# olga24912/lodestar

Hardware: AMD Instinct MI355X
Metric: verified signature sets/sec (node) (higher is better)
Workload: dtype u32/u64 (28-bit-limb Montgomery integer arithmetic); 1 GPU; C2 gossip attestation flood: 16384 single-pubkey sets per GPU, 1 set per batchable job; pk_mode=device table, sig_encoding=compressed 96 B, distinct_messages=16384, group_sets=1024, group_policy=0, inflight=32, slots=3, hw_queues=4, merge_sets=131072, pipeline_depth=3, parallelism=shard-by-job x1 (in-process devices), no collective

## Files before the change

### include/blsgpu.h

```cpp
#ifndef BLSGPU_H
#define BLSGPU_H

#include <stdint.h>

#ifdef __cplusplus
extern "C" {
#endif

#define BLSGPU_ABI_VERSION 8

#define BLSGPU_JOB_BATCHABLE 1u
#define BLSGPU_JOB_URGENT 2u

enum blsgpu_code {
  BLSGPU_OK = 0,
  BLSGPU_BAD_ENCODING = 1,
  BLSGPU_POINT_NOT_ON_CURVE = 2,
  BLSGPU_POINT_NOT_IN_GROUP = 3,
  BLSGPU_AGGR_TYPE_MISMATCH = 4,
  BLSGPU_VERIFY_FAIL = 5,
  BLSGPU_PK_IS_INFINITY = 6,
  BLSGPU_BAD_SCALAR = 7,
  BLSGPU_INVALID_SIZE = 8,
  BLSGPU_EMPTY_AGGREGATE = 9,
  BLSGPU_EMPTY_SET = 10,
  BLSGPU_DEVICE_ERROR = 11,
  BLSGPU_ERR_ARGS = 100,
  BLSGPU_ERR_NO_DEVICE = 101,
  BLSGPU_ERR_CLOSED = 102,
  BLSGPU_ERR_ENTROPY = 103
};

typedef struct blsgpu_ctx blsgpu_ctx;

typedef struct blsgpu_batch {
  uint32_t n_sets;
  uint32_t n_jobs;
  const uint32_t* job_first_set;
  const uint8_t* job_flags;
  const uint8_t* pk_bytes;
  const uint32_t* set_pk_first;
  const uint32_t* pk_index;
  const uint8_t* msgs;
  const uint8_t* sigs;
  const uint32_t* sig_len;
  uint32_t sig_stride;
  uint64_t seed;
} blsgpu_batch;

typedef struct blsgpu_stats {
  uint32_t groups;
  uint32_t batch_retries;
  uint32_t batch_sigs_success;
  uint32_t devices_used;
  double device_ms;
  double stage_ms[8];
  uint32_t unique_messages;
  uint32_t pairing_units;
  uint32_t miller_chunks;
  uint32_t run_sets;
  uint32_t run_calls;
  uint32_t fallback_jobs;
  uint32_t fallback_miller;
  uint32_t urgent_lane;
  double host_ms;
} blsgpu_stats;

int blsgpu_init(const int* devices, int n_devices, blsgpu_ctx** out);
void blsgpu_destroy(blsgpu_ctx* ctx);
int blsgpu_device_count(const blsgpu_ctx* ctx);

int blsgpu_pubkeys_upload(blsgpu_ctx* ctx, uint32_t first_index, const uint8_t* pk96, uint32_t n);
uint32_t blsgpu_pubkeys_count(const blsgpu_ctx* ctx);

int blsgpu_verify(blsgpu_ctx* ctx, const blsgpu_batch* batch, int8_t* job_result, blsgpu_stats* stats);

typedef void (*blsgpu_done_cb)(void* user, int status);
int blsgpu_submit(blsgpu_ctx* ctx, const blsgpu_batch* batch, int8_t* job_result, blsgpu_stats* stats,
                  blsgpu_done_cb done, void* user);

int blsgpu_set_option(blsgpu_ctx* ctx, const char* key, int64_t value);
int blsgpu_get_option(const blsgpu_ctx* ctx, const char* key, int64_t* value);

int blsgpu_chunkify(uint32_t len, uint32_t min_per_chunk, uint32_t* chunk_first, uint32_t* n_chunks);

int blsgpu_aggregate_pubkeys(blsgpu_ctx* ctx, const blsgpu_batch* b, uint8_t* out, uint32_t out_len,
                             int8_t* status);

#define BLSGPU_AGG_VALIDATE 1u

int blsgpu_aggregate_signatures(blsgpu_ctx* ctx, uint32_t n_groups, const uint32_t* group_first,
                                const uint8_t* sigs, uint32_t sig_stride, const uint32_t* sig_len,
                                uint32_t flags, uint8_t* out, uint32_t out_len, int8_t* status,
                                uint32_t* first_bad);
uint32_t blsgpu_sig_agg_lanes(uint32_t n_groups, uint32_t n_sigs);

int blsgpu_randomness_words(uint32_t n, uint64_t seed, uint64_t* words);

int blsgpu_aggregate_with_randomness(blsgpu_ctx* ctx, uint32_t n_groups, const uint32_t* group_first,
                                     const uint8_t* pk_bytes, const uint32_t* pk_index, const uint8_t* sigs,
                                     uint32_t sig_stride, const uint32_t* sig_len, uint64_t seed, uint8_t* out_pk,
                                     uint32_t out_pk_len, uint8_t* out_sig, uint32_t out_sig_len, int8_t* status,
                                     uint32_t* first_bad);
uint32_t blsgpu_awr_lanes(uint32_t n_groups, uint32_t n_sets);

#define BLSGPU_SAME_LANE_FORMS 1u

typedef struct blsgpu_same_message_stats {
  uint32_t groups_accepted;
  uint32_t groups_retried;
  uint32_t retry_sets;
  uint32_t unique_messages;
  uint32_t form;
  double device_ms;
} blsgpu_same_message_stats;

int blsgpu_verify_same_message(blsgpu_ctx* ctx, uint32_t n_groups, const uint32_t* group_first,
                               const uint8_t* msgs , const uint8_t* pk_bytes,
                               const uint32_t* pk_index, const uint8_t* sigs, uint32_t sig_stride,
                               const uint32_t* sig_len, uint64_t seed, uint32_t flags,
                               int8_t* set_result , int8_t* group_result ,
                               blsgpu_same_message_stats* stats );
uint32_t blsgpu_same_message_form(uint32_t n_items, uint32_t flags);

int blsgpu_key_validate(blsgpu_ctx* ctx, uint32_t n, const uint8_t* pks, uint32_t pk_len, uint32_t stride,
                        uint8_t* out96, int8_t* status);

#define BLSGPU_ROOT_OBJECT 0
#define BLSGPU_ROOT_ATTESTATION_DATA 1
int blsgpu_signing_roots(blsgpu_ctx* ctx, int kind, uint32_t n, const uint8_t* objects, uint32_t object_stride,
                         const uint8_t* domains, uint32_t domain_stride, uint8_t* out32);

int blsgpu_shard_jobs(const uint32_t* job_first_set, const uint32_t* set_pk_first, uint32_t n_jobs,
                      uint32_t n_parts, uint32_t* part_first_job);

int blsgpu_route_call(uint32_t n_sets, uint32_t n_devices, const int64_t* device_load, int64_t split_sets,
                      uint32_t start, uint32_t* out_devices, uint32_t* n_out);

int blsgpu_batch_scalars(const blsgpu_batch* b, uint64_t* words);

#define BLSGPU_INJECT_ENTROPY 1
#define BLSGPU_INJECT_DEVICE 2
int blsgpu_debug_inject(int what, int64_t skip, int64_t count);

const char* blsgpu_code_name(int code);

int blsgpu_debug_op(blsgpu_ctx* ctx, int op, uint32_t n, const uint8_t* in, uint32_t in_stride,
                    uint8_t* out, uint32_t out_stride, int32_t* status);

#ifdef __cplusplus
}
#endif
#endif
```

### lodestar_amd/build.py

```python
import hashlib
import os
import subprocess
import sys
import time

PKG = os.path.dirname(os.path.abspath(__file__))
ROOT = os.path.dirname(PKG)
CSRC = os.path.join(PKG, "csrc")
LIB = os.environ.get("BLSGPU_LIB") or os.path.join(PKG, "libblsgpu.so")
ARCH = os.environ.get("BLSGPU_ARCH", "gfx950")
HIPCC = os.environ.get("HIPCC", "/opt/rocm/bin/hipcc")
SOURCES = ["k_sig.hip", "k_msm.hip", "k_hash.hip", "k_hmap.hip", "k_pk.hip", "k_sigagg.hip", "k_awr.hip", "k_same.hip", "k_miller.hip", "k_group.hip", "k_inv.hip", "k_ssz.hip", "k_debug.hip",
           "runtime.cpp", "helpers.cpp"]


OBJ_DIR = os.path.join(PKG, "build")


TU_DEFINES = {"k_sig.hip": ["BLS_INLINE_BIG=1"]}


def tu_defines():
    env = os.environ.get("BLSGPU_TU_DEFINES")
    if env is None:
        return TU_DEFINES
    out = {}
    for part in filter(None, env.split(";")):
        tu, _, defs = part.partition("=")
        out[tu] = [d for d in defs.split("+") if d]
    return out


_ILP = ["-mllvm", "-amdgpu-sched-strategy=max-ilp"]
_MINREG = ["-mllvm", "-amdgpu-sched-strategy=iterative-minreg"]
TU_CFLAGS = {"k_hash.hip": _MINREG, "k_pk.hip": _ILP}


def tu_cflags():
    env = os.environ.get("BLSGPU_TU_CFLAGS")
    if env is None:
        return TU_CFLAGS
    out = {}
    for part in filter(None, env.split(";")):
        tu, _, flags = part.partition("=")
        out[tu] = flags.split()
    return out


def _headers():
    out = [os.path.join(ROOT, "include", "blsgpu.h")]
    for f in os.listdir(CSRC):
        if f.endswith((".hpp", ".h")):
            out.append(os.path.join(CSRC, f))
    return out


def _tu_deps(src):
    if src.endswith(".cpp"):
        return [os.path.join(CSRC, f) for f in (src, "kernels.h", "batch_rand.hpp", "runtime_internal.hpp",
                                                "helper_layout.hpp", "miller_plan.hpp")] + [
            os.path.join(ROOT, "include", "blsgpu.h")]
    return [os.path.join(CSRC, src)] + _headers()


def _deps():
    return _headers() + [os.path.join(CSRC, s) for s in SOURCES] + [os.path.abspath(__file__)]


def up_to_date():
    if not os.path.exists(LIB):
        return False
    t = os.path.getmtime(LIB)
    return all(os.path.getmtime(d) <= t for d in _deps())


def build(force=False, verbose=True):
    if not force and up_to_date():
        build_node_addon(verbose=verbose)
        return LIB
    objs = []
    common = ["-O3", "-std=c++17", "-fPIC", f"--offload-arch={ARCH}", "-I", os.path.join(ROOT, "include")]
    defines = os.environ.get("BLSGPU_DEFINES", "").split()
    common += ["-D" + d for d in defines]
    cflags = os.environ.get("BLSGPU_CFLAGS", "").split()
    common += cflags
    tu_defs = tu_defines()
    os.makedirs(OBJ_DIR, exist_ok=True)
    key = os.path.splitext(os.path.basename(LIB))[0] + ("." + "_".join(defines).replace("=", "-") if defines else "")
    if cflags:
        key += ".cf" + hashlib.md5(" ".join(cflags).encode()).hexdigest()[:8]
    procs = []
    t0 = time.time()
    for src in SOURCES:
        tdefs = tu_defs.get(src, [])
        tflags = tu_cflags().get(src, [])
        obj = os.path.join(OBJ_DIR, key + "." + os.path.splitext(src)[0] +
                           ("." + "_".join(tdefs).replace("=", "-") if tdefs else "") +
                           (".cf" + hashlib.md5(" ".join(tflags).encode()).hexdigest()[:8] if tflags else "") + ".o")
        objs.append(obj)
        if not force and os.path.exists(obj) and all(os.path.getmtime(d) <= os.path.getmtime(obj) for d in _tu_deps(src)):
            continue
        cmd = [HIPCC] + common + ["-D" + d for d in tdefs] + tflags + ["-c", os.path.join(CSRC, src), "-o", obj]
        if verbose:
            print(" ".join(cmd), flush=True)
        procs.append((src, subprocess.Popen(cmd)))
    for src, p in procs:
        if p.wait() != 0:
            raise RuntimeError(f"hipcc failed on {src}")
        if verbose:
            print(f"  {src}: done at {time.time() - t0:.0f} s", flush=True)
    cmd = [HIPCC, f"--offload-arch={ARCH}", "-shared", "-o", LIB] + objs + ["-lpthread"]
    if verbose:
        print(" ".join(cmd), flush=True)
    subprocess.check_call(cmd)
    build_node_addon(verbose=verbose)
    return LIB


NODE_DIR = os.path.join(PKG, "node")
ADDON = os.path.join(NODE_DIR, "blsgpu_napi.node")
NODE_INC = "/usr/include/node"


def build_node_addon(force=False, verbose=True):
    src = os.path.join(NODE_DIR, "blsgpu_napi.c")
    if not os.path.exists(os.path.join(NODE_INC, "node_api.h")):
        if verbose:
            print("node headers not found: N-API addon not built", flush=True)
        return None
    if not force and os.path.exists(ADDON) and os.path.getmtime(ADDON) >= max(
            os.path.getmtime(src), os.path.getmtime(LIB), os.path.getmtime(os.path.join(ROOT, "include", "blsgpu.h"))):
        return ADDON
    cmd = ["gcc", "-O2", "-std=c11", "-Wall", "-Wno-unused-parameter", "-shared", "-fPIC",
           "-DNODE_GYP_MODULE_NAME=blsgpu_napi", "-I", NODE_INC, "-I", os.path.join(ROOT, "include"), src,
           "-o", ADDON, "-L", PKG, "-l:libblsgpu.so", "-Wl,-rpath,$ORIGIN/.."]
    if verbose:
        print(" ".join(cmd), flush=True)
    subprocess.check_call(cmd)
    return ADDON


if __name__ == "__main__":
    build(force="--force" in sys.argv)
```

### lodestar_amd/csrc/helpers.cpp

```cpp
#include "helper_layout.hpp"
#include "runtime_internal.hpp"

using namespace blsgpu_rt;
namespace hl = helper_layout;

static_assert(hl::kFp == W_FP && hl::kG1A == W_G1A && hl::kG1J == W_G1J && hl::kG2A == W_G2A && hl::kG2J == W_G2J &&
                  hl::kFp12 == W_FP12 && hl::kAwrTabWords == AWR_TAB_WORDS && hl::kMillerLineWords == kMillerLineWords,
              "helper_layout.hpp restates the element widths of kernels.h");

namespace {

template <class Body>
int helper_call(blsgpu_ctx* ctx, bool reads_table, Body body) {
  if (!enter(ctx)) return BLSGPU_ERR_CLOSED;
  struct Leave {
    blsgpu_ctx* ctx;
    ~Leave() { leave(ctx); }
  } leave_on_exit{ctx};
  Device& d = *ctx->devs[0];
  try {
    std::lock_guard<std::mutex> helper(d.helper_mu);
    std::shared_lock<std::shared_mutex> tl(d.table_mu, std::defer_lock);
    if (reads_table) tl.lock();
    HIPCHK(hipSetDevice(d.id));
    return body(d, d.helper, d.table_stream);
  } catch (HipError&) {
    return BLSGPU_DEVICE_ERROR;
  }
}

struct Grouped {
  uint32_t G;
  const uint32_t* group_first;
  const uint8_t* sigs;
  uint32_t sig_stride;
  const uint32_t* sig_len;
  const uint8_t* pk_bytes = nullptr;
  const uint32_t* pk_index = nullptr;
  uint32_t n = 0;
};

int check_group_layout(Grouped& a) {
  if (a.group_first[0] != 0) return BLSGPU_ERR_ARGS;
  for (uint32_t g = 0; g < a.G; g++)
    if (a.group_first[g + 1] < a.group_first[g]) return BLSGPU_ERR_ARGS;
  a.n = a.group_first[a.G];
  if (a.n > (1u << 20)) return BLSGPU_ERR_ARGS;
  if (a.sig_stride < 192)
    for (uint32_t k = 0; k < a.n; k++)
      if (a.sig_len[k] == 192) return BLSGPU_ERR_ARGS;
  return BLSGPU_OK;
}

int same_begin(const Device& d, const Grouped& a, uint64_t seed, std::vector<uint64_t>& words, uint64_t& hash_key) {
  batch_rand::Key key;
  if (!resolve_key(seed, key, hash_key)) return BLSGPU_ERR_ENTROPY;
  words.resize(a.n);
  batch_rand::words(key, 0, a.n, words.data());
  if (a.pk_index)
    for (uint32_t k = 0; k < a.n; k++)
      if (a.pk_index[k] >= d.table_n) return BLSGPU_ERR_ARGS;
  return BLSGPU_OK;
}

template <class Layout>
PipelineBuffers sig_inputs(Slot& sl, const Grouped& a, const Layout& l, uint8_t* flags, uint8_t* status,
                           hipStream_t s) {
  uint8_t* din = sl.d_in.p;
  HIPCHK(hipMemcpyAsync(din + l.gf, a.group_first, (size_t)(a.G + 1) * 4, hipMemcpyHostToDevice, s));
  if (a.n) {
    HIPCHK(hipMemcpyAsync(din + l.len, a.sig_len, (size_t)a.n * 4, hipMemcpyHostToDevice, s));
    HIPCHK(hipMemcpyAsync(din + l.sigs, a.sigs, (size_t)a.n * a.sig_stride, hipMemcpyHostToDevice, s));
  }
  PipelineBuffers pb{};
  pb.n = a.n;
  pb.sigs = din + l.sigs;
  pb.sig_len = reinterpret_cast<uint32_t*>(din + l.len);
  pb.sig_stride = a.sig_stride;
  pb.sig_aff = sl.d_work.p;
  pb.flags = flags;
  pb.status = reinterpret_cast<int8_t*>(status);
  return pb;
}

template <class Layout>
AwrBuffers same_inputs(Device& d, const Grouped& a, const Layout& l, uint8_t* bytes, const uint64_t* words,
                       uint32_t lanes, hipStream_t s, PipelineBuffers& pb) {
  uint8_t* din = d.helper.d_in.p;
  uint32_t* w = d.helper.d_work.p;
  pb = sig_inputs(d.helper, a, l.in, bytes + l.b_fl, bytes + l.b_st, s);
  if (a.n) {
    HIPCHK(hipMemcpyAsync(din + l.in.words, words, (size_t)a.n * 8, hipMemcpyHostToDevice, s));
    HIPCHK(hipMemcpyAsync(din + l.in.keys, a.pk_bytes ? (const void*)a.pk_bytes : (const void*)a.pk_index,
                          l.in.key_bytes, hipMemcpyHostToDevice, s));
  }
  AwrBuffers ab{};
  ab.n = a.n;
  ab.n_groups = a.G;
  ab.group_first = reinterpret_cast<uint32_t*>(din + l.in.gf);
  ab.words = reinterpret_cast<uint64_t*>(din + l.in.words);
  ab.pk_bytes = a.pk_bytes ? din + l.in.keys : nullptr;
  ab.pk_index = a.pk_bytes ? nullptr : reinterpret_cast<uint32_t*>(din + l.in.keys);
  ab.pk_table = d.table.p;
  ab.pk_table_n = d.table_n;
  ab.sig_aff = pb.sig_aff;
  ab.sig_flags = pb.flags;
  ab.sig_status = pb.status;
  ab.tab = w + l.w_tab;
  ab.tab_n = lanes;
  ab.sum_pk = w + l.w_sum_pk;
  ab.sum_sig = w + l.w_sum_sig;
  ab.err_k = reinterpret_cast<uint32_t*>(bytes + l.b_ek);
  ab.err_c = reinterpret_cast<int8_t*>(bytes + l.b_ec);
  return ab;
}

}

extern "C" {

int blsgpu_aggregate_pubkeys(blsgpu_ctx* ctx, const blsgpu_batch* b, uint8_t* out, uint32_t out_len,
                             int8_t* status) {
  if (!ctx || ctx->devs.empty() || !b || !out || !status || (out_len != 48 && out_len != 96)) return BLSGPU_ERR_ARGS;
  const uint32_t n = b->n_sets;
  if (n == 0) return BLSGPU_OK;
  if (!b->pk_bytes && (!b->set_pk_first || !b->pk_index)) return BLSGPU_ERR_ARGS;
  return helper_call(ctx, true, [&](Device& d, Slot& sl, hipStream_t s) -> int {
    std::vector<uint32_t> spf(n + 1);
    for (uint32_t i = 0; i <= n; i++) spf[i] = b->set_pk_first ? b->set_pk_first[i] : i;
    const uint32_t npk = spf[n];
    if (!b->pk_bytes)
      for (uint32_t k = 0; k < npk; k++)
        if (b->pk_index[k] >= d.table_n) return BLSGPU_ERR_ARGS;
    const hl::AggPubkeys l(n, npk, b->pk_bytes != nullptr, out_len);
    sl.d_in.ensure(l.total);
    sl.d_work.ensure(l.work_words);
    uint8_t* din = sl.d_in.p;
    HIPCHK(hipMemcpyAsync(din + l.spf, spf.data(), (size_t)(n + 1) * 4, hipMemcpyHostToDevice, s));
    HIPCHK(hipMemcpyAsync(din + l.keys, b->pk_bytes ? (const void*)b->pk_bytes : (const void*)b->pk_index,
                          l.key_bytes, hipMemcpyHostToDevice, s));
    PipelineBuffers pb{};
    pb.n = n;
    pb.set_pk_first = reinterpret_cast<uint32_t*>(din + l.spf);
    pb.pk_bytes = b->pk_bytes ? din + l.keys : nullptr;
    pb.pk_index = b->pk_bytes ? nullptr : reinterpret_cast<uint32_t*>(din + l.keys);
    pb.pk_table = d.table.p;
    pb.pk_table_n = d.table_n;
    pb.pk_jac = sl.d_work.p;
    pb.status = reinterpret_cast<int8_t*>(din + l.st);
    launch_pk_aggregate(pb, n, s);
    launch_pk_serialize(pb, n, din + l.out, out_len, s);
    HIPCHK(hipGetLastError());
    HIPCHK(hipMemcpyAsync(out, din + l.out, (size_t)n * out_len, hipMemcpyDeviceToHost, s));
    HIPCHK(hipMemcpyAsync(status, din + l.st, n, hipMemcpyDeviceToHost, s));
    HIPCHK(hipStreamSynchronize(s));
    return BLSGPU_OK;
  });
}

int blsgpu_aggregate_signatures(blsgpu_ctx* ctx, uint32_t n_groups, const uint32_t* group_first,
                                const uint8_t* sigs, uint32_t sig_stride, const uint32_t* sig_len, uint32_t flags,
                                uint8_t* out, uint32_t out_len, int8_t* status, uint32_t* first_bad) {
  if (!ctx || ctx->devs.empty() || !group_first || !sigs || !sig_len || !out || !status) return BLSGPU_ERR_ARGS;
  if ((out_len != 96 && out_len != 192) || sig_stride < 96 || (flags & ~BLSGPU_AGG_VALIDATE)) return BLSGPU_ERR_ARGS;
  if (n_groups == 0) return BLSGPU_OK;
  Grouped a{n_groups, group_first, sigs, sig_stride, sig_len};
  if (int e = check_group_layout(a)) return e;
  const uint32_t n = a.n, G = n_groups;
  return helper_call(ctx, false, [&](Device& d, Slot& sl, hipStream_t s) -> int {
    const hl::AggSigs l(G, n, sig_stride, out_len);
    sl.d_in.ensure(l.total);
    sl.d_work.ensure(l.work_words);
    uint8_t* din = sl.d_in.p;
    const PipelineBuffers pb = sig_inputs(sl, a, l, din + l.fl, din + l.st, s);
    const uint32_t* d_first = reinterpret_cast<uint32_t*>(din + l.gf);
    uint32_t* agg = sl.d_work.p + l.w_agg;
    int8_t* d_gst = reinterpret_cast<int8_t*>(din + l.gst);
    uint32_t* d_fb = reinterpret_cast<uint32_t*>(din + l.fb);
    launch_sig_decode(pb, n, s, n <= 4096, nullptr, false, (flags & BLSGPU_AGG_VALIDATE) != 0);
    launch_sig_aggregate(pb, d_first, G, n, agg, d_gst, d_fb, s);
    launch_sig_agg_serialize(d_first, G, agg, d_gst, din + l.out, out_len, s);
    HIPCHK(hipGetLastError());
    HIPCHK(hipMemcpyAsync(out, din + l.out, (size_t)G * out_len, hipMemcpyDeviceToHost, s));
    HIPCHK(hipMemcpyAsync(status, din + l.gst, G, hipMemcpyDeviceToHost, s));
    if (first_bad) HIPCHK(hipMemcpyAsync(first_bad, din + l.fb, (size_t)G * 4, hipMemcpyDeviceToHost, s));
    HIPCHK(hipStreamSynchronize(s));
    return BLSGPU_OK;
  });
}

uint32_t blsgpu_sig_agg_lanes(uint32_t n_groups, uint32_t n_sigs) { return sig_agg_lanes(n_groups, n_sigs); }

int blsgpu_randomness_words(uint32_t n, uint64_t seed, uint64_t* words) {
  if (n && !words) return BLSGPU_ERR_ARGS;
  batch_rand::Key key;
  uint64_t hash_key = 0;
  if (!resolve_key(seed, key, hash_key)) return BLSGPU_ERR_ENTROPY;
  batch_rand::words(key, 0, n, words);
  return BLSGPU_OK;
}

int blsgpu_aggregate_with_randomness(blsgpu_ctx* ctx, uint32_t n_groups, const uint32_t* group_first,
                                     const uint8_t* pk_bytes, const uint32_t* pk_index, const uint8_t* sigs,
                                     uint32_t sig_stride, const uint32_t* sig_len, uint64_t seed, uint8_t* out_pk,
                                     uint32_t out_pk_len, uint8_t* out_sig, uint32_t out_sig_len, int8_t* status,
                                     uint32_t* first_bad) {
  if (!ctx || ctx->devs.empty() || !group_first || !sigs || !sig_len || !out_pk || !out_sig || !status)
    return BLSGPU_ERR_ARGS;
  if ((pk_bytes != nullptr) == (pk_index != nullptr)) return BLSGPU_ERR_ARGS;
  if ((out_pk_len != 48 && out_pk_len != 96) || (out_sig_len != 96 && out_sig_len != 192) || sig_stride < 96)
    return BLSGPU_ERR_ARGS;
  if (n_groups == 0) return BLSGPU_OK;
  Grouped a{n_groups, group_first, sigs, sig_stride, sig_len, pk_bytes, pk_index};
  if (int e = check_group_layout(a)) return e;
  const uint32_t n = a.n, G = n_groups;
  return helper_call(ctx, true, [&](Device& d, Slot& sl, hipStream_t s) -> int {
    std::vector<uint64_t> words;
    uint64_t hash_key = 0;
    if (int e = same_begin(d, a, seed, words, hash_key)) return e;
    const uint32_t L = awr_lanes(G, n), lanes = awr_launch_lanes(G, L);
    const hl::Awr l(G, n, sig_stride, pk_bytes != nullptr, out_pk_len, out_sig_len, lanes);
    sl.d_in.ensure(l.total);
    sl.d_work.ensure(l.work_words);
    uint8_t* din = sl.d_in.p;
    PipelineBuffers pb;
    const AwrBuffers ab = same_inputs(d, a, l, din, words.data(), lanes, s, pb);
    int8_t* d_gst = reinterpret_cast<int8_t*>(din + l.gst);
    uint32_t* d_fb = reinterpret_cast<uint32_t*>(din + l.fb);
    launch_sig_decode(pb, n, s, n <= 4096, nullptr, false, true);
    launch_awr_sums(ab, L, s);
    launch_awr_serialize(ab, din + l.opk, out_pk_len, din + l.osig, out_sig_len, d_gst, d_fb, s);
    HIPCHK(hipGetLastError());
    HIPCHK(hipMemcpyAsync(out_pk, din + l.opk, (size_t)G * out_pk_len, hipMemcpyDeviceToHost, s));
    HIPCHK(hipMemcpyAsync(out_sig, din + l.osig, (size_t)G * out_sig_len, hipMemcpyDeviceToHost, s));
    HIPCHK(hipMemcpyAsync(status, din + l.gst, G, hipMemcpyDeviceToHost, s));
    if (first_bad) HIPCHK(hipMemcpyAsync(first_bad, din + l.fb, (size_t)G * 4, hipMemcpyDeviceToHost, s));
    HIPCHK(hipStreamSynchronize(s));
    return BLSGPU_OK;
  });
}

uint32_t blsgpu_awr_lanes(uint32_t n_groups, uint32_t n_sets) { return awr_lanes(n_groups, n_sets); }

constexpr uint32_t kSameCoopMax = 512;
uint32_t blsgpu_same_message_form(uint32_t n_items, uint32_t flags) {
  return (flags & BLSGPU_SAME_LANE_FORMS) || n_items > kSameCoopMax ? 1u : 0u;
}
namespace {
inline bool same_serial() {
  static const bool on = [] {
    const char* v = getenv("BLSGPU_SAME_SERIAL");
    return v && v[0] == '1';
  }();
  return on;
}
void same_pairing_phase(const PipelineBuffers& pm, uint32_t n_items, const uint32_t* iota, uint32_t* pk_aff,
                        uint8_t* include, const uint32_t* msg_idx, const uint32_t* S, uint32_t* F, uint32_t* Gs,
                        uint8_t* ok, bool lane, hipStream_t s) {
  PipelineBuffers pb = pm;
  pb.n = n_items;
  pb.pk_aff = pk_aff;
  pb.include = include;
  pb.msg_idx = msg_idx;
  pb.n_chunks = n_items;
  pb.chunk_first = iota;
  pb.chunk_items = iota;
  pb.f_chunk = F;
  if (!lane) {
    launch_miller_coop(pb, false, s, false);
    launch_group_check(S, F, n_items, ok, s);
  } else {
    launch_miller_acc6(pb, false, s);
    launch_group_sig_miller(S, n_items, Gs, s, false, true);
    launch_group_check6(F, Gs, n_items, ok, s);
  }
}
}

int blsgpu_verify_same_message(blsgpu_ctx* ctx, uint32_t n_groups, const uint32_t* group_first, const uint8_t* msgs,
                               const uint8_t* pk_bytes, const uint32_t* pk_index, const uint8_t* sigs,
                               uint32_t sig_stride, const uint32_t* sig_len, uint64_t seed, uint32_t flags,
                               int8_t* set_result, int8_t* group_result, blsgpu_same_message_stats* stats) {
  if (!ctx || ctx->devs.empty() || !group_first || !msgs || !sigs || !sig_len || !set_result) return BLSGPU_ERR_ARGS;
  if ((pk_bytes != nullptr) == (pk_index != nullptr)) return BLSGPU_ERR_ARGS;
  if (sig_stride < 96 || (flags & ~BLSGPU_SAME_LANE_FORMS)) return BLSGPU_ERR_ARGS;
  if (n_groups == 0) {
    if (stats) memset(stats, 0, sizeof *stats);
    return BLSGPU_OK;
  }
  Grouped a{n_groups, group_first, sigs, sig_stride, sig_len, pk_bytes, pk_index};
  if (int e = check_group_layout(a)) return e;
  const uint32_t n = a.n, G = n_groups;
  std::vector<int8_t> h_set(n), h_grp(G);
  blsgpu_same_message_stats st;
  memset(&st, 0, sizeof st);
  const int rc = helper_call(ctx, true, [&](Device& d, Slot& sl, hipStream_t s) -> int {
    std::vector<uint64_t> words;
    uint64_t hash_key = 0;
    if (int e = same_begin(d, a, seed, words, hash_key)) return e;
    std::vector<uint32_t> gmsg(G), uniq;
    {
      MsgIndex mi(G, hash_key ^ 0x6a09e667f3bcc908ull);
      for (uint32_t g = 0; g < G; g++) gmsg[g] = mi.find_or_add(msgs, g, uniq);
    }
    const uint32_t U = (uint32_t)uniq.size();
    st.unique_messages = U;
    bool streams_used = false;
    try {
      if (!d.same_st[0]) {
        for (auto& e : d.same_ev) HIPCHK(hipEventCreateWithFlags(&e, hipEventDisableTiming));
        HIPCHK(hipStreamCreateWithFlags(&d.same_st[1], hipStreamNonBlocking));
        HIPCHK(hipStreamCreateWithFlags(&d.same_st[0], hipStreamNonBlocking));
      }
      const auto t0 = std::chrono::steady_clock::now();
      const bool serial = same_serial();
      hipStream_t sb = serial ? s : d.same_st[0], sc = serial ? s : d.same_st[1];
      const bool lane_g = blsgpu_same_message_form(G, flags) != 0;
      const uint32_t L = awr_lanes(G, n), lanes = awr_launch_lanes(G, L);
      const hl::Same l(G, n, U, sig_stride, pk_bytes != nullptr, lanes);
      sl.d_in.ensure(l.in_total);
      sl.d_bytes.ensure(l.bytes_total);
      sl.d_work.ensure(l.work_words);
      if (lane_g) sl.d_lines.ensure(l.lines_words);
      streams_used = true;
      uint8_t* din = sl.d_in.p;
      uint8_t* db = sl.d_bytes.p;
      uint32_t* w = sl.d_work.p;
      std::vector<uint32_t> iota((size_t)G + 1);
      for (uint32_t g = 0; g <= G; g++) iota[g] = g;
      std::vector<uint8_t> umsgs((size_t)U * 32);
      for (uint32_t u = 0; u < U; u++) memcpy(umsgs.data() + (size_t)u * 32, msgs + (size_t)uniq[u] * 32, 32);
      PipelineBuffers pb;
      const AwrBuffers ab = same_inputs(d, a, l, db, words.data(), lanes, s, pb);
      HIPCHK(hipMemcpyAsync(din + l.umsg, umsgs.data(), (size_t)U * 32, hipMemcpyHostToDevice, s));
      HIPCHK(hipMemcpyAsync(din + l.gmsg, gmsg.data(), (size_t)G * 4, hipMemcpyHostToDevice, s));
      HIPCHK(hipMemcpyAsync(din + l.iota, iota.data(), (size_t)(G + 1) * 4, hipMemcpyHostToDevice, s));
      AwrBuffers ab_pk = ab;
      ab_pk.tab = w + l.w_tab_pk;
      uint32_t* g_pk_aff = w + l.w_pk_aff;
      uint32_t* g_inv = w + l.w_inv;
      uint32_t* g_F = w + l.w_F;
      uint32_t* g_G = w + l.w_G;
      PipelineBuffers pm{};
      pm.umsgs = din + l.umsg;
      pm.n_umsg = U;
      pm.nm = U;
      pm.inv_buf = w + l.w_minv;
      pm.h_aff = w + l.w_haff;
      pm.h_jac = w + l.w_hjac;
      pm.h_norm = w + l.w_hnorm;
      pm.h_prep = w + l.w_hprep;
      pm.h_q = w + l.w_hq;
      pm.mflags = db + l.b_mf;
      pm.lines = sl.d_lines.p;
      uint8_t* g_inc = db + l.b_inc;
      int8_t* g_code = reinterpret_cast<int8_t*>(db + l.b_code);
      uint8_t* g_ok = db + l.b_ok;
      int8_t* d_gres = reinterpret_cast<int8_t*>(db + l.b_gres);
      int8_t* d_sres = reinterpret_cast<int8_t*>(db + l.b_sres);
      const uint32_t* d_gmsg = reinterpret_cast<uint32_t*>(din + l.gmsg);
      const uint32_t* d_iota = reinterpret_cast<uint32_t*>(din + l.iota);
      HIPCHK(hipEventRecord(d.same_ev[0], s));
      if (!serial) {
        HIPCHK(hipStreamWaitEvent(sb, d.same_ev[0], 0));
        HIPCHK(hipStreamWaitEvent(sc, d.same_ev[0], 0));
      }
      launch_sig_decode(pb, n, s, n <= 4096, nullptr, false, true);
      launch_awr_sum_sig(ab, L, s);
      launch_awr_sum_pk(ab_pk, L, sb);
      launch_batch_inv(ab.sum_pk, G, 2 * W_FP, g_inv, G, sb);
      HIPCHK(hipEventRecord(d.same_ev[1], sb));
      bool have_lines = false;
      launch_hash_to_g2(pm, sc, U <= 4096, false);
      launch_h_affine(pm, sc);
      if (lane_g) {
        launch_miller_lines2(pm, sc);
        have_lines = true;
      }
      HIPCHK(hipEventRecord(d.same_ev[2], sc));
      if (!serial) {
        HIPCHK(hipStreamWaitEvent(s, d.same_ev[1], 0));
        HIPCHK(hipStreamWaitEvent(s, d.same_ev[2], 0));
      }
      launch_same_group_items(ab, g_inv, g_pk_aff, g_inc, g_code, s);
      same_pairing_phase(pm, G, d_iota, g_pk_aff, g_inc, d_gmsg, ab.sum_sig, g_F, g_G, g_ok, lane_g, s);
      launch_same_group_results(ab.group_first, G, n, g_inc, g_code, g_ok, d_sres, d_gres, s);
      HIPCHK(hipGetLastError());
      HIPCHK(hipMemcpyAsync(h_grp.data(), d_gres, G, hipMemcpyDeviceToHost, s));
      HIPCHK(hipStreamSynchronize(s));
      if (lane_g) st.form |= 1;
      std::vector<uint32_t> rlist, rmsg, riota;
      for (uint32_t g = 0; g < G; g++) {
        if (group_first[g + 1] == group_first[g]) continue;
        if (h_grp[g] == 1) {
          st.groups_accepted++;
          continue;
        }
        st.groups_retried++;
        for (uint32_t k = group_first[g]; k < group_first[g + 1]; k++) {
          rlist.push_back(k);
          rmsg.push_back(gmsg[g]);
        }
      }
      const uint32_t nr = (uint32_t)rlist.size();
      st.retry_sets = nr;
      if (nr) {
        const bool lane_r = blsgpu_same_message_form(nr, flags) != 0;
        const hl::SameRetry r(nr);
        sl.d_list.ensure(r.list_words);
        sl.d_ok.ensure(r.ok_bytes);
        sl.d_fb.ensure(r.fb_words);
        sl.d_S.ensure(r.S_words);
        sl.d_F.ensure(r.F_words);
        if (lane_r) sl.d_G.ensure(r.F_words);
        if (lane_r && !have_lines) {
          sl.d_lines.ensure(l.lines_words);
          pm.lines = sl.d_lines.p;
        }
        riota.resize((size_t)nr + 1);
        for (uint32_t q = 0; q <= nr; q++) riota[q] = q;
        uint32_t* dl = sl.d_list.p;
        HIPCHK(hipMemcpyAsync(dl, rlist.data(), (size_t)nr * 4, hipMemcpyHostToDevice, s));
        HIPCHK(hipMemcpyAsync(dl + r.msg, rmsg.data(), (size_t)nr * 4, hipMemcpyHostToDevice, s));
        HIPCHK(hipMemcpyAsync(dl + r.iota, riota.data(), (size_t)(nr + 1) * 4, hipMemcpyHostToDevice, s));
        uint8_t* r_inc = sl.d_ok.p;
        int8_t* r_code = reinterpret_cast<int8_t*>(sl.d_ok.p + r.code);
        uint8_t* r_ok = sl.d_ok.p + r.ok;
        launch_same_retry_items(ab, dl, nr, sl.d_fb.p, sl.d_S.p, r_inc, r_code, s);
        if (lane_r && !have_lines) launch_miller_lines2(pm, s);
        same_pairing_phase(pm, nr, dl + r.iota, sl.d_fb.p, r_inc, dl + r.msg, sl.d_S.p, sl.d_F.p, sl.d_G.p, r_ok, lane_r,
                           s);
        launch_same_retry_results(dl, nr, r_inc, r_code, r_ok, d_sres, s);
        HIPCHK(hipGetLastError());
        if (lane_r) st.form |= 2;
      }
      if (n) HIPCHK(hipMemcpyAsync(h_set.data(), d_sres, n, hipMemcpyDeviceToHost, s));
      HIPCHK(hipStreamSynchronize(s));
      st.device_ms = ms_since(t0);
    } catch (HipError&) {
      if (streams_used) {
        (void)hipStreamSynchronize(d.table_stream);
        for (hipStream_t x : d.same_st)
          if (x) (void)hipStreamSynchronize(x);
      }
      throw;
    }
    return BLSGPU_OK;
  });
  if (rc == BLSGPU_OK) {
    if (n) memcpy(set_result, h_set.data(), n);
    if (group_result) memcpy(group_result, h_grp.data(), G);
    if (stats) *stats = st;
  }
  return rc;
}

int blsgpu_key_validate(blsgpu_ctx* ctx, uint32_t n, const uint8_t* pks, uint32_t pk_len, uint32_t stride,
                        uint8_t* out96, int8_t* status) {
  if (!ctx || ctx->devs.empty() || !pks || !status || stride < pk_len) return BLSGPU_ERR_ARGS;
  if (pk_len != 48 && pk_len != 96) return BLSGPU_ERR_ARGS;
  if (n == 0) return BLSGPU_OK;
  return helper_call(ctx, false, [&](Device& d, Slot& sl, hipStream_t s) -> int {
    const hl::KeyValidate l(n, stride);
    sl.d_in.ensure(l.total);
    uint8_t* din = sl.d_in.p;
    HIPCHK(hipMemcpyAsync(din, pks, (size_t)n * stride, hipMemcpyHostToDevice, s));
    launch_key_validate(din, n, pk_len, stride, din + l.out, reinterpret_cast<int8_t*>(din + l.st), s);
    HIPCHK(hipGetLastError());
    if (out96) HIPCHK(hipMemcpyAsync(out96, din + l.out, (size_t)n * 96, hipMemcpyDeviceToHost, s));
    HIPCHK(hipMemcpyAsync(status, din + l.st, n, hipMemcpyDeviceToHost, s));
    HIPCHK(hipStreamSynchronize(s));
    return BLSGPU_OK;
  });
}

int blsgpu_signing_roots(blsgpu_ctx* ctx, int kind, uint32_t n, const uint8_t* objects, uint32_t object_stride,
                         const uint8_t* domains, uint32_t domain_stride, uint8_t* out32) {
  if (!ctx || ctx->devs.empty() || !objects || !domains || !out32) return BLSGPU_ERR_ARGS;
  const uint32_t obj_len = kind == BLSGPU_ROOT_OBJECT ? 32 : (kind == BLSGPU_ROOT_ATTESTATION_DATA ? 128 : 0);
  if (!obj_len || object_stride < obj_len || (domain_stride != 0 && domain_stride < 32)) return BLSGPU_ERR_ARGS;
  if (n == 0) return BLSGPU_OK;
  return helper_call(ctx, false, [&](Device& d, Slot& sl, hipStream_t s) -> int {
    const hl::SigningRoots l(n, object_stride, domain_stride);
    sl.d_in.ensure(l.total);
    uint8_t* din = sl.d_in.p;
    HIPCHK(hipMemcpyAsync(din, objects, (size_t)n * object_stride, hipMemcpyHostToDevice, s));
    HIPCHK(hipMemcpyAsync(din + l.dom, domains, l.dom_bytes, hipMemcpyHostToDevice, s));
    launch_signing_roots(kind, din, n, object_stride, din + l.dom, domain_stride, din + l.out, s);
    HIPCHK(hipGetLastError());
    HIPCHK(hipMemcpyAsync(out32, din + l.out, 32 * (size_t)n, hipMemcpyDeviceToHost, s));
    HIPCHK(hipStreamSynchronize(s));
    return BLSGPU_OK;
  });
}

int blsgpu_debug_op(blsgpu_ctx* ctx, int op, uint32_t n, const uint8_t* in, uint32_t in_stride, uint8_t* out,
                    uint32_t out_stride, int32_t* status) {
  if (!ctx || ctx->devs.empty() || !in || !out || !status) return BLSGPU_ERR_ARGS;
  struct OpSize {
    int op;
    uint32_t in, out;
  };
  static const OpSize kOpSizes[] = {{0, 96, 48},    {1, 194, 192},  {2, 32, 192},   {3, 288, 576},  {4, 576, 576},
                                    {5, 104, 96},   {6, 200, 192},  {7, 64, 96},    {8, 32, 96},    {9, 200, 2880},
                                    {10, 104, 1440}, {11, 840, 56}, {16, 576, 576}, {17, 288, 576}, {18, 384, 192}};
  const OpSize* sz = nullptr;
  for (const OpSize& o : kOpSizes)
    if (o.op == op) sz = &o;
  if (!sz || in_stride < sz->in || out_stride < sz->out) return BLSGPU_ERR_ARGS;
  if (n == 0) return BLSGPU_OK;
  return helper_call(ctx, false, [&](Device& d, Slot& sl, hipStream_t s) -> int {
    struct Temp {
      void* p = nullptr;
      ~Temp() {
        if (p) (void)hipFree(p);
      }
    } din, dout, dst;
    HIPCHK(hipMalloc(&din.p, (size_t)n * in_stride));
    HIPCHK(hipMalloc(&dout.p, (size_t)n * out_stride));
    HIPCHK(hipMalloc(&dst.p, (size_t)n * 4));
    HIPCHK(hipMemcpyAsync(din.p, in, (size_t)n * in_stride, hipMemcpyHostToDevice, s));
    HIPCHK(hipMemsetAsync(dout.p, 0, (size_t)n * out_stride, s));
    launch_debug_op(op, n, (uint8_t*)din.p, in_stride, (uint8_t*)dout.p, out_stride, (int32_t*)dst.p, s);
    HIPCHK(hipGetLastError());
    HIPCHK(hipMemcpyAsync(out, dout.p, (size_t)n * out_stride, hipMemcpyDeviceToHost, s));
    HIPCHK(hipMemcpyAsync(status, dst.p, (size_t)n * 4, hipMemcpyDeviceToHost, s));
    HIPCHK(hipStreamSynchronize(s));
    return BLSGPU_OK;
  });
}

}
```

### lodestar_amd/csrc/k_pk.hip

```cpp
#include "k_common.hpp"

#ifndef BLSGPU_PK_AGG_GROUPS
#define BLSGPU_PK_AGG_GROUPS 1
#endif
__global__ __launch_bounds__(WAVE) void k_pk_aggregate(PipelineBuffers b, uint32_t n_sets) {
  __shared__ uint32_t red[WAVE * W_G1J];
  __shared__ uint32_t err_k[WAVE];
  __shared__ int32_t err_c[WAVE];
  if (blockIdx.x >= n_sets) return;
  const uint32_t set = b.agg_sets ? b.agg_sets[blockIdx.x] : blockIdx.x;
  uint32_t lane = threadIdx.x;
  int8_t* agg_status = b.status + 2 * b.n;
  const uint32_t first = b.set_pk_first[set], last = b.set_pk_first[set + 1];
  g1j acc = jac_infinity<fp>();
  uint32_t my_err_k = 0xffffffffu;
  int my_err = 0;
  for (uint32_t k = first + lane; k < last; k += WAVE) {
    g1a q;
    if (b.pk_bytes) {
      uint8_t raw[96];
      const uint8_t* src = b.pk_bytes + (size_t)k * 96;
#pragma unroll
      for (int t = 0; t < 96; t++) raw[t] = src[t];
      bool inf = false;
      const int st = pk_decode96(raw, q, inf);
      if (st != BLS_OK) {
        if (my_err == 0) {
          my_err = st;
          my_err_k = k;
        }
        continue;
      }
      if (inf) continue;
    } else {
      const uint32_t idx = b.pk_index[k];
      if (idx >= b.pk_table_n) {
        if (my_err == 0) {
          my_err = BLS_DEVICE_ERROR;
          my_err_k = k;
        }
        continue;
      }
      q = ld_pktab(b.pk_table, idx);
    }
    acc = jac_add_aff(acc, q);
  }
  err_k[lane] = my_err_k;
  err_c[lane] = my_err;
  __syncthreads();
  if (lane == 0) {
    uint32_t bk = 0xffffffffu;
    int bc = 0;
    for (int l = 0; l < WAVE; l++)
      if (err_k[l] < bk) {
        bk = err_k[l];
        bc = err_c[l];
      }
    agg_status[set] = (int8_t)bc;
  }
  const uint32_t cnt = last - first;
  if (cnt <= 1) {
    if (lane == 0) st_g1j(b.pk_jac, b.n, set, acc);
    return;
  }
#pragma unroll 1
  for (int s = WAVE / 2; s >= 1; s >>= 1) {
    if (lane >= (uint32_t)s && lane < (uint32_t)(2 * s)) {
#pragma unroll
      for (int l = 0; l < BLS_NL; l++) {
        red[(lane - s) * W_G1J + l] = acc.x.l[l];
        red[(lane - s) * W_G1J + W_FP + l] = acc.y.l[l];
        red[(lane - s) * W_G1J + 2 * W_FP + l] = acc.z.l[l];
      }
    }
    __syncthreads();
    if (lane < (uint32_t)s) {
      g1j o;
#pragma unroll
      for (int l = 0; l < BLS_NL; l++) {
        o.x.l[l] = red[lane * W_G1J + l];
        o.y.l[l] = red[lane * W_G1J + W_FP + l];
        o.z.l[l] = red[lane * W_G1J + 2 * W_FP + l];
      }
      acc = jac_add(acc, o);
    }
    __syncthreads();
  }
  if (lane == 0) st_g1j(b.pk_jac, b.n, set, acc);
}

BLS_INL fp fp_shfl_xor(const fp& x, int m) {
  fp r;
#pragma unroll
  for (int i = 0; i < BLS_NL; i++) r.l[i] = (uint32_t)__shfl_xor((int)x.l[i], m);
  return r;
}
template <int L>
__global__ __launch_bounds__(WAVE) __attribute__((amdgpu_waves_per_eu(2, 2))) void k_pk_aggregate_g(PipelineBuffers b, uint32_t n_sets) {
  const uint32_t q = blockIdx.x * WAVE + threadIdx.x, t = q % L;
  const uint32_t si = q / L;
  const bool on = si < n_sets;
  const uint32_t set = on ? (b.agg_sets ? b.agg_sets[si] : si) : 0;
  const uint32_t first = on ? b.set_pk_first[set] : 0, last = on ? b.set_pk_first[set + 1] : 0;
  g1j acc = jac_infinity<fp>();
  uint32_t my_err_k = 0xffffffffu;
  int my_err = 0;
  for (uint32_t k = first + t; k < last; k += L) {
    g1a pt;
    if (b.pk_bytes) {
      uint8_t raw[96];
      const uint8_t* src = b.pk_bytes + (size_t)k * 96;
#pragma unroll
      for (int z = 0; z < 96; z++) raw[z] = src[z];
      bool inf = false;
      const int st = pk_decode96(raw, pt, inf);
      if (st != BLS_OK) {
        if (my_err == 0) {
          my_err = st;
          my_err_k = k;
        }
        continue;
      }
      if (inf) continue;
    } else {
      const uint32_t idx = b.pk_index[k];
      if (idx >= b.pk_table_n) {
        if (my_err == 0) {
          my_err = BLS_DEVICE_ERROR;
          my_err_k = k;
        }
        continue;
      }
      pt = ld_pktab(b.pk_table, idx);
    }
    acc = jac_add_aff(acc, pt);
  }
#pragma unroll 1
  for (int m = L / 2; m >= 1; m >>= 1) {
    g1j o;
    o.x = fp_shfl_xor(acc.x, m);
    o.y = fp_shfl_xor(acc.y, m);
    o.z = fp_shfl_xor(acc.z, m);
    const uint32_t ok = (uint32_t)__shfl_xor((int)my_err_k, m);
    const int oc = __shfl_xor(my_err, m);
    if (ok < my_err_k) {
      my_err_k = ok;
      my_err = oc;
    }
    acc = jac_add(acc, o);
  }
  if (on && t == 0) {
    b.status[2 * b.n + set] = (int8_t)my_err;
    st_g1j(b.pk_jac, b.n, set, acc);
  }
}

__device__ __forceinline__ int set_pubkey(const PipelineBuffers& b, uint32_t i, g1j& P) {
  const bool one = b.set_pk_first && b.pk_direct1 && b.set_pk_first[i + 1] - b.set_pk_first[i] == 1;
  if (one && !b.pk_bytes) {
    const uint32_t idx = b.pk_index[b.set_pk_first[i]];
    if (idx >= b.pk_table_n) return BLS_DEVICE_ERROR;
    P = jac_from_aff(ld_pktab(b.pk_table, idx));
    return BLS_OK;
  }
  if (b.pk_bytes && (!b.set_pk_first || one)) {
    uint8_t raw[96];
    const uint32_t k = b.set_pk_first ? b.set_pk_first[i] : i;
    const uint4* src = reinterpret_cast<const uint4*>(b.pk_bytes + (size_t)k * 96);
#pragma unroll
    for (int k = 0; k < 6; k++) {
      uint4 v = src[k];
      uint32_t w[4] = {v.x, v.y, v.z, v.w};
#pragma unroll
      for (int j = 0; j < 16; j++) raw[16 * k + j] = (uint8_t)(w[j >> 2] >> (8 * (j & 3)));
    }
    g1a a;
    bool inf = false;
    int st = pk_decode96(raw, a, inf);
    if (st == BLS_OK && inf) st = BLS_PK_IS_INFINITY;
    if (st == BLS_OK) P = jac_from_aff(a);
    return st;
  }
  if (b.set_pk_first[i + 1] == b.set_pk_first[i]) return BLS_EMPTY_AGGREGATE;
  const int st = b.status[2 * b.n + i];
  if (st) return st;
  P = ld_g1j(b.pk_jac, b.n, i);
  return jac_is_inf(P) ? BLS_PK_IS_INFINITY : BLS_OK;
}

STAGE_KERNEL_W(BLSGPU_WPE_PK) void k_pk_finish(PipelineBuffers b, uint32_t n_sets, int8_t* pk_status) {
  uint32_t i = blockIdx.x * WAVE + threadIdx.x;
  if (i >= n_sets) return;
  g1j P;
  int st = set_pubkey(b, i, P);
  g1j R = jac_infinity<fp>();
  if (st == BLS_OK) {
    const uint64_t w = b.scalars[i];
    R = (w == 0) ? P : jac_mul_scalar_word(P, w, b.scal_tab, b.n, i);
  }
  st_g1j(b.pk_jac, b.n, i, R);
  pk_status[i] = (int8_t)st;
}

STAGE_KERNEL void k_unit_aggregate(PipelineBuffers b) {
  uint32_t u = blockIdx.x * WAVE + threadIdx.x;
  if (u >= b.n_units) return;
  const uint32_t a = b.unit_set_first[u], e = b.unit_set_first[u + 1];
  g1a out;
  out.x = fp_zero();
  out.y = fp_zero();
  bool ok = false;
  if (e - a == 1) {
    const uint32_t i = b.unit_sets[a];
    if (b.include[i]) {
      out = ld_g1a(b.pk_aff, b.n, i);
      ok = true;
    }
  } else {
    g1j acc = jac_infinity<fp>();
    for (uint32_t k = a; k < e; k++) {
      const uint32_t i = b.unit_sets[k];
      if (b.include[i]) acc = jac_add_aff(acc, ld_g1a(b.pk_aff, b.n, i));
    }
    ok = jac_to_aff(acc, out);
  }
  st_g1a(b.unit_p, b.n, u, out);
  b.unit_ok[u] = ok ? 1 : 0;
}

__global__ __launch_bounds__(WAVE) void k_pk_serialize(PipelineBuffers b, uint32_t n_sets, uint8_t* out,
                                                       uint32_t out_len) {
  uint32_t i = blockIdx.x * WAVE + threadIdx.x;
  if (i >= n_sets) return;
  int st = b.set_pk_first[i + 1] == b.set_pk_first[i] ? BLS_EMPTY_AGGREGATE : b.status[2 * b.n + i];
  uint8_t buf[96];
  for (int k = 0; k < 96; k++) buf[k] = 0;
  if (st == BLS_OK) {
    g1a a;
    if (!jac_to_aff(ld_g1j(b.pk_jac, b.n, i), a)) {
      buf[0] = out_len == 48 ? 0xc0 : 0x40;
    } else if (out_len == 48) {
      g1a_compress(a, buf);
    } else {
      g1a_to_be96(a, buf);
    }
  }
  uint8_t* o = out + (size_t)i * out_len;
  for (uint32_t k = 0; k < out_len; k++) o[k] = buf[k];
  b.status[i] = (int8_t)st;
}

__global__ __launch_bounds__(WAVE) void k_key_validate(const uint8_t* pks, uint32_t n, uint32_t pk_len, uint32_t stride,
                                                       uint8_t* out96, int8_t* status) {
  uint32_t i = blockIdx.x * WAVE + threadIdx.x;
  if (i >= n) return;
  uint8_t raw[96];
  const uint8_t* src = pks + (size_t)i * stride;
  for (uint32_t k = 0; k < 96; k++) raw[k] = k < pk_len ? src[k] : 0;
  g1a a;
  const int st = pk_key_validate(raw, pk_len, a);
  uint8_t buf[96];
  for (int k = 0; k < 96; k++) buf[k] = 0;
  if (st == BLS_OK) g1a_to_be96(a, buf);
  if (out96)
    for (int k = 0; k < 96; k++) out96[(size_t)i * 96 + k] = buf[k];
  status[i] = (int8_t)st;
}

__global__ __launch_bounds__(WAVE) void k_pk_table_fill(const uint8_t* pk96, uint32_t n, uint32_t* table_dst,
                                                        int8_t* status) {
  uint32_t i = blockIdx.x * WAVE + threadIdx.x;
  if (i >= n) return;
  uint8_t raw[96];
  for (int k = 0; k < 96; k++) raw[k] = pk96[(size_t)i * 96 + k];
  g1a a;
  bool inf = false;
  int st = pk_decode96(raw, a, inf);
  if (st == BLS_OK && inf) st = BLS_PK_IS_INFINITY;
  uint32_t* dst = table_dst + (size_t)i * W_PKTAB;
  for (int l = 0; l < BLS_NL; l++) {
    dst[l] = st == BLS_OK ? a.x.l[l] : 0;
    dst[BLS_NL + l] = st == BLS_OK ? a.y.l[l] : 0;
  }
  dst[2 * BLS_NL] = 0;
  dst[2 * BLS_NL + 1] = 0;
  dst[2 * BLS_NL + 2] = 0;
  dst[2 * BLS_NL + 3] = 0;
  status[i] = (int8_t)st;
}

static inline dim3 grid_for(uint32_t n) { return dim3((n + WAVE - 1) / WAVE); }

void launch_pk_aggregate(const PipelineBuffers& b, uint32_t n, hipStream_t s) {
  if (b.agg_sets) n = b.n_agg;
  if (!n) return;
  const uint32_t lanes = 1024 * WAVE;
  if ((uint64_t)n * 64 <= lanes || !BLSGPU_PK_AGG_GROUPS)
    hipLaunchKernelGGL(k_pk_aggregate, dim3(n), dim3(WAVE), 0, s, b, n);
  else if ((uint64_t)n * 32 <= 2 * lanes)
    hipLaunchKernelGGL(k_pk_aggregate_g<32>, dim3((n * 32 + WAVE - 1) / WAVE), dim3(WAVE), 0, s, b, n);
  else if ((uint64_t)n * 16 <= 2 * lanes)
    hipLaunchKernelGGL(k_pk_aggregate_g<16>, dim3((n * 16 + WAVE - 1) / WAVE), dim3(WAVE), 0, s, b, n);
  else
    hipLaunchKernelGGL(k_pk_aggregate_g<8>, dim3((n * 8 + WAVE - 1) / WAVE), dim3(WAVE), 0, s, b, n);
}
void launch_pk_finish(const PipelineBuffers& b, uint32_t n, hipStream_t s) {
  if (n) hipLaunchKernelGGL(k_pk_finish, grid_for(n), dim3(WAVE), 0, s, b, n, b.status + b.n);
}
void launch_unit_aggregate(const PipelineBuffers& b, hipStream_t s) {
  if (b.n_units) hipLaunchKernelGGL(k_unit_aggregate, grid_for(b.n_units), dim3(WAVE), 0, s, b);
}
void launch_pk_serialize(const PipelineBuffers& b, uint32_t n, uint8_t* out, uint32_t out_len, hipStream_t s) {
  if (n) hipLaunchKernelGGL(k_pk_serialize, grid_for(n), dim3(WAVE), 0, s, b, n, out, out_len);
}
void launch_key_validate(const uint8_t* pks, uint32_t n, uint32_t pk_len, uint32_t stride, uint8_t* out96,
                         int8_t* status, hipStream_t s) {
  if (n) hipLaunchKernelGGL(k_key_validate, grid_for(n), dim3(WAVE), 0, s, pks, n, pk_len, stride, out96, status);
}
void launch_pk_table_fill(const uint8_t* pk96, uint32_t n, uint32_t* table_dst, int8_t* status, hipStream_t s) {
  if (n) hipLaunchKernelGGL(k_pk_table_fill, grid_for(n), dim3(WAVE), 0, s, pk96, n, table_dst, status);
}
```

### lodestar_amd/csrc/kernels.h

```cpp
#pragma once
#include <hip/hip_runtime.h>
#include <stdint.h>
#include <vector>

#define W_FP 14
#define W_G1A (2 * W_FP)
#define W_G1J (3 * W_FP)
#define W_G2A (4 * W_FP)
#define W_G2J (6 * W_FP)
#define W_FP12 (12 * W_FP)
#define W_PKTAB 32
#define MILLER_STEPS 68
#define W_LINE (3 * 2 * W_FP)

#define SF_SIG_INF 1u
#define MF_H_INF 1u

struct PipelineBuffers {
  uint32_t n;
  const uint8_t* sigs;
  const uint32_t* sig_len;
  uint32_t sig_stride;
  const uint8_t* pk_bytes;
  const uint32_t* set_pk_first;
  const uint32_t* pk_index;
  const uint32_t* pk_table;
  uint32_t pk_table_n;
  const uint32_t* agg_sets;
  uint32_t n_agg;
  uint32_t pk_direct1;
  const uint64_t* scalars;
  uint32_t* scal_tab;
  const uint32_t* job_first_set;
  uint32_t n_jobs;
  const uint8_t* umsgs;
  const uint32_t* msg_idx;
  uint32_t n_umsg;
  uint32_t nm;
  uint32_t n_units;
  const uint32_t* unit_set_first;
  const uint32_t* unit_sets;
  const uint32_t* unit_msg;
  uint32_t* sig_aff;
  uint32_t* h_aff;
  uint32_t* h_jac;
  uint32_t* h_norm;
  uint32_t* h_prep;
  uint32_t* h_q;
  uint32_t* inv_buf;
  uint32_t* inv_buf_pk;
  uint32_t* pk_jac;
  uint32_t* pk_aff;
  uint32_t* rsig;
  uint32_t* unit_p;
  uint32_t n_chunks;
  const uint32_t* chunk_first;
  const uint32_t* chunk_items;
  uint32_t* f_chunk;
  uint32_t* lines;
  uint8_t* flags;
  uint8_t* mflags;
  uint8_t* unit_ok;
  int8_t* status;
  int8_t* job_err;
  uint8_t* include;
};

void launch_sig_decode(const PipelineBuffers& b, uint32_t n_sets, hipStream_t s, bool coop = false,
                       hipEvent_t decoded = nullptr, bool exclusive = true, bool subgroup = true);
void launch_spec_mask(const PipelineBuffers& b, uint32_t n_sets, uint8_t* spec, hipStream_t s);
void launch_hash_prep(const PipelineBuffers& b, hipStream_t s);
void launch_hash_map(const PipelineBuffers& b, const uint32_t* inv, hipStream_t s);
void launch_hash_to_g2(const PipelineBuffers& b, hipStream_t s, bool coop = false,
                       bool exclusive = true);
void launch_pk_aggregate(const PipelineBuffers& b, uint32_t n_sets, hipStream_t s);
void launch_pk_finish(const PipelineBuffers& b, uint32_t n_sets, hipStream_t s);
void launch_batch_inv(const uint32_t* src, uint32_t src_stride, int w0, uint32_t* dst, uint32_t n, hipStream_t s);
void launch_pk_affine(const PipelineBuffers& b, uint32_t n_sets, hipStream_t s);
void launch_h_affine(const PipelineBuffers& b, hipStream_t s);
void launch_sig_scale(const PipelineBuffers& b, uint32_t n_sets, hipStream_t s, const uint32_t* list = nullptr);
#ifndef MSM_SLICE
#define MSM_SLICE 256
#endif
#define MSM_BUCKET_WORDS (128 * W_G2J)
#define MSM_WINDOW_WORDS (16 * W_G2J)
void launch_sig_msm(const PipelineBuffers& b, const uint32_t* slices, uint32_t n_slices, const uint32_t* range_slices,
                    uint32_t n_ranges, uint32_t* B, uint32_t* W, uint32_t* S, hipStream_t s, bool lane_tail = false,
                    uint32_t tree_slices = 0);
void launch_job_mask(const PipelineBuffers& b, hipStream_t s);
void launch_unit_aggregate(const PipelineBuffers& b, hipStream_t s);
void launch_miller_lines(const PipelineBuffers& b, hipStream_t s);
void launch_miller_lines2(const PipelineBuffers& b, hipStream_t s);
void launch_miller_accx(const PipelineBuffers& b, bool units, hipStream_t s);
#define MILLER_MAX_SEGS 8
struct MillerSegs {
  uint32_t n;
  uint32_t first[MILLER_MAX_SEGS + 1];
  uint32_t dbl[MILLER_MAX_SEGS];
};
void launch_miller_acc(const PipelineBuffers& b, bool units, hipStream_t s, const MillerSegs* segs = nullptr);
void launch_miller_acc2(const PipelineBuffers& b, bool units, hipStream_t s);
void launch_miller_acc6(const PipelineBuffers& b, bool units, hipStream_t s);
#ifndef BLSGPU_EXCLUSIVE_SMALL
#define BLSGPU_EXCLUSIVE_SMALL 1
#endif
void launch_miller_coop(const PipelineBuffers& b, bool units, hipStream_t s, bool exclusive = false);
void launch_group_reduce(const PipelineBuffers& b, const uint32_t* f_ranges, uint32_t n_groups, uint32_t* F,
                         hipStream_t s);
void launch_group_tree(const PipelineBuffers& b, const uint32_t* f_ranges, uint32_t n_groups, const uint32_t* runs,
                       uint32_t n_runs, const uint32_t* pairs, const std::vector<uint32_t>& level_end, uint32_t* F,
                       hipStream_t s, const MillerSegs* segs = nullptr, uint32_t* H = nullptr);
void launch_group_check(const uint32_t* S, const uint32_t* F, uint32_t n_groups, uint8_t* ok, hipStream_t s,
                        const uint32_t* sel = nullptr, uint32_t n_sel = 0, const uint32_t* G = nullptr,
                        bool exclusive = false, bool lane = false);
void launch_group_check6(const uint32_t* F, const uint32_t* G, uint32_t n_groups, uint8_t* ok, hipStream_t s,
                         const uint32_t* sel = nullptr, uint32_t n_sel = 0);
void launch_check6_miller(const uint32_t* S, const uint32_t* F, uint32_t n_groups, uint8_t* ok, hipStream_t s,
                          const uint32_t* sel, uint32_t n_sel, uint32_t* lines, uint8_t* flags);
void launch_group_sig_miller_sel(const uint32_t* S, uint32_t n_groups, const uint32_t* sel, uint32_t n_sel, uint32_t* G,
                                 hipStream_t s);
void launch_group_sig_miller(const uint32_t* S, uint32_t n_groups, uint32_t* G, hipStream_t s, bool exclusive = false,
                             bool lane = false);
void launch_copy_words(uint32_t* dst, const uint32_t* src, size_t n, hipStream_t s);
void launch_group_reduce_lane(const PipelineBuffers& b, const uint32_t* set_ranges, const uint32_t* f_ranges,
                              uint32_t n_groups, uint32_t* S, uint32_t* F, hipStream_t s);
void launch_range_combine_lane(const uint32_t* S_in, const uint32_t* F_in, uint32_t n_in, const uint32_t* ranges,
                               uint32_t n_out, uint32_t* S_out, uint32_t* F_out, hipStream_t s);
void launch_range_combine(const uint32_t* S_in, const uint32_t* F_in, uint32_t n_in, const uint32_t* ranges,
                          uint32_t n_out, uint32_t* S_out, uint32_t* F_out, hipStream_t s);
void launch_pk_table_fill(const uint8_t* pk96, uint32_t n, uint32_t* table_dst, int8_t* status, hipStream_t s);
void launch_pk_serialize(const PipelineBuffers& b, uint32_t n_sets, uint8_t* out, uint32_t out_len, hipStream_t s);
void launch_key_validate(const uint8_t* pks, uint32_t n, uint32_t pk_len, uint32_t stride, uint8_t* out96,
                         int8_t* status, hipStream_t s);
inline uint32_t sig_agg_lanes(uint32_t n_groups, uint32_t n_sigs) {
  if (n_groups == 0) return 1;
  const uint64_t n = n_groups, lanes = 1024 * 64;
  const uint32_t by_count = n * 64 <= lanes ? 64 : n * 32 <= 2 * lanes ? 32 : n * 16 <= 2 * lanes ? 16
                            : n * 8 <= 2 * lanes ? 8 : 1;
  const uint64_t mean = ((uint64_t)n_sigs + n - 1) / n;
  const uint32_t by_size = mean <= 3 ? 1 : mean <= 8 ? 8 : mean <= 16 ? 16 : mean <= 32 ? 32 : 64;
  return by_count < by_size ? by_count : by_size;
}
void launch_sig_aggregate(const PipelineBuffers& b, const uint32_t* group_first, uint32_t n_groups, uint32_t n_sigs,
                          uint32_t* agg, int8_t* agg_status, uint32_t* first_bad, hipStream_t s);
void launch_sig_agg_serialize(const uint32_t* group_first, uint32_t n_groups, const uint32_t* agg, int8_t* agg_status,
                              uint8_t* out, uint32_t out_len, hipStream_t s);
struct AwrBuffers {
  uint32_t n;
  uint32_t n_groups;
  const uint32_t* group_first;
  const uint64_t* words;
  const uint8_t* pk_bytes;
  const uint32_t* pk_index;
  const uint32_t* pk_table;
  uint32_t pk_table_n;
  const uint32_t* sig_aff;
  const uint8_t* sig_flags;
  const int8_t* sig_status;
  uint32_t* tab;
  uint32_t tab_n;
  uint32_t* sum_pk;
  uint32_t* sum_sig;
  uint32_t* err_k;
  int8_t* err_c;
};
#define AWR_TAB_WORDS (9 * W_G2J)
inline uint32_t awr_lanes(uint32_t n_groups, uint32_t n_sets) {
  if (n_groups == 0) return 1;
  const uint64_t n = n_groups, lanes = 1024 * 64;
  const uint32_t by_count = n * 64 <= lanes ? 64 : n * 32 <= lanes ? 32 : n * 16 <= lanes ? 16 : n * 8 <= lanes ? 8 : 1;
  const uint64_t mean = ((uint64_t)n_sets + n - 1) / n;
  const uint32_t by_size = mean <= 1 ? 1 : mean <= 8 ? 8 : mean <= 16 ? 16 : mean <= 32 ? 32 : 64;
  return by_count < by_size ? by_count : by_size;
}
uint32_t awr_launch_lanes(uint32_t n_groups, uint32_t L);
void launch_awr_sums(const AwrBuffers& a, uint32_t L, hipStream_t s);
void launch_awr_sum_pk(const AwrBuffers& a, uint32_t L, hipStream_t s);
void launch_awr_sum_sig(const AwrBuffers& a, uint32_t L, hipStream_t s);
void launch_same_group_items(const AwrBuffers& a, const uint32_t* inv, uint32_t* pk_aff, uint8_t* include, int8_t* code,
                             hipStream_t s);
void launch_same_retry_items(const AwrBuffers& a, const uint32_t* list, uint32_t n_retry, uint32_t* pk_aff, uint32_t* S,
                             uint8_t* include, int8_t* code, hipStream_t s);
void launch_same_group_results(const uint32_t* group_first, uint32_t n_groups, uint32_t n_sets, const uint8_t* include,
                               const int8_t* code, const uint8_t* ok, int8_t* set_result, int8_t* group_result,
                               hipStream_t s);
void launch_same_retry_results(const uint32_t* list, uint32_t n_retry, const uint8_t* include, const int8_t* code,
                               const uint8_t* ok, int8_t* set_result, hipStream_t s);
void launch_awr_serialize(const AwrBuffers& a, uint8_t* out_pk, uint32_t out_pk_len, uint8_t* out_sig,
                          uint32_t out_sig_len, int8_t* status, uint32_t* first_bad, hipStream_t s);
void launch_signing_roots(int kind, const uint8_t* in, uint32_t n, uint32_t in_stride, const uint8_t* domain,
                          uint32_t domain_stride, uint8_t* out, hipStream_t s);
void launch_debug_op(int op, uint32_t n, const uint8_t* in, uint32_t in_stride, uint8_t* out, uint32_t out_stride,
                     int32_t* status, hipStream_t s);
```

### lodestar_amd/csrc/runtime.cpp

```cpp
#include <pthread.h>
#include <stdio.h>
#include <sys/random.h>

#include <cmath>
#include <string>
#include <system_error>

#include "runtime_internal.hpp"
#include "miller_plan.hpp"

using namespace blsgpu_rt;

namespace {

std::atomic<int64_t> g_fail_run_skip{0}, g_fail_run_count{0};
thread_local bool tl_dispatcher = false;

inline uint32_t chunk_size(uint32_t len, uint32_t min_per_chunk) {
  const uint32_t count = min_per_chunk ? len / min_per_chunk : 0;
  return count <= 1 ? len : (len + count - 1) / count;
}

struct GroupPlanEntry {
  uint32_t first, end;
// ... 75 lines not shown
};

}

namespace {

void shard_rule(const uint32_t* jfs, const uint32_t* spf, uint32_t n_jobs, uint32_t n_parts, uint32_t* out) {
  const uint32_t n_sets = n_jobs ? jfs[n_jobs] : 0;
  std::vector<double> set_prefix(n_sets + 1, 0.0);
  for (uint32_t i = 0; i < n_sets; i++)
    set_prefix[i + 1] = set_prefix[i] + 1.0 + (spf ? (double)(spf[i + 1] - spf[i]) / 256.0 : 0.0);
  std::vector<double> cost(n_jobs + 1);
  for (uint32_t j = 0; j <= n_jobs; j++) cost[j] = set_prefix[n_jobs ? jfs[j] : 0];
  uint32_t j0 = 0;
  out[0] = 0;
  for (uint32_t k = 0; k < n_parts; k++) {
    uint32_t j1;
    if (k + 1 == n_parts) {
      j1 = n_jobs;
    } else {
      const double target = cost[n_jobs] * (k + 1) / n_parts;
      j1 = (uint32_t)(std::upper_bound(cost.begin(), cost.end(), target) - cost.begin());
      j1 = j1 ? j1 - 1 : 0;
      j1 = std::max(j0, j1);
    }
    out[k + 1] = j1;
    j0 = j1;
  }
}

uint32_t route_rule(uint32_t n_sets, uint32_t n_dev, const int64_t* load, int64_t split_sets, uint32_t start,
                    uint32_t* out) {
  if (n_dev == 0) return 0;
  const uint64_t per = (uint64_t)std::max<int64_t>(1, split_sets);
  const uint32_t k = (uint32_t)std::max<uint64_t>(1, std::min<uint64_t>(n_dev, n_sets / per));
  std::vector<uint32_t> order(n_dev);
  for (uint32_t d = 0; d < n_dev; d++) order[d] = d;
  std::stable_sort(order.begin(), order.end(), [&](uint32_t a, uint32_t b) {
    if (load[a] != load[b]) return load[a] < load[b];
    return (a + n_dev - start % n_dev) % n_dev < (b + n_dev - start % n_dev) % n_dev;
  });
  std::sort(order.begin(), order.begin() + k);
  for (uint32_t i = 0; i < k; i++) out[i] = order[i];
  return k;
}


uint32_t adapt_group_sets(Device& d, int64_t group_sets, double sets_per_job) {
  double f;
  {
    std::lock_guard<std::mutex> lk(d.fail_mu);
    f = d.fail_rate;
  }
  const uint32_t gmax = (uint32_t)std::max<int64_t>(1, group_sets);
  if (f <= 0 || gmax <= 8) return gmax;
  const double retry = 13600.0 / (16.0 * std::max(1.0, sets_per_job)) + 1300.0, fixed = 14700.0;
  uint32_t best = gmax;
  double best_c = fixed / gmax + (1.0 - std::pow(1.0 - f, (double)gmax)) * retry;
  for (uint32_t g = 8; g < gmax; g *= 2) {
    const double c = fixed / g + (1.0 - std::pow(1.0 - f, (double)g)) * retry;
    if (c < best_c) best_c = c, best = g;
  }
  return best;
}

static bool host_trace() {
  static const bool on = [] {
    const char* v = getenv("BLSGPU_HOST_TRACE");
    return v && v[0] == '1';
  }();
  return on;
}
thread_local std::chrono::steady_clock::time_point tl_run_t0;
thread_local double tl_merge_ms = 0;

void release_inflight(Device& d, Slot& sl) {
  {
    std::lock_guard<std::mutex> lk(d.q_mu);
    if (!sl.in_flight) return;
    sl.in_flight = false;
    d.runs_inflight--;
  }
  d.q_cv.notify_all();
}

int run_shard(Device& d, Slot& sl, const blsgpu_batch& b, const Shard& sh, int8_t* job_result, uint64_t seed,
              const Options& opt, uint32_t max_index, blsgpu_stats& st, const uint64_t* scal_words,
              const std::vector<GroupPlanEntry>* plan = nullptr) {
  const uint32_t n = sh.set_end - sh.set_begin;
  const uint32_t nj = sh.job_end - sh.job_begin;
  if (nj == 0) return BLSGPU_OK;
  HIPCHK(hipSetDevice(d.id));
  const auto t_prep0 = std::chrono::steady_clock::now();
  const uint64_t grow0 = tl_async_grow;
  const uint32_t s0 = sh.set_begin;
  const uint32_t stride = std::max<uint32_t>(n, 1);
  const bool table_mode = b.pk_bytes == nullptr;
  const bool bytes_agg = b.pk_bytes && b.set_pk_first;
  const uint32_t pk_base = b.set_pk_first ? b.set_pk_first[s0] : 0;
  const uint32_t npk = b.set_pk_first ? b.set_pk_first[sh.set_end] - pk_base : 0;
  if (table_mode && npk && max_index >= d.table_n) return BLSGPU_ERR_ARGS;

  std::vector<uint64_t> scal(n);
  std::vector<std::pair<uint32_t, uint32_t>> group_jobs;
  std::vector<uint8_t> group_batchable;
  if (plan) {
    for (const GroupPlanEntry& g : *plan) {
      uint32_t sets = 0;
      for (uint32_t j = g.first; j < g.end; j++)
        sets += b.job_first_set[sh.job_begin + j + 1] - b.job_first_set[sh.job_begin + j];
      if (!sets) continue;
      group_jobs.push_back({g.first, g.end});
      group_batchable.push_back(g.batchable);
    }
  } else {
    const uint32_t gs = opt.group_adapt ? adapt_group_sets(d, opt.group_sets, (double)n / std::max(nj, 1u))
                                        : (uint32_t)opt.group_sets;
    uint32_t cur_sets = 0;
    bool open = false;
    for (uint32_t j = 0; j < nj; j++) {
      const uint32_t gj = sh.job_begin + j;
      const uint32_t a = b.job_first_set[gj] - s0, e = b.job_first_set[gj + 1] - s0;
      const bool batchable = b.job_flags && (b.job_flags[gj] & 1u);
      if (e == a) {
        open = false;
        continue;
      }
      if (!batchable) {
        group_jobs.push_back({j, j + 1});
        open = false;
        continue;
      }
      if (!open || cur_sets >= gs) {
        group_jobs.push_back({j, j});
        cur_sets = 0;
        open = true;
      }
      group_jobs.back().second = j + 1;
      cur_sets += e - a;
    }
  }
  memcpy(scal.data(), scal_words, (size_t)n * 8);
  auto job_sets = [&](uint32_t j) {
    const uint32_t gj = sh.job_begin + j;
    return std::make_pair(b.job_first_set[gj] - s0, b.job_first_set[gj + 1] - s0);
  };
  const uint32_t ng0 = (uint32_t)group_jobs.size();

  std::vector<uint32_t> msg_idx(n), uniq;
  if (opt.dedupe) {
    MsgIndex mi(n, seed ^ 0x6a09e667f3bcc908ull);
    uniq.reserve(n);
    const uint8_t* ms = b.msgs + (size_t)s0 * 32;
    constexpr uint32_t kAhead = 16;
    size_t hq[kAhead];
    for (uint32_t i = 0; i < std::min(n, kAhead); i++) {
      hq[i] = mi.hash(ms, i);
      __builtin_prefetch(&mi.slot[hq[i]]);
    }
    for (uint32_t i = 0; i < n; i++) {
      const size_t h = hq[i % kAhead];
      if (i + kAhead < n) {
        hq[i % kAhead] = mi.hash(ms, i + kAhead);
        __builtin_prefetch(&mi.slot[hq[i % kAhead]]);
      }
      msg_idx[i] = mi.find_or_add_h(ms, i, h, uniq);
    }
  } else {
    uniq.resize(n);
    for (uint32_t i = 0; i < n; i++) msg_idx[i] = uniq[i] = i;
  }
  const uint32_t n_umsg = (uint32_t)uniq.size();
  const uint32_t nm = std::max<uint32_t>(n_umsg, 1);
  const double t_dedupe_ms = host_trace() ? ms_since(t_prep0) : 0;
  std::vector<uint32_t> unit_of_set(n, UINT32_MAX), unit_msg, unit_first, unit_sets, g_unit_first(ng0 + 1, 0);
  bool merged = false;
  if (opt.dedupe && n_umsg < n) {
    std::vector<uint32_t> stamp(n_umsg, UINT32_MAX), unit_of_msg(n_umsg, 0);
    for (uint32_t g = 0; g < ng0; g++) {
      g_unit_first[g] = (uint32_t)unit_msg.size();
      const uint32_t a = job_sets(group_jobs[g].first).first, e = job_sets(group_jobs[g].second - 1).second;
      for (uint32_t i = a; i < e; i++) {
        const uint32_t m = msg_idx[i];
        if (stamp[m] != g) {
          stamp[m] = g;
          unit_of_msg[m] = (uint32_t)unit_msg.size();
          unit_msg.push_back(m);
        }
        unit_of_set[i] = unit_of_msg[m];
      }
    }
    g_unit_first[ng0] = (uint32_t)unit_msg.size();
    merged = unit_msg.size() < (size_t)n;
    if (merged) {
      const uint32_t nu = (uint32_t)unit_msg.size();
      unit_first.assign(nu + 1, 0);
      for (uint32_t i = 0; i < n; i++)
        if (unit_of_set[i] != UINT32_MAX) unit_first[unit_of_set[i] + 1]++;
      for (uint32_t u = 0; u < nu; u++) unit_first[u + 1] += unit_first[u];
      unit_sets.resize(unit_first[nu]);
      std::vector<uint32_t> fill(unit_first.begin(), unit_first.end() - 1);
      for (uint32_t i = 0; i < n; i++)
        if (unit_of_set[i] != UINT32_MAX) unit_sets[fill[unit_of_set[i]]++] = i;
    }
  }
  const uint32_t n_units = merged ? (uint32_t)unit_msg.size() : 0;
  const uint32_t n_items = merged ? n_units : n;
  const bool coop = n_items <= (uint32_t)opt.coop_max && opt.miller_k <= 1;
  const bool coop_g2 = n <= (uint32_t)opt.coop_g2_max;
  const bool excl = BLSGPU_EXCLUSIVE_SMALL && n_items <= (uint32_t)opt.coop_excl_max && (!sl.urgent || opt.urgent_excl);
  const uint32_t mk_whole = coop ? 1u : opt.miller_k > 0 ? (uint32_t)opt.miller_k : miller_k_auto(n_items);
  auto group_items = [&](uint32_t g) -> std::pair<uint32_t, uint32_t> {
    if (merged) return {g_unit_first[g], g_unit_first[g + 1]};
    return {job_sets(group_jobs[g].first).first, job_sets(group_jobs[g].second - 1).second};
  };
  const AccForm form_whole = acc_form(mk_whole, n_items, opt.miller_lanes, opt.acc6_max, opt.miller_pairs != 0);
  uint32_t mk = mk_whole, segs = 1;
  bool seg_plan = false;
  if (opt.miller_segments > 0) {
    if (!coop && form_whole == AccForm::one) segs = (uint32_t)std::min<int64_t>(opt.miller_segments, mk);
  } else if (!coop && opt.miller_lanes == 0 && (form_whole == AccForm::one || form_whole == AccForm::two)) {
    std::vector<uint32_t> g_len(ng0);
    for (uint32_t g = 0; g < ng0; g++) g_len[g] = group_items(g).second - group_items(g).first;
    bool hold = false;
    if (opt.keep_f && !merged && mk_whole == 1 && ng0) {
      std::lock_guard<std::mutex> lk(d.fail_mu);
      hold = miller_plan::hold_kept_values(d.fail_rate, (double)n / ng0);
    }
    const miller_plan::Plan pl =
        miller_plan::plan_auto(n_items, g_len.data(), ng0, stride, opt.miller_k > 0 || hold, mk_whole);
    seg_plan = pl.k != mk_whole || pl.segs > 1;
    mk = pl.k, segs = pl.segs;
  }
  const bool interleave = segs > 1 || seg_plan;
  std::vector<uint32_t> chunk_first{0}, chunk_items, g_chunks(2 * (size_t)ng0);
  chunk_items.reserve(n);
  for (uint32_t g = 0; g < ng0; g++) {
    const auto ae = group_items(g);
    const auto cr = add_chunks(chunk_first, chunk_items, ae.first, ae.second, mk, interleave);
    g_chunks[2 * g] = cr.first;
    g_chunks[2 * g + 1] = cr.second;
  }
  const uint32_t n_chunks = (uint32_t)chunk_first.size() - 1;
  segs = miller_plan::fit_segments(n_chunks, segs, stride);
  MillerSegs msegs{};
  {
    const miller_plan::Segments sg = miller_plan::segments(segs);
    msegs.n = sg.n;
    for (uint32_t j = 0; j <= sg.n; j++) msegs.first[j] = sg.first[j];
    for (uint32_t j = 0; j < sg.n; j++) msegs.dbl[j] = sg.dbl[j];
  }
  const bool keep_f = opt.keep_f && !merged && mk == 1 && n_chunks == n;
  const bool small = n <= (uint32_t)opt.small_max;
  const bool spec = BLSGPU_STREAM_PAIRS && (small || opt.spec_large) && sl.alone && !opt.serial;
  const bool rsig_spec = spec && small && opt.rsig_spec;
  constexpr uint32_t kMsmHalfSliceMaxSets = 32768, kMsmSmallSliceMaxSets = 1024;
  const uint32_t slice_len = n <= kMsmSmallSliceMaxSets  ? 32
                             : n <= kMsmHalfSliceMaxSets ? (uint32_t)opt.msm_slice_mid
                                                         : MSM_SLICE;
  std::vector<uint32_t> slices, range_slices{0};
  uint32_t msm_tree = 0;
  for (uint32_t g = 0; g < ng0; g++)
    add_slices(slices, range_slices, job_sets(group_jobs[g].first).first, job_sets(group_jobs[g].second - 1).second,
               slice_len);
  const uint32_t n_slices = (uint32_t)(slices.size() / 2);
  if (n <= kMsmHalfSliceMaxSets && opt.msm_tree) {
    for (uint32_t g = 0; g < ng0; g++) msm_tree = std::max(msm_tree, range_slices[g + 1] - range_slices[g]);
    if ((uint64_t)ng0 * msm_tree > 2ull * n_slices) msm_tree = 0;
  }
  std::vector<uint32_t> ftree, f_level_end;
  uint32_t f_k = 1, f_max = 0;
  const uint32_t n_slots = n_chunks * segs, n_franges = ng0 * segs;
  std::vector<uint32_t> f_rng(2 * (size_t)n_franges);
  for (uint32_t j = 0; j < segs; j++)
    for (uint32_t g = 0; g < ng0; g++) {
      f_rng[2 * ((size_t)j * ng0 + g)] = j * n_chunks + g_chunks[2 * g];
      f_rng[2 * ((size_t)j * ng0 + g) + 1] = j * n_chunks + g_chunks[2 * g + 1];
    }
  if (n_slots > 16384)
    for (const uint32_t heads = opt.f_run_max > 16 ? 256u : 8192u;
         n_slots / f_k > heads && f_k < (uint32_t)opt.f_run_max;)
      f_k *= 2;
  for (uint32_t g = 0; g < ng0; g++) f_max = std::max(f_max, g_chunks[2 * g + 1] - g_chunks[2 * g]);
  if (f_k > 1)
    for (uint32_t r = 0; r < n_franges; r++)
      for (uint32_t x = f_rng[2 * r], e = f_rng[2 * r + 1]; x < e; x += f_k)
        if (std::min(e, x + f_k) - x > 1) {
          ftree.push_back(x);
          ftree.push_back(std::min(e, x + f_k));
        }
  const uint32_t n_fruns = (uint32_t)(ftree.size() / 2);
  for (uint32_t st = f_k; st < f_max; st *= 2) {
    for (uint32_t r = 0; r < n_franges; r++)
      for (uint32_t i = f_rng[2 * r], e = f_rng[2 * r + 1]; i + st < e; i += 2 * st) {
        ftree.push_back(i);
        ftree.push_back(i + st);
      }
    f_level_end.push_back((uint32_t)(ftree.size() / 2) - n_fruns);
  }
  std::vector<uint32_t> agg_sets;
  if (table_mode || bytes_agg)
    for (uint32_t i = 0; i < n; i++)
      if (b.set_pk_first[s0 + i + 1] - b.set_pk_first[s0 + i] >= 2) agg_sets.push_back(i);

  const double t_struct_ms = host_trace() ? ms_since(t_prep0) : 0;
  uint32_t sig_w = 96;
  for (uint32_t i = 0; i < n; i++)
    if (b.sig_len[s0 + i] == 192) {
      sig_w = 192;
      break;
    }
  const size_t o_scal = 0, o_jobs = al256(o_scal + (size_t)n * 8), o_sigs = al256(o_jobs + (size_t)(nj + 1) * 4),
               o_siglen = al256(o_sigs + (size_t)n * sig_w), o_umsg = al256(o_siglen + (size_t)n * 4),
               o_midx = al256(o_umsg + (size_t)n_umsg * 32), o_ranges = al256(o_midx + (size_t)n * 4),
               o_franges = al256(o_ranges + (size_t)std::max(ng0, 1u) * 8),
               o_ufirst = al256(o_franges + (size_t)std::max(n_franges, 1u) * 8),
               o_usets = al256(o_ufirst + (size_t)(n_units + 1) * 4), o_umsgi = al256(o_usets + (size_t)unit_sets.size() * 4),
               o_cfirst = al256(o_umsgi + (size_t)n_units * 4), o_citems = al256(o_cfirst + (size_t)(n_chunks + 1) * 4),
               o_agg = al256(o_citems + chunk_items.size() * 4), o_slices = al256(o_agg + agg_sets.size() * 4),
               o_rslices = al256(o_slices + slices.size() * 4), o_ftree = al256(o_rslices + range_slices.size() * 4),
               o_pk = al256(o_ftree + ftree.size() * 4);
  size_t in_bytes;
  if (table_mode)
    in_bytes = al256(o_pk + (size_t)(n + 1) * 4) + (size_t)npk * 4;
  else if (bytes_agg)
    in_bytes = al256(o_pk + (size_t)(n + 1) * 4) + (size_t)npk * 96;
  else
    in_bytes = o_pk + (size_t)n * 96;
  const size_t o_pk2 = al256(o_pk + (size_t)(n + 1) * 4);
  hipStream_t* const dst = sl.urgent ? d.ust : d.st;
  const int npairs = sl.urgent ? 2 : d.npairs;
  const int par = sl.urgent ? 0 : BLSGPU_STREAM_PAIRS ? (int)(d.run_seq.fetch_add(1) % (uint32_t)npairs) : 0;
  const int other = (par + 1) % npairs;
  hipStream_t s = BLSGPU_STREAM_PAIRS ? dst[2 * par] : dst[kSig];
  sl.set_stream(s);
  sl.h_in.ensure(in_bytes);
  sl.d_in.ensure(in_bytes);
  uint8_t* const hin = sl.h_in.p;
  memcpy(hin + o_scal, scal.data(), (size_t)n * 8);
  uint32_t* hjobs = reinterpret_cast<uint32_t*>(hin + o_jobs);
  for (uint32_t j = 0; j < nj; j++) hjobs[j] = job_sets(j).first;
  hjobs[nj] = n;
  uint8_t* hsigs = hin + o_sigs;
  uint32_t* hsiglen = reinterpret_cast<uint32_t*>(hin + o_siglen);
  if (b.sig_stride == sig_w) {
    memcpy(hsigs, b.sigs + (size_t)s0 * sig_w, (size_t)n * sig_w);
    memcpy(hsiglen, b.sig_len + s0, (size_t)n * 4);
  } else {
    for (uint32_t i = 0; i < n; i++) {
      const uint32_t len = b.sig_len[s0 + i];
      const uint32_t cl = (len == 96 || len == 192) ? len : 0;
      memcpy(hsigs + (size_t)i * sig_w, b.sigs + (size_t)(s0 + i) * b.sig_stride, cl);
      hsiglen[i] = len;
    }
  }
  for (uint32_t u = 0; u < n_umsg; u++) memcpy(hin + o_umsg + (size_t)u * 32, b.msgs + (size_t)(s0 + uniq[u]) * 32, 32);
  memcpy(hin + o_midx, msg_idx.data(), (size_t)n * 4);
  uint32_t* hranges = reinterpret_cast<uint32_t*>(hin + o_ranges);
  uint32_t* hfranges = reinterpret_cast<uint32_t*>(hin + o_franges);
  for (uint32_t g = 0; g < ng0; g++) {
    hranges[2 * g] = job_sets(group_jobs[g].first).first;
    hranges[2 * g + 1] = job_sets(group_jobs[g].second - 1).second;
  }
  memcpy(hfranges, f_rng.data(), f_rng.size() * 4);
  memcpy(hin + o_cfirst, chunk_first.data(), chunk_first.size() * 4);
  memcpy(hin + o_citems, chunk_items.data(), chunk_items.size() * 4);
  if (!agg_sets.empty()) memcpy(hin + o_agg, agg_sets.data(), agg_sets.size() * 4);
  if (!slices.empty()) memcpy(hin + o_slices, slices.data(), slices.size() * 4);
  memcpy(hin + o_rslices, range_slices.data(), range_slices.size() * 4);
  if (!ftree.empty()) memcpy(hin + o_ftree, ftree.data(), ftree.size() * 4);
  if (merged) {
    memcpy(hin + o_ufirst, unit_first.data(), (size_t)(n_units + 1) * 4);
    memcpy(hin + o_usets, unit_sets.data(), unit_sets.size() * 4);
    memcpy(hin + o_umsgi, unit_msg.data(), (size_t)n_units * 4);
  }
  if (table_mode || bytes_agg) {
    uint32_t* hpkfirst = reinterpret_cast<uint32_t*>(hin + o_pk);
    for (uint32_t i = 0; i <= n; i++) hpkfirst[i] = b.set_pk_first[s0 + i] - pk_base;
    if (table_mode)
      memcpy(hin + o_pk2, b.pk_index + pk_base, (size_t)npk * 4);
    else
      memcpy(hin + o_pk2, b.pk_bytes + (size_t)pk_base * 96, (size_t)npk * 96);
  } else {
    memcpy(hin + o_pk, b.pk_bytes + (size_t)s0 * 96, (size_t)n * 96);
  }

  const size_t ob_flags = 0, ob_mflags = al256(n), ob_unit = al256(ob_mflags + nm), ob_status = al256(ob_unit + n),
               ob_include = al256(ob_status + 3 * (size_t)stride), ob_spec = al256(ob_include + stride),
               bytes_total = al256(ob_spec + stride);
  sl.d_bytes.ensure(bytes_total);
  const uint32_t max_ranges = std::max<uint32_t>(std::max(ng0, nj), 1);
  const size_t o_ok = al256(nj), res_bytes = o_ok + max_ranges;
  sl.d_res.ensure(res_bytes);
  sl.h_res.ensure(res_bytes);
  sl.d_S.ensure((size_t)W_G2J * max_ranges);
  sl.d_F.ensure((size_t)W_FP12 * max_ranges);
  sl.d_G.ensure((size_t)W_FP12 * std::max<uint32_t>(ng0, 1));
  sl.d_msmB.ensure((size_t)MSM_BUCKET_WORDS * std::max<uint32_t>(n_slices, 1));
  sl.d_msmW.ensure((size_t)MSM_WINDOW_WORDS * max_ranges);
  const size_t per_set = W_G2A + W_G1J + W_G1A + W_FP12 + 8 * W_G1J + 2 * W_FP + (merged ? W_G1A : 0);
  sl.d_work.ensure((size_t)stride * per_set + (size_t)nm * (W_G2A + W_G2J + W_FP + 14 * W_FP + 2 * W_G2J));
  sl.d_lines.ensure((size_t)nm * kMillerLineWords);
  if (keep_f) sl.d_fkeep.ensure((size_t)stride * W_FP12);
  if (segs > 1) sl.d_fseg.ensure((size_t)W_FP12 * n_franges);
  if (rsig_spec) sl.d_fb.ensure((size_t)stride * 9 * W_G2J);
  uint8_t* const din = sl.d_in.p;
  uint8_t* const d_ok0 = sl.d_res.p + o_ok;

  PipelineBuffers pb;
  memset(&pb, 0, sizeof pb);
  pb.n = stride;
  pb.sigs = din + o_sigs;
  pb.sig_len = reinterpret_cast<uint32_t*>(din + o_siglen);
  pb.sig_stride = sig_w;
  pb.pk_bytes = table_mode ? nullptr : din + (bytes_agg ? o_pk2 : o_pk);
  pb.set_pk_first = (table_mode || bytes_agg) ? reinterpret_cast<uint32_t*>(din + o_pk) : nullptr;
  pb.pk_index = table_mode ? reinterpret_cast<uint32_t*>(din + o_pk2) : nullptr;
  pb.pk_table = d.table.p;
  pb.pk_table_n = d.table_n;
  pb.agg_sets = reinterpret_cast<uint32_t*>(din + o_agg);
  pb.n_agg = (uint32_t)agg_sets.size();
  pb.pk_direct1 = 1;
  pb.scalars = reinterpret_cast<uint64_t*>(din + o_scal);
  pb.job_first_set = reinterpret_cast<uint32_t*>(din + o_jobs);
  pb.n_jobs = nj;
  pb.umsgs = din + o_umsg;
  pb.msg_idx = reinterpret_cast<uint32_t*>(din + o_midx);
  pb.n_umsg = n_umsg;
  pb.nm = nm;
  pb.n_units = n_units;
  pb.unit_set_first = reinterpret_cast<uint32_t*>(din + o_ufirst);
  pb.unit_sets = reinterpret_cast<uint32_t*>(din + o_usets);
  pb.unit_msg = reinterpret_cast<uint32_t*>(din + o_umsgi);
  uint32_t* w = sl.d_work.p;
  pb.sig_aff = w; w += (size_t)stride * W_G2A;
  pb.pk_jac = w; w += (size_t)stride * W_G1J;
  pb.pk_aff = w; w += (size_t)stride * W_G1A;
  pb.rsig = nullptr;
  pb.f_chunk = w; w += (size_t)stride * W_FP12;
  pb.scal_tab = w; w += (size_t)stride * 8 * W_G1J;
  if (merged) {
    pb.unit_p = w; w += (size_t)stride * W_G1A;
  }
  pb.n_chunks = n_chunks;
  pb.chunk_first = reinterpret_cast<uint32_t*>(din + o_cfirst);
  pb.chunk_items = reinterpret_cast<uint32_t*>(din + o_citems);
  pb.inv_buf = w; w += (size_t)stride * W_FP;
  pb.inv_buf_pk = w; w += (size_t)stride * W_FP;
  pb.h_aff = w; w += (size_t)nm * W_G2A;
  pb.h_jac = w; w += (size_t)nm * W_G2J;
  pb.h_norm = w; w += (size_t)nm * W_FP;
  pb.h_prep = w; w += (size_t)nm * 14 * W_FP;
  pb.h_q = w;
  pb.lines = sl.d_lines.p;
  uint8_t* const db = sl.d_bytes.p;
  pb.flags = db + ob_flags;
  pb.mflags = db + ob_mflags;
  pb.unit_ok = db + ob_unit;
  pb.status = reinterpret_cast<int8_t*>(db + ob_status);
  pb.include = db + ob_include;
  pb.job_err = reinterpret_cast<int8_t*>(sl.d_res.p);

  const bool prof = opt.profile;
  const bool lane_tail = opt.lane_tail_min > 0 && n >= (uint32_t)opt.lane_tail_min;
  hipStream_t sm = BLSGPU_STREAM_PAIRS ? dst[2 * par + 1] : dst[kMsg],
              sp = BLSGPU_STREAM_PAIRS ? (small && sl.alone ? dst[2 * other] : s) : dst[kPk],
              stl = BLSGPU_STREAM_PAIRS ? s : dst[kTail];
  if (opt.serial) sm = sp = stl = s;
  auto beg = [&](int k, hipStream_t st) {
    if (prof) HIPCHK(hipEventRecord(sl.ev[2 * k], st));
  };
  auto end = [&](int k, hipStream_t st) {
    if (prof) HIPCHK(hipEventRecord(sl.ev[2 * k + 1], st));
  };
  {
    std::unique_lock<std::mutex> enq(d.enq_mu, std::defer_lock);
    if (!sl.urgent) enq.lock();
    st.host_ms = ms_since(tl_run_t0);
    if (host_trace())
      fprintf(stderr,
              "[blsgpu host] run %u sets: merge %.2f ms, prep %.2f ms (dedupe %.2f, structure %.2f), pick-to-copy %.2f "
              "ms, %zu B in, %u Miller chunks of %u x %u segments\n",
              n, tl_merge_ms, ms_since(t_prep0), t_dedupe_ms, t_struct_ms, ms_since(tl_run_t0), in_bytes, n_chunks, mk,
              segs);
    const bool own_copy = opt.copy_stream && !opt.serial && !sl.urgent && tl_async_grow == grow0;
    hipStream_t sc = own_copy ? d.table_stream : s;
    HIPCHK(hipMemcpyAsync(din, hin, in_bytes, hipMemcpyHostToDevice, sc));
    HIPCHK(hipEventRecord(sl.join_in, sc));
    if (own_copy) HIPCHK(hipStreamWaitEvent(s, sl.join_in, 0));
    HIPCHK(hipStreamWaitEvent(sm, sl.join_in, 0));
    HIPCHK(hipStreamWaitEvent(sp, sl.join_in, 0));
    beg(1, sm);
    launch_hash_to_g2(pb, sm, coop_g2, excl);
    launch_h_affine(pb, sm);
    end(1, sm);
    beg(kStages, sm);
    if (!coop) {
      const bool two = opt.lines_lanes == 2;
      if (two)
        launch_miller_lines2(pb, sm);
      else
        launch_miller_lines(pb, sm);
    }
    end(kStages, sm);
    beg(2, sp);
    if ((table_mode || bytes_agg) && pb.n_agg) launch_pk_aggregate(pb, n, sp);
    end(2, sp);
    beg(3, sp);
    launch_pk_finish(pb, n, sp);
    launch_pk_affine(pb, n, sp);
    end(3, sp);
    HIPCHK(hipEventRecord(sl.join_pk, sp));
    hipStream_t smsm = spec ? dst[2 * other + 1] : s;
    PipelineBuffers pbm = pb;
    if (spec) pbm.include = db + ob_spec;
    beg(0, s);
    launch_sig_decode(pb, n, s, coop_g2, spec ? sl.join_dec : nullptr, excl);
    end(0, s);
    const uint32_t* d_slices = reinterpret_cast<uint32_t*>(din + o_slices);
    const uint32_t* d_rslices = reinterpret_cast<uint32_t*>(din + o_rslices);
    if (rsig_spec) {
      HIPCHK(hipEventRecord(sl.join_rsig, s));
      HIPCHK(hipStreamWaitEvent(sp, sl.join_rsig, 0));
      PipelineBuffers pq = pb;
      pq.rsig = sl.d_fb.p;
      pq.scal_tab = sl.d_fb.p + (size_t)stride * W_G2J;
      launch_sig_scale(pq, n, sp);
      HIPCHK(hipEventRecord(sl.join_rsig, sp));
    }
    if (spec) {
      HIPCHK(hipStreamWaitEvent(smsm, sl.join_dec, 0));
      launch_spec_mask(pb, n, pbm.include, smsm);
      launch_sig_msm(pbm, d_slices, n_slices, d_rslices, ng0, sl.d_msmB.p, sl.d_msmW.p, sl.d_S.p, smsm, false,
                     msm_tree);
      HIPCHK(hipEventRecord(sl.join_msm, smsm));
    }
    HIPCHK(hipStreamWaitEvent(s, sl.join_pk, 0));
    beg(4, s);
    launch_job_mask(pb, s);
    HIPCHK(hipEventRecord(sl.join_mask, s));
    HIPCHK(hipStreamWaitEvent(sm, sl.join_mask, 0));
    beg(5, sm);
    if (merged) launch_unit_aggregate(pb, sm);
    if (coop)
      launch_miller_coop(pb, merged, sm, excl);
    else if (seg_plan)
      launch_miller_acc(pb, merged, sm, &msegs);
    else
      launch_miller_acc_auto(pb, merged, sm, mk, opt.miller_lanes, opt.acc6_max, opt.miller_pairs != 0, &msegs);
    end(5, sm);
    if (keep_f && opt.keep_copy == 1)
      launch_copy_words(sl.d_fkeep.p, pb.f_chunk, (size_t)stride * W_FP12, sm);
    else if (keep_f)
      HIPCHK(hipMemcpyAsync(sl.d_fkeep.p, pb.f_chunk, (size_t)stride * W_FP12 * 4, hipMemcpyDeviceToDevice, sm));
    const uint32_t* d_franges = reinterpret_cast<uint32_t*>(din + o_franges);
    beg(6, sm);
    const uint32_t* d_ftree = reinterpret_cast<uint32_t*>(din + o_ftree);
    launch_group_tree(pb, d_franges, ng0, d_ftree, n_fruns, d_ftree + 2 * (size_t)n_fruns, f_level_end, sl.d_F.p, sm,
                      &msegs, sl.d_fseg.p);
    end(6, sm);
    HIPCHK(hipEventRecord(sl.join_msg, sm));
    if (spec)
      HIPCHK(hipStreamWaitEvent(s, sl.join_msm, 0));
    else
      launch_sig_msm(pb, d_slices, n_slices, d_rslices, ng0, sl.d_msmB.p, sl.d_msmW.p, sl.d_S.p, s,
                     lane_tail && (opt.lane_tail_parts & 1), msm_tree);
    end(4, s);
    const bool tail_msg = opt.tail_on_msg && !opt.serial && BLSGPU_STREAM_PAIRS;
    hipStream_t sg = s;
    if (spec && opt.spec_gsm && !tail_msg) sg = smsm;
    if (tail_msg) {
      HIPCHK(hipEventRecord(sl.join_gsm, s));
      HIPCHK(hipStreamWaitEvent(sm, sl.join_gsm, 0));
      sg = stl = sm;
    }
    beg(kStages + 1, sg);
    launch_group_sig_miller(sl.d_S.p, ng0, sl.d_G.p, sg, excl && coop,
                            lane_tail && (opt.lane_tail_parts & 2));
    end(kStages + 1, sg);
    HIPCHK(hipEventRecord(sl.join_gsm, sg));
    HIPCHK(hipStreamWaitEvent(stl, sl.join_gsm, 0));
    HIPCHK(hipStreamWaitEvent(stl, sl.join_msg, 0));
    if (rsig_spec) HIPCHK(hipStreamWaitEvent(stl, sl.join_rsig, 0));
    beg(7, stl);
    launch_group_check(sl.d_S.p, sl.d_F.p, ng0, d_ok0, stl, nullptr, 0, sl.d_G.p, excl && coop);
    end(7, stl);
    HIPCHK(hipGetLastError());
    HIPCHK(hipMemcpyAsync(sl.h_res.p, sl.d_res.p, o_ok + ng0, hipMemcpyDeviceToHost, stl));
    HIPCHK(hipEventRecord(sl.done, stl));
  }
  if (opt.early_release && !opt.serial) {
    HIPCHK(hipEventSynchronize(sl.join_msg));
    release_inflight(d, sl);
  }
  HIPCHK(hipEventSynchronize(sl.done));
  if (batch_rand::take_injection(g_fail_run_skip, g_fail_run_count)) throw HipError{hipErrorLaunchFailure};
  release_inflight(d, sl);
  st.groups += ng0;
  st.unique_messages += n_umsg;
  st.pairing_units += merged ? n_units : n;
  st.miller_chunks += n_chunks;
  st.run_sets = n;
  if (prof) {
    for (int k = 0; k < kStages; k++) {
      float ms = 0;
      HIPCHK(hipEventElapsedTime(&ms, sl.ev[2 * k], sl.ev[2 * k + 1]));
      if (k == 5 || k == 7) {
        const int x = k == 5 ? kStages : kStages + 1;
        float ml = 0;
        HIPCHK(hipEventElapsedTime(&ml, sl.ev[2 * x], sl.ev[2 * x + 1]));
        ms += ml;
      }
      st.stage_ms[k] += ms;
    }
  }

  std::vector<int> jr(nj, 0);
  for (uint32_t j = 0; j < nj; j++) {
    const int err = (int8_t)sl.h_res.p[j];
    jr[j] = err ? -err : 2;
  }
  std::vector<uint32_t> retry;
  std::vector<uint32_t> failed_g;
  for (uint32_t g = 0; g < ng0; g++) {
    std::vector<uint32_t> clean;
    bool dropped = false;
    for (uint32_t j = group_jobs[g].first; j < group_jobs[g].second; j++) {
      if (jr[j] == 2)
        clean.push_back(j);
      else if (job_sets(j).second > job_sets(j).first)
        dropped = true;
    }
    if (spec && dropped && !clean.empty()) {
      if (plan && group_batchable[g]) st.batch_retries++;
      if (!plan && clean.size() > 1) st.batch_retries++;
      retry.insert(retry.end(), clean.begin(), clean.end());
      continue;
    }
    if (plan) {
      if (!group_batchable[g]) {
      } else if (clean.size() == group_jobs[g].second - group_jobs[g].first && sl.h_res.p[o_ok + g]) {
        st.batch_sigs_success += job_sets(group_jobs[g].second - 1).second - job_sets(group_jobs[g].first).first;
      } else {
        st.batch_retries++;
      }
    }
    if (clean.empty()) continue;
    if (plan) {
      if (sl.h_res.p[o_ok + g]) {
        for (uint32_t j : clean) jr[j] = 1;
      } else {
        retry.insert(retry.end(), clean.begin(), clean.end());
        failed_g.push_back(g);
      }
      continue;
    }
    if (sl.h_res.p[o_ok + g]) {
      for (uint32_t j : clean) jr[j] = 1;
      if (group_jobs[g].second - group_jobs[g].first > 1)
        for (uint32_t j : clean) st.batch_sigs_success += job_sets(j).second - job_sets(j).first;
    } else {
      if (clean.size() > 1) st.batch_retries++;
      retry.insert(retry.end(), clean.begin(), clean.end());
      failed_g.push_back(g);
    }
  }

  if (!retry.empty()) {
    constexpr uint32_t kFbSub = 16;
    constexpr uint32_t kFbLaneMin = 128;
    const uint32_t nr = (uint32_t)retry.size();
    const hipStream_t sfb = sl.fb ? sl.fb : stl;
    sl.set_stream(sfb);
    std::vector<uint32_t> rfirst{0}, ritems, rr(2 * (size_t)nr), rf(2 * (size_t)nr), rsl, rrs{0}, rset;
    for (uint32_t q = 0; q < nr; q++) {
      const auto js = job_sets(retry[q]);
      rr[2 * q] = js.first;
      rr[2 * q + 1] = js.second;
      add_slices(rsl, rrs, js.first, js.second);
      for (uint32_t i = js.first; i < js.second; i++) rset.push_back(i);
      if (keep_f) {
        rf[2 * q] = js.first;
        rf[2 * q + 1] = js.second;
        continue;
      }
      const auto cr = add_chunks(rfirst, ritems, js.first, js.second, mk_whole);
      rf[2 * q] = cr.first;
      rf[2 * q + 1] = cr.second;
    }
    const bool small_jobs = rset.size() < (size_t)32 * nr;
    constexpr uint32_t kFbDirectMax = 640;
    const bool busy = (!small && !sl.alone) || opt.fb_force_busy;
    auto lane_checks = [&](uint32_t count) { return busy && opt.fb_lane_min > 0 && count >= (uint32_t)opt.fb_lane_min; };
    const bool direct = (small && nr <= kFbDirectMax) || (busy && opt.fb_direct_min > 0 && nr >= (uint32_t)opt.fb_direct_min);
    const uint32_t nsub = !direct && nr >= 2 * kFbSub ? (nr + kFbSub - 1) / kFbSub : 0;
    auto fb_check = [&](const uint32_t* S, const uint32_t* F, uint32_t ng, uint8_t* ok, const uint32_t* sel,
                        uint32_t count) {
      if (lane_checks(count) && opt.fb_check6 == 2) {
        sl.d_lines.ensure((size_t)ng * kMillerLineWords);
        sl.d_fbflags.ensure(ng);
        launch_check6_miller(S, F, ng, ok, sfb, sel, count, sl.d_lines.p, sl.d_fbflags.p);
      } else if (lane_checks(count) && opt.fb_check6) {
        sl.d_G.ensure((size_t)W_FP12 * ng);
        launch_group_sig_miller_sel(S, ng, sel, count, sl.d_G.p, sfb);
        launch_group_check6(F, sl.d_G.p, ng, ok, sfb, sel, count);
      } else {
        launch_group_check(S, F, ng, ok, sfb, sel, count, nullptr, false, lane_checks(count));
      }
    };
    std::vector<uint32_t> subr(2 * (size_t)nsub);
    for (uint32_t t = 0; t < nsub; t++) {
      subr[2 * t] = t * kFbSub;
      subr[2 * t + 1] = std::min(nr, (t + 1) * kFbSub);
    }
    const uint32_t nc = (uint32_t)rfirst.size() - 1;
    const uint32_t nrs = (uint32_t)(rsl.size() / 2);
    const size_t o_rsl = 4 * (size_t)nr + rfirst.size() + ritems.size(), o_rrs = o_rsl + rsl.size(),
                 o_rset = o_rrs + rrs.size(), o_sub = o_rset + rset.size(), o_sel = o_sub + subr.size();
    const size_t words = o_sel + nr;
    sl.h_list.ensure(words);
    sl.d_list.ensure(words);
    uint32_t* hl = sl.h_list.p;
    memcpy(hl, rr.data(), rr.size() * 4);
    memcpy(hl + 2 * (size_t)nr, rf.data(), rf.size() * 4);
    memcpy(hl + 4 * (size_t)nr, rfirst.data(), rfirst.size() * 4);
// ... 541 lines not shown
    {
      std::unique_lock<std::mutex> lk(d->q_mu);
      d->q_cv.wait(lk, [&] {
        return d->stop || sl->retire ||
               (!d->queue.empty() && d->runs_inflight < std::max<int64_t>(1, d->queue.front().call->opt.pipeline_depth));
      });
      if (sl->retire) return;
      if (d->queue.empty()) return;
      parts.push_back(d->queue.front());
      d->queue.pop_front();
      const Call* c0 = parts[0].call;
      uint32_t total = task_sets(parts[0]);
      int64_t cap = c0->opt.merge_sets;
      if (cap > 0 && c0->opt.merge_balance) {
        int64_t backlog = total;
        for (const Task& t : d->queue) backlog += task_sets(t);
        if (backlog > cap) {
          const int64_t runs = (backlog + cap - 1) / cap;
          cap = (backlog + runs - 1) / runs;
        }
      }
      const auto t_start = std::chrono::steady_clock::now();
      const auto deadline = t_start + std::chrono::microseconds(c0->opt.merge_wait_us);
      const auto idle_end = t_start + std::chrono::microseconds(c0->opt.idle_wait_us);
      auto idle_deadline = t_start + std::chrono::microseconds(c0->opt.idle_wait_us / 4);
      for (;;) {
        size_t took = 0;
        while (!d->queue.empty() && cap > 0 && !(c0->ctx->closed)) {
          const Task& nx = d->queue.front();
          const Call* c = nx.call;
          if ((int64_t)(total + task_sets(nx)) > cap || pk_mode(c->b) != pk_mode(c0->b) || !c->opt.same_run(c0->opt))
            break;
          total += task_sets(nx);
          parts.push_back(nx);
          d->queue.pop_front();
          took++;
        }
        const bool room = cap > 0 && (int64_t)total < cap && d->queue.empty();
        if (!room || d->stop || c0->ctx->closed) break;
        if (d->runs_inflight == 0) {
          if (c0->opt.idle_wait_us <= 0) break;
          const auto now = std::chrono::steady_clock::now();
          if (took) idle_deadline = std::min(idle_end, now + std::chrono::microseconds(c0->opt.idle_wait_us / 4));
          if (now >= idle_deadline) break;
          if (d->q_cv.wait_until(lk, idle_deadline) == std::cv_status::timeout && d->queue.empty()) break;
          continue;
        }
        if (d->q_cv.wait_until(lk, deadline) == std::cv_status::timeout && d->queue.empty()) break;
      }
      sl->alone = d->runs_inflight == 0;
      d->runs_inflight++;
      sl->in_flight = true;
    }
    tl_run_t0 = std::chrono::steady_clock::now();
    tl_merge_ms = 0;
    struct InflightGuard {
      Device* d;
      Slot* sl;
      ~InflightGuard() { release_inflight(*d, *sl); }
    } guard{d, sl};
    if (parts.size() == 1) {
      run_task(*d, *sl, parts[0]);
      continue;
    }
    std::vector<int> rcs(parts.size(), BLSGPU_OK);
    try {
      std::shared_lock<std::shared_mutex> tl(d->table_mu);
      run_merged(*d, *sl, parts, rcs);
    } catch (...) {
      for (size_t p = 0; p < parts.size(); p++) {
        const Shard& sh = parts[p].call->shards[parts[p].shard];
        for (uint32_t j = sh.job_begin; j < sh.job_end; j++) parts[p].call->job_result[j] = -BLSGPU_DEVICE_ERROR;
        rcs[p] = BLSGPU_DEVICE_ERROR;
      }
    }
    for (size_t p = 0; p < parts.size(); p++) {
      Call* c = parts[p].call;
      c->rc[parts[p].shard] = rcs[p];
      d->load.fetch_sub(c->shards[parts[p].shard].cost, std::memory_order_relaxed);
      if (c->remaining.fetch_sub(1) == 1) finish_call(c);
    }
  }
}

bool ensure_urgent_streams(Device* d, Slot* sl);
void urgent_loop(Device* d, Slot* sl) {
  tl_dispatcher = true;
  pthread_setname_np(pthread_self(), "blsgpu-urgent");
  (void)hipSetDevice(d->id);
  for (;;) {
    std::vector<Task> parts;
    {
      std::unique_lock<std::mutex> lk(d->q_mu);
      d->q_cv.wait(lk, [&] { return d->stop || !d->uqueue.empty(); });
      if (d->uqueue.empty()) return;
      parts.push_back(d->uqueue.front());
      d->uqueue.pop_front();
      const Call* c0 = parts[0].call;
      uint32_t total = task_sets(parts[0]);
      const auto gap = std::chrono::microseconds(std::max<int64_t>(c0->opt.urgent_wait_us, 0));
      const auto linger_end = std::chrono::steady_clock::now() + 8 * gap;
      for (;;) {
        bool blocked = false;
        while (!d->uqueue.empty()) {
          const Task& nx = d->uqueue.front();
          if ((int64_t)(total + task_sets(nx)) > c0->opt.urgent_max_sets || pk_mode(nx.call->b) != pk_mode(c0->b) ||
              !nx.call->opt.same_run(c0->opt)) {
            blocked = true;
            break;
          }
          total += task_sets(nx);
          parts.push_back(nx);
          d->uqueue.pop_front();
        }
        if (blocked || gap.count() == 0 || d->stop || (int64_t)total >= c0->opt.urgent_max_sets) break;
        const auto now = std::chrono::steady_clock::now();
        if (now >= linger_end) break;
        if (!d->q_cv.wait_for(lk, std::min<std::chrono::steady_clock::duration>(gap, linger_end - now),
                              [&] { return d->stop || !d->uqueue.empty(); }))
          break;
      }
    }
    sl->alone = true;
    tl_run_t0 = std::chrono::steady_clock::now();
    tl_merge_ms = 0;
    const size_t np = parts.size();
    if (!ensure_urgent_streams(d, sl)) {
      for (size_t p = 0; p < np; p++) {
        Call* c = parts[p].call;
        const Shard& sh = c->shards[parts[p].shard];
        for (uint32_t j = sh.job_begin; j < sh.job_end; j++) c->job_result[j] = -BLSGPU_DEVICE_ERROR;
        c->rc[parts[p].shard] = BLSGPU_DEVICE_ERROR;
        c->sst[parts[p].shard].urgent_lane = 1;
        if (c->remaining.fetch_sub(1) == 1) finish_call(c);
      }
      d->upending.fetch_sub((int)np, std::memory_order_relaxed);
      continue;
    }
    if (np == 1) {
      run_task(*d, *sl, parts[0]);
    } else {
      std::vector<int> rcs(np, BLSGPU_OK);
      try {
        std::shared_lock<std::shared_mutex> tl(d->table_mu);
        run_merged(*d, *sl, parts, rcs);
      } catch (...) {
        for (size_t p = 0; p < np; p++) {
          const Shard& sh = parts[p].call->shards[parts[p].shard];
          for (uint32_t j = sh.job_begin; j < sh.job_end; j++) parts[p].call->job_result[j] = -BLSGPU_DEVICE_ERROR;
          rcs[p] = BLSGPU_DEVICE_ERROR;
        }
      }
      for (size_t p = 0; p < np; p++) {
        Call* c = parts[p].call;
        c->rc[parts[p].shard] = rcs[p];
        c->sst[parts[p].shard].urgent_lane = 1;
        if (c->remaining.fetch_sub(1) == 1) finish_call(c);
      }
    }
    d->upending.fetch_sub((int)np, std::memory_order_relaxed);
  }
}

void free_slot(Device* d, Slot* s) {
  (void)hipSetDevice(d->id);
  hipStream_t last = s->d_in.st;
  s->release_all();
  if (last) (void)hipStreamSynchronize(last);
  for (auto& e : s->ev)
    if (e) (void)hipEventDestroy(e);
  for (hipEvent_t e : {s->join_in, s->join_msg, s->join_pk, s->join_mask, s->join_gsm, s->join_dec, s->join_msm,
                       s->join_rsig, s->done})
    if (e) (void)hipEventDestroy(e);
  if (s->fb) (void)hipStreamSynchronize(s->fb), (void)hipStreamDestroy(s->fb);
  delete s;
}

hipStream_t make_stream(const std::vector<uint32_t>& mask, int prio) {
  hipStream_t st = nullptr;
  if (!mask.empty())
    HIPCHK(hipExtStreamCreateWithCUMask(&st, (uint32_t)mask.size(), mask.data()));
  else
    HIPCHK(hipStreamCreateWithPriority(&st, hipStreamNonBlocking, prio));
  return st;
}

void create_streams(blsgpu_ctx* ctx, Device* d) {
  HIPCHK(hipSetDevice(d->id));
  int prio_lo = 0, prio_hi = 0;
  HIPCHK(hipDeviceGetStreamPriorityRange(&prio_lo, &prio_hi));
  int n_cu = 0;
  HIPCHK(hipDeviceGetAttribute(&n_cu, hipDeviceAttributeMultiprocessorCount, d->id));
  const int part = (int)std::min<int64_t>(ctx->urgent_cus, n_cu / 2) & ~7;
  d->urgent_cus = part;
  const size_t words = (size_t)(n_cu + 31) / 32;
  std::vector<uint32_t> pmask(words, 0);
  d->main_mask.clear();
  for (int i = 0; i < n_cu; i++)
    if (part == 0 || i < part) pmask[i / 32] |= 1u << (i % 32);
  if (part > 0 && ctx->urgent_isolate == 1) {
    d->main_mask.assign(words, 0);
    for (int i = part; i < n_cu; i++) d->main_mask[i / 32] |= 1u << (i % 32);
  }
  if (ctx->urgent_isolate == 3) d->main_mask.assign(words, ~0u);
  if (ctx->urgent_isolate == 2) pmask.clear();
  d->npairs = ctx->hw_queues >= 6 ? kMaxPairs : 2;
  for (int k = 0; k < 2 * d->npairs; k++) {
    const bool high = ctx->pipeline_prio && ((BLSGPU_STREAM_PRIO & (1 << (k & 3))) != 0 || (k >= kStreams && (k & 1)));
    d->st[k] = make_stream(d->main_mask, high ? prio_hi : prio_lo);
  }
  d->umask = pmask;
  d->uprio = prio_hi;
#if BLSGPU_URGENT_EAGER
  for (int k = 0; k < 4; k++) d->ust[k] = make_stream(d->umask, d->uprio);
#endif
}

bool ensure_urgent_streams(Device* d, Slot* sl) {
  if (d->ust[0]) return true;
  try {
    HIPCHK(hipSetDevice(d->id));
    for (int k = 0; k < 4; k++) d->ust[k] = make_stream(d->umask, d->uprio);
  } catch (HipError&) {
    for (hipStream_t& st : d->ust)
      if (st) (void)hipStreamDestroy(st), st = nullptr;
    return false;
  }
  sl->set_stream(d->ust[0]);
  return true;
}

void create_slot_events(Device* d, Slot* s) {
  const unsigned wait_flags = hipEventDisableTiming | (d->blocking_sync ? hipEventBlockingSync : 0u);
  for (hipEvent_t* e : {&s->join_in, &s->join_pk, &s->join_mask, &s->join_gsm, &s->join_dec, &s->join_msm, &s->join_rsig})
    HIPCHK(hipEventCreateWithFlags(e, hipEventDisableTiming));
  for (hipEvent_t* e : {&s->join_msg, &s->done}) HIPCHK(hipEventCreateWithFlags(e, wait_flags));
  for (auto& e : s->ev) HIPCHK(hipEventCreate(&e));
}

void add_slot(Device* d) {
  Slot* s = new Slot();
  HIPCHK(hipSetDevice(d->id));
  try {
    s->set_stream(d->st[kSig]);
    create_slot_events(d, s);
    int prio_lo = 0, prio_hi = 0;
    HIPCHK(hipDeviceGetStreamPriorityRange(&prio_lo, &prio_hi));
    s->fb = make_stream(d->main_mask, prio_lo);
  } catch (HipError&) {
    free_slot(d, s);
    throw;
  }
  d->slots.push_back(s);
  d->workers.emplace_back(worker_loop, d, s);
}

void resize_slots(Device* d, int64_t want) {
  std::vector<std::thread> joins;
  std::vector<Slot*> gone;
  {
    std::lock_guard<std::mutex> lk(d->q_mu);
    while ((int64_t)d->slots.size() < want) add_slot(d);
    while ((int64_t)d->slots.size() > want) {
      Slot* s = d->slots.back();
      s->retire = true;
      gone.push_back(s);
      joins.push_back(std::move(d->workers.back()));
      d->slots.pop_back();
      d->workers.pop_back();
    }
  }
  d->q_cv.notify_all();
  for (size_t k = 0; k < joins.size(); k++) {
    try {
      joins[k].join();
      free_slot(d, gone[k]);
    } catch (std::system_error&) {
      joins[k].detach();
    }
  }
}

void destroy_device(Device* d) {
  {
    std::lock_guard<std::mutex> lk(d->q_mu);
    d->stop = true;
  }
  d->q_cv.notify_all();
  for (auto& t : d->workers) t.join();
  if (d->uworker.joinable()) d->uworker.join();
  for (Slot* s : d->slots) free_slot(d, s);
  if (d->uslot) free_slot(d, d->uslot);
  (void)hipSetDevice(d->id);
  for (hipStream_t st : d->st)
    if (st) (void)hipStreamSynchronize(st), (void)hipStreamDestroy(st);
  for (hipStream_t st : d->ust)
    if (st) (void)hipStreamSynchronize(st), (void)hipStreamDestroy(st);
  for (hipStream_t st : d->same_st)
    if (st) (void)hipStreamSynchronize(st), (void)hipStreamDestroy(st);
  for (hipEvent_t e : d->same_ev)
    if (e) (void)hipEventDestroy(e);
  d->helper.release_all();
  d->table.release();
  if (d->table_stream) (void)hipStreamDestroy(d->table_stream);
  delete d;
}

int64_t hw_queues_of_process() {
  const char* v = getenv("GPU_MAX_HW_QUEUES");
  const long q = v ? strtol(v, nullptr, 10) : 0;
  return q > 0 ? q : 4;
}

int64_t default_slots(int64_t) { return 3; }

int ensure_slots(blsgpu_ctx* ctx) {
  std::lock_guard<std::mutex> lk(ctx->slots_mu);
  if (ctx->slots_started) return BLSGPU_OK;
  try {
    for (Device* d : ctx->devs) {
      if (!d->st[0]) {
        d->blocking_sync = ctx->blocking_sync != 0;
        create_streams(ctx, d);
      }
      resize_slots(d, ctx->slots_per_device);
      if (!d->uslot) {
        Slot* u = new Slot();
        u->urgent = true;
        try {
          u->set_stream(d->ust[0]);
          create_slot_events(d, u);
        } catch (HipError&) {
          free_slot(d, u);
          throw;
        }
        d->uslot = u;
        try {
          d->uworker = std::thread(urgent_loop, d, u);
        } catch (std::system_error&) {
          d->uslot = nullptr;
          free_slot(d, u);
          return BLSGPU_DEVICE_ERROR;
        }
      }
    }
  } catch (HipError&) {
    return BLSGPU_DEVICE_ERROR;
  }
  ctx->slots_started = true;
  return BLSGPU_OK;
}

int64_t shard_cost(const blsgpu_batch& b, const Shard& sh) {
  int64_t c = 256 * (int64_t)(sh.set_end - sh.set_begin);
  if (b.set_pk_first) c += b.set_pk_first[sh.set_end] - b.set_pk_first[sh.set_begin];
  return c;
}

bool launch_urgent(blsgpu_ctx* ctx, Call* c) {
  const blsgpu_batch& b = c->b;
  const uint32_t nd = (uint32_t)std::min<int64_t>((int64_t)ctx->devs.size(), c->opt.max_devices);
  if (!c->opt.urgent_lane || (int64_t)b.n_sets > c->opt.urgent_max_sets || nd == 0) return false;
  const uint32_t start = ctx->route_seq.fetch_add(1, std::memory_order_relaxed) % nd;
  uint32_t best = start;
  for (uint32_t k = 1; k < nd; k++) {
    const uint32_t x = (start + k) % nd;
    if (ctx->devs[x]->upending.load(std::memory_order_relaxed) < ctx->devs[best]->upending.load(std::memory_order_relaxed))
      best = x;
  }
  Device* d = ctx->devs[best];
  if (!d->uslot) return false;
  Shard sh{0, b.n_jobs, 0, b.n_sets};
  sh.dev = best;
  sh.cost = 0;
  c->shards.push_back(sh);
  c->sst.assign(1, blsgpu_stats{});
  c->rc.assign(1, BLSGPU_OK);
  c->remaining = 1;
  c->t0 = std::chrono::steady_clock::now();
  d->upending.fetch_add(1, std::memory_order_relaxed);
  {
    std::lock_guard<std::mutex> lk(d->q_mu);
    d->uqueue.push_back({c, 0});
  }
  d->q_cv.notify_all();
  return true;
}

void launch_call(blsgpu_ctx* ctx, Call* c) {
  const blsgpu_batch& b = c->b;
  bool urgent = false;
  if (b.job_flags)
    for (uint32_t j = 0; j < b.n_jobs && !urgent; j++) urgent = (b.job_flags[j] & BLSGPU_JOB_URGENT) != 0;
  if (urgent && launch_urgent(ctx, c)) return;
  const uint32_t nd_all = (uint32_t)std::min<int64_t>((int64_t)ctx->devs.size(), c->opt.max_devices);
  std::vector<int64_t> load(nd_all);
  for (uint32_t d = 0; d < nd_all; d++) load[d] = ctx->devs[d]->load.load(std::memory_order_relaxed);
  std::vector<uint32_t> devs(std::max<uint32_t>(nd_all, 1));
  const uint32_t nd = route_rule(b.n_sets, nd_all, load.data(), c->opt.route_split_sets,
                                 ctx->route_seq.fetch_add(1, std::memory_order_relaxed), devs.data());
  std::vector<uint32_t> parts(nd + 1);
  shard_rule(b.job_first_set, b.set_pk_first, b.n_jobs, nd, parts.data());
  for (uint32_t k = 0; k < nd; k++) {
    Shard sh{parts[k], parts[k + 1], b.n_jobs ? b.job_first_set[parts[k]] : 0,
             b.n_jobs ? b.job_first_set[parts[k + 1]] : 0};
    sh.dev = devs[k];
    sh.cost = shard_cost(b, sh);
    c->shards.push_back(sh);
  }
  c->sst.assign(nd, blsgpu_stats{});
  c->rc.assign(nd, BLSGPU_OK);
  c->remaining = nd;
  c->t0 = std::chrono::steady_clock::now();
  for (uint32_t k = 0; k < nd; k++) {
    Device* d = ctx->devs[c->shards[k].dev];
    d->load.fetch_add(c->shards[k].cost, std::memory_order_relaxed);
    {
      std::lock_guard<std::mutex> lk(d->q_mu);
      if (urgent)
        d->queue.push_front({c, k});
      else
        d->queue.push_back({c, k});
    }
    d->q_cv.notify_all();
  }
}

}
bool blsgpu_rt::resolve_key(uint64_t seed, batch_rand::Key& key, uint64_t& hash_key) {
  if (seed == 0) {
    if (!batch_rand::os_key(key)) return false;
    hash_key = batch_rand::hash_key(key);
  } else {
    key = batch_rand::seed_key(seed);
    hash_key = batch_rand::hash_key(key);
  }
  return true;
}
namespace {

void reject_all(const blsgpu_batch* b, int8_t* job_result, int code) {
  if (job_result)
    for (uint32_t j = 0; j < b->n_jobs; j++) job_result[j] = (int8_t)-code;
}

Options snapshot(blsgpu_ctx* ctx) {
  std::lock_guard<std::mutex> lk(ctx->opt_mu);
  return ctx->opt;
}

}

extern "C" {

int blsgpu_init(const int* devices, int n_devices, blsgpu_ctx** out) {
  if (!out) return BLSGPU_ERR_ARGS;
  *out = nullptr;
  int count = 0;
  if (hipGetDeviceCount(&count) != hipSuccess || count <= 0) return BLSGPU_ERR_NO_DEVICE;
  std::vector<int> ids;
  if (devices && n_devices > 0) {
    for (int i = 0; i < n_devices; i++) {
      if (devices[i] < 0 || devices[i] >= count) return BLSGPU_ERR_ARGS;
      ids.push_back(devices[i]);
    }
  } else {
    for (int i = 0; i < count; i++) ids.push_back(i);
  }
  blsgpu_ctx* ctx = new blsgpu_ctx();
  ctx->hw_queues = hw_queues_of_process();
  ctx->slots_per_device = default_slots(ctx->hw_queues);
  if (const char* v = getenv("BLSGPU_MILLER_SEGMENTS")) {
    const long j = strtol(v, nullptr, 10);
    if (j >= 1 && j <= MILLER_MAX_SEGS) ctx->opt.miller_segments = j;
  }
  try {
    for (int id : ids) {
      Device* d = new Device();
      d->id = id;
      ctx->devs.push_back(d);
      HIPCHK(hipSetDevice(id));
      HIPCHK(hipStreamCreateWithFlags(&d->table_stream, hipStreamNonBlocking));
    }
  } catch (HipError&) {
    blsgpu_destroy(ctx);
    return BLSGPU_ERR_NO_DEVICE;
  }
  *out = ctx;
  return BLSGPU_OK;
}

void blsgpu_destroy(blsgpu_ctx* ctx) {
  if (!ctx) return;
  {
    std::unique_lock<std::mutex> lk(ctx->active_mu);
    ctx->closed = true;
    ctx->active_cv.wait(lk, [&] { return ctx->active == 0; });
  }
  for (Device* d : ctx->devs) destroy_device(d);
  delete ctx;
}

int blsgpu_device_count(const blsgpu_ctx* ctx) { return ctx ? (int)ctx->devs.size() : 0; }

uint32_t blsgpu_pubkeys_count(const blsgpu_ctx* ctx) {
  if (!ctx || ctx->devs.empty()) return 0;
  uint32_t n = UINT32_MAX;
  for (Device* d : ctx->devs) {
    std::shared_lock<std::shared_mutex> lk(d->table_mu);
    n = std::min(n, d->table_n);
  }
  return n;
}

int blsgpu_pubkeys_upload(blsgpu_ctx* ctx, uint32_t first_index, const uint8_t* pk96, uint32_t n) {
  if (!ctx) return BLSGPU_ERR_ARGS;
  if (n == 0) return BLSGPU_OK;
  if (!pk96) return BLSGPU_ERR_ARGS;
  if (!enter(ctx)) return BLSGPU_ERR_CLOSED;
  std::lock_guard<std::mutex> tl(ctx->table_mu);
  int result = BLSGPU_OK;
  for (Device* d : ctx->devs) {
    std::shared_lock<std::shared_mutex> lk(d->table_mu);
    if (first_index > d->table_n) result = BLSGPU_ERR_ARGS;
  }
  auto upload_one = [&](Device* d) -> int {
    try {
      HIPCHK(hipSetDevice(d->id));
      hipStream_t ts = d->table_stream;
      const uint32_t need = first_index + n;
      uint8_t* dpk = nullptr;
      int8_t* dst = nullptr;
      uint32_t* tmp = nullptr;
      HIPCHK(hipMalloc((void**)&dpk, (size_t)n * 96));
      HIPCHK(hipMalloc((void**)&dst, n));
      HIPCHK(hipMalloc((void**)&tmp, (size_t)n * W_PKTAB * 4));
      HIPCHK(hipMemcpyAsync(dpk, pk96, (size_t)n * 96, hipMemcpyHostToDevice, ts));
      launch_pk_table_fill(dpk, n, tmp, dst, ts);
      HIPCHK(hipGetLastError());
      std::vector<int8_t> hst(n);
      HIPCHK(hipMemcpyAsync(hst.data(), dst, n, hipMemcpyDeviceToHost, ts));
      HIPCHK(hipStreamSynchronize(ts));
      int err = 0;
      for (uint32_t i = 0; i < n && !err; i++) err = hst[i];
      if (!err) {
        std::unique_lock<std::shared_mutex> lk(d->table_mu);
        if (need > d->table.cap / W_PKTAB) {
          DevBuf<uint32_t> nt;
          nt.ensure((size_t)std::max<uint32_t>(need, d->table_n + d->table_n / 2) * W_PKTAB);
          if (d->table_n)
            HIPCHK(hipMemcpyAsync(nt.p, d->table.p, (size_t)d->table_n * W_PKTAB * 4, hipMemcpyDeviceToDevice, ts));
          d->table.release();
          d->table = nt;
        }
        HIPCHK(hipMemcpyAsync(d->table.p + (size_t)first_index * W_PKTAB, tmp, (size_t)n * W_PKTAB * 4,
                              hipMemcpyDeviceToDevice, ts));
        HIPCHK(hipStreamSynchronize(ts));
        d->table_n = std::max(d->table_n, need);
      }
      (void)hipFree(dpk);
      (void)hipFree(dst);
      (void)hipFree(tmp);
      return err;
    } catch (HipError&) {
      return BLSGPU_DEVICE_ERROR;
    } catch (std::exception&) {
      return BLSGPU_DEVICE_ERROR;
    }
  };
  if (!result) {
    std::vector<int> rc(ctx->devs.size(), 0);
    if (ctx->devs.size() == 1) {
      rc[0] = upload_one(ctx->devs[0]);
    } else {
      std::vector<std::thread> th;
      for (size_t k = 0; k < ctx->devs.size(); k++) th.emplace_back([&, k] { rc[k] = upload_one(ctx->devs[k]); });
      for (auto& t : th) t.join();
    }
    for (int r : rc)
      if (r && !result) result = r;
  }
  leave(ctx);
  return result;
}

int blsgpu_set_option(blsgpu_ctx* ctx, const char* key, int64_t value) {
  if (!ctx || !key) return BLSGPU_ERR_ARGS;
  std::string k(key);
  if (k == "urgent_cus" || k == "urgent_isolate" || k == "blocking_sync" || k == "pipeline_prio") {
    std::lock_guard<std::mutex> sk(ctx->slots_mu);
    if (ctx->slots_started) return BLSGPU_ERR_ARGS;
    if (k == "blocking_sync" || k == "pipeline_prio") {
      if (value < 0 || value > 1) return BLSGPU_ERR_ARGS;
      (k == "blocking_sync" ? ctx->blocking_sync : ctx->pipeline_prio) = value;
    } else if (k == "urgent_cus") {
      if (value < 0 || value > 128 || (value & 7)) return BLSGPU_ERR_ARGS;
      ctx->urgent_cus = value;
    } else {
      if (value < 0 || value > 3) return BLSGPU_ERR_ARGS;
      ctx->urgent_isolate = value;
    }
    return BLSGPU_OK;
  }
  if (k == "slots") {
    if (value < 1 || value > 64 || tl_dispatcher) return BLSGPU_ERR_ARGS;
    std::lock_guard<std::mutex> sk(ctx->slots_mu);
    ctx->slots_per_device = value;
    if (ctx->slots_started) {
      try {
        for (Device* d : ctx->devs) resize_slots(d, value);
      } catch (HipError&) {
        return BLSGPU_DEVICE_ERROR;
      }
    }
    return BLSGPU_OK;
  }
  std::lock_guard<std::mutex> lk(ctx->opt_mu);
  if (k == "group_sets") {
    if (value < 1) return BLSGPU_ERR_ARGS;
    ctx->opt.group_sets = value;
  } else if (k == "profile") {
    ctx->opt.profile = value != 0;
  } else if (k == "max_devices") {
    if (value < 1) return BLSGPU_ERR_ARGS;
    ctx->opt.max_devices = value;
  } else if (k == "dedupe") {
    ctx->opt.dedupe = value != 0;
  } else if (k == "merge_sets") {
    if (value < 0) return BLSGPU_ERR_ARGS;
    ctx->opt.merge_sets = value;
  } else if (k == "miller_k") {
    if (value < 0 || value > 64) return BLSGPU_ERR_ARGS;
    ctx->opt.miller_k = value;
  } else if (k == "group_policy") {
    if (value < 0 || value > 1) return BLSGPU_ERR_ARGS;
    ctx->opt.group_policy = value;
  } else if (k == "merge_wait_us") {
    if (value < 0 || value > 1000000) return BLSGPU_ERR_ARGS;
    ctx->opt.merge_wait_us = value;
  } else if (k == "idle_wait_us") {
    if (value < 0 || value > 1000000) return BLSGPU_ERR_ARGS;
    ctx->opt.idle_wait_us = value;
  } else if (k == "pipeline_depth") {
    if (value < 1 || value > 64) return BLSGPU_ERR_ARGS;
    ctx->opt.pipeline_depth = value;
  } else if (k == "serial") {
    ctx->opt.serial = value != 0;
  } else if (k == "miller_lanes") {
    if (value < 0 || (value > 3 && value != 6)) return BLSGPU_ERR_ARGS;
    ctx->opt.miller_lanes = value;
  } else if (k == "msm_slice_mid") {
    if (value < 8 || value > MSM_SLICE) return BLSGPU_ERR_ARGS;
    ctx->opt.msm_slice_mid = value;
  } else if (k == "copy_stream") {
    ctx->opt.copy_stream = value != 0;
  } else if (k == "tail_on_msg") {
    ctx->opt.tail_on_msg = value != 0;
  } else if (k == "early_release") {
    ctx->opt.early_release = value != 0;
  } else if (k == "merge_balance") {
    ctx->opt.merge_balance = value != 0;
  } else if (k == "lines_lanes") {
    if (value < 1 || value > 2) return BLSGPU_ERR_ARGS;
    ctx->opt.lines_lanes = value;
  } else if (k == "msm_tree") {
    ctx->opt.msm_tree = value != 0;
  } else if (k == "coop_max") {
    if (value < 0 || value > (1 << 24)) return BLSGPU_ERR_ARGS;
    ctx->opt.coop_max = value;
  } else if (k == "coop_g2_max") {
    if (value < 0 || value > (1 << 24)) return BLSGPU_ERR_ARGS;
    ctx->opt.coop_g2_max = value;
  } else if (k == "coop_excl_max") {
    if (value < 0 || value > (1 << 24)) return BLSGPU_ERR_ARGS;
    ctx->opt.coop_excl_max = value;
  } else if (k == "rsig_spec") {
    ctx->opt.rsig_spec = value != 0;
  } else if (k == "spec_large") {
    ctx->opt.spec_large = value != 0;
  } else if (k == "spec_gsm") {
    ctx->opt.spec_gsm = value != 0;
  } else if (k == "fb_lane_min") {
    if (value < 0) return BLSGPU_ERR_ARGS;
    ctx->opt.fb_lane_min = value;
  } else if (k == "fb_force_busy") {
    ctx->opt.fb_force_busy = value != 0;
  } else if (k == "keep_f") {
    ctx->opt.keep_f = value != 0;
  } else if (k == "keep_copy") {
    ctx->opt.keep_copy = value != 0;
  } else if (k == "urgent_lane") {
    ctx->opt.urgent_lane = value != 0;
  } else if (k == "urgent_max_sets") {
    if (value < 0) return BLSGPU_ERR_ARGS;
    ctx->opt.urgent_max_sets = value;
  } else if (k == "urgent_excl") {
    ctx->opt.urgent_excl = value != 0;
  } else if (k == "group_adapt") {
    ctx->opt.group_adapt = value != 0;
  } else if (k == "urgent_wait_us") {
    if (value < 0 || value > 100000) return BLSGPU_ERR_ARGS;
    ctx->opt.urgent_wait_us = value;
  } else if (k == "fb_check6") {
    if (value < 0 || value > 2) return BLSGPU_ERR_ARGS;
    ctx->opt.fb_check6 = value;
  } else if (k == "fb_direct_min") {
    if (value < 0) return BLSGPU_ERR_ARGS;
    ctx->opt.fb_direct_min = value;
  } else if (k == "small_max") {
    if (value < 0) return BLSGPU_ERR_ARGS;
    ctx->opt.small_max = value;
  } else if (k == "miller_pairs") {
    if (value < 0 || value > 1) return BLSGPU_ERR_ARGS;
    ctx->opt.miller_pairs = value;
  } else if (k == "acc6_max") {
    if (value < 0) return BLSGPU_ERR_ARGS;
    ctx->opt.acc6_max = value;
  } else if (k == "route_split_sets") {
    if (value < 1) return BLSGPU_ERR_ARGS;
    ctx->opt.route_split_sets = value;
  } else if (k == "lane_tail_parts") {
    if (value < 0 || value > 3) return BLSGPU_ERR_ARGS;
    ctx->opt.lane_tail_parts = value;
  } else if (k == "lane_tail_min") {
    if (value < 0) return BLSGPU_ERR_ARGS;
    ctx->opt.lane_tail_min = value;
  } else if (k == "f_run_max") {
    if (value < 1 || value > 1024 || (value & (value - 1))) return BLSGPU_ERR_ARGS;
    ctx->opt.f_run_max = value;
  } else {
    return BLSGPU_ERR_ARGS;
  }
  return BLSGPU_OK;
}

int blsgpu_get_option(const blsgpu_ctx* cctx, const char* key, int64_t* value) {
  if (!cctx || !key || !value) return BLSGPU_ERR_ARGS;
  blsgpu_ctx* ctx = const_cast<blsgpu_ctx*>(cctx);
  const std::string k(key);
  if (k == "slots") {
    std::lock_guard<std::mutex> sk(ctx->slots_mu);
    if (ctx->slots_started && !ctx->devs.empty()) {
      std::lock_guard<std::mutex> lk(ctx->devs[0]->q_mu);
      *value = (int64_t)ctx->devs[0]->slots.size();
    } else {
      *value = ctx->slots_per_device;
    }
    return BLSGPU_OK;
  }
  if (k == "hw_queues") {
    *value = ctx->hw_queues;
    return BLSGPU_OK;
  }
  if (k == "blocking_sync" || k == "pipeline_prio") {
    std::lock_guard<std::mutex> sk(ctx->slots_mu);
    *value = k == "blocking_sync" ? ctx->blocking_sync : ctx->pipeline_prio;
    return BLSGPU_OK;
  }
  if (k == "urgent_cus" || k == "urgent_isolate") {
    std::lock_guard<std::mutex> sk(ctx->slots_mu);
    if (k == "urgent_cus")
      *value = ctx->slots_started && !ctx->devs.empty() ? ctx->devs[0]->urgent_cus : ctx->urgent_cus;
    else
      *value = ctx->urgent_isolate;
    return BLSGPU_OK;
  }
  if (k == "abi_version") {
    *value = BLSGPU_ABI_VERSION;
    return BLSGPU_OK;
  }
  if (k == "spurious_groups") {
    uint64_t c = 0;
    for (const Device* d : ctx->devs) c += d->spurious_groups.load(std::memory_order_relaxed);
    *value = (int64_t)c;
    return BLSGPU_OK;
  }
  std::lock_guard<std::mutex> lk(ctx->opt_mu);
  const Options& o = ctx->opt;
  if (k == "group_sets") *value = o.group_sets;
  else if (k == "profile") *value = o.profile;
  else if (k == "max_devices") *value = o.max_devices;
  else if (k == "dedupe") *value = o.dedupe;
  else if (k == "merge_sets") *value = o.merge_sets;
  else if (k == "miller_k") *value = o.miller_k;
  else if (k == "group_policy") *value = o.group_policy;
  else if (k == "merge_wait_us") *value = o.merge_wait_us;
  else if (k == "idle_wait_us") *value = o.idle_wait_us;
  else if (k == "pipeline_depth") *value = o.pipeline_depth;
  else if (k == "serial") *value = o.serial;
  else if (k == "miller_lanes") *value = o.miller_lanes;
  else if (k == "f_run_max") *value = o.f_run_max;
  else if (k == "lane_tail_min") *value = o.lane_tail_min;
  else if (k == "lane_tail_parts") *value = o.lane_tail_parts;
  else if (k == "msm_slice_mid") *value = o.msm_slice_mid;
  else if (k == "msm_tree") *value = o.msm_tree;
  else if (k == "lines_lanes") *value = o.lines_lanes;
  else if (k == "merge_balance") *value = o.merge_balance;
  else if (k == "early_release") *value = o.early_release;
  else if (k == "tail_on_msg") *value = o.tail_on_msg;
  else if (k == "copy_stream") *value = o.copy_stream;
  else if (k == "coop_max") *value = o.coop_max;
  else if (k == "coop_g2_max") *value = o.coop_g2_max;
  else if (k == "coop_excl_max") *value = o.coop_excl_max;
  else if (k == "rsig_spec") *value = o.rsig_spec;
  else if (k == "spec_large") *value = o.spec_large;
  else if (k == "spec_gsm") *value = o.spec_gsm;
  else if (k == "fb_lane_min") *value = o.fb_lane_min;
  else if (k == "route_split_sets") *value = o.route_split_sets;
  else if (k == "acc6_max") *value = o.acc6_max;
  else if (k == "miller_pairs") *value = o.miller_pairs;
  else if (k == "small_max") *value = o.small_max;
  else if (k == "fb_direct_min") *value = o.fb_direct_min;
  else if (k == "fb_check6") *value = o.fb_check6;
  else if (k == "fb_force_busy") *value = o.fb_force_busy;
  else if (k == "keep_f") *value = o.keep_f;
  else if (k == "keep_copy") *value = o.keep_copy;
  else if (k == "urgent_lane") *value = o.urgent_lane;
  else if (k == "urgent_max_sets") *value = o.urgent_max_sets;
  else if (k == "urgent_excl") *value = o.urgent_excl;
  else if (k == "urgent_wait_us") *value = o.urgent_wait_us;
  else if (k == "group_adapt") *value = o.group_adapt;
  else return BLSGPU_ERR_ARGS;
  return BLSGPU_OK;
}

int blsgpu_chunkify(uint32_t len, uint32_t min_per_chunk, uint32_t* chunk_first, uint32_t* n_chunks) {
  if (!chunk_first || !n_chunks || min_per_chunk == 0) return BLSGPU_ERR_ARGS;
  const uint32_t per = chunk_size(len, min_per_chunk);
  uint32_t c = 0;
  if (len / min_per_chunk <= 1) chunk_first[c++] = 0;
  else
    for (uint32_t i = 0; i < len; i += per) chunk_first[c++] = i;
  chunk_first[c] = len;
  *n_chunks = c;
  return BLSGPU_OK;
}

int blsgpu_verify(blsgpu_ctx* ctx, const blsgpu_batch* b, int8_t* job_result, blsgpu_stats* stats) {
  if (!ctx) return BLSGPU_ERR_ARGS;
  int v = validate_batch(b);
  if (v) return v;
  if (b->n_jobs && !job_result) return BLSGPU_ERR_ARGS;
  if (!enter(ctx)) return BLSGPU_ERR_CLOSED;
  Call c;
  c.ctx = ctx;
  c.b = *b;
  c.job_result = job_result;
  c.stats = stats;
  if (!resolve_key(b->seed, c.key, c.seed)) {
    reject_all(b, job_result, BLSGPU_DEVICE_ERROR);
    leave(ctx);
    return BLSGPU_ERR_ENTROPY;
  }
  c.max_index = max_table_index(b);
  c.opt = snapshot(ctx);
  c.sync = true;
  if (b->n_jobs == 0) {
    if (stats) *stats = blsgpu_stats{};
    leave(ctx);
    return BLSGPU_OK;
  }
// ... 147 lines not shown
```

### lodestar_amd/csrc/runtime_internal.hpp

```cpp
#pragma once
#include <hip/hip_runtime.h>
#include <stdint.h>
#include <stdlib.h>
#include <string.h>

#include <algorithm>
#include <atomic>
#include <chrono>
#include <condition_variable>
#include <deque>
#include <mutex>
#include <shared_mutex>
#include <thread>
#include <vector>

#include "../../include/blsgpu.h"
#include "batch_rand.hpp"
#include "kernels.h"

namespace blsgpu_rt __attribute__((visibility("hidden"))) {

struct HipError {
  hipError_t e;
};
#define HIPCHK(x)                             \
  do {                                        \
    hipError_t _e = (x);                      \
    if (_e != hipSuccess) throw HipError{_e}; \
  } while (0)

inline thread_local uint64_t tl_async_grow = 0;
inline bool poison_buffers() {
  static const bool on = [] {
    const char* v = getenv("BLSGPU_POISON");
    return v && v[0] == '1';
  }();
  return on;
}
inline bool sync_grow() {
  static const bool on = [] {
    const char* v = getenv("BLSGPU_SYNC_GROW");
    return v && v[0] == '1';
  }();
  return on;
}
inline std::mutex g_grow_mu;
inline bool grow_unlocked() {
  static const bool on = [] {
    const char* v = getenv("BLSGPU_GROW_UNLOCKED");
    return v && v[0] == '1';
  }();
  return on;
}
inline bool fb_verify() {
  static const bool on = [] {
    const char* v = getenv("BLSGPU_FB_VERIFY");
    return v && v[0] == '1';
  }();
  return on;
}
inline bool grow_free() {
  static const bool on = [] {
    const char* v = getenv("BLSGPU_GROW_FREE");
    return v && v[0] == '1';
  }();
  return on;
}
template <class T>
struct DevBuf {
  T* p = nullptr;
  size_t cap = 0;
  hipStream_t st = nullptr;
  std::vector<T*> retired;
  void ensure(size_t n) {
    if (n <= cap) return;
    std::unique_lock<std::mutex> lk(g_grow_mu, std::defer_lock);
    if (!grow_unlocked()) lk.lock();
    const size_t c = std::max<size_t>(n, cap * 2);
    if (st && sync_grow()) {
      HIPCHK(hipDeviceSynchronize());
      if (p) HIPCHK(hipFree(p));
      p = nullptr;
      HIPCHK(hipMalloc((void**)&p, c * sizeof(T)));
      if (poison_buffers()) HIPCHK(hipMemset(p, 0xA5, c * sizeof(T)));
      HIPCHK(hipDeviceSynchronize());
      tl_async_grow++;
    } else if (st) {
      if (p && grow_free()) HIPCHK(hipFreeAsync(p, st));
      else if (p) retired.push_back(p);
      p = nullptr;
      HIPCHK(hipMallocAsync((void**)&p, c * sizeof(T), st));
      if (poison_buffers()) HIPCHK(hipMemsetAsync(p, 0xA5, c * sizeof(T), st));
      tl_async_grow++;
    } else {
      if (p) HIPCHK(hipFree(p));
      p = nullptr;
      HIPCHK(hipMalloc((void**)&p, c * sizeof(T)));
      if (poison_buffers()) {
        HIPCHK(hipMemset(p, 0xA5, c * sizeof(T)));
        HIPCHK(hipStreamSynchronize(nullptr));
      }
    }
    cap = c;
  }
  void release() {
    std::unique_lock<std::mutex> lk(g_grow_mu, std::defer_lock);
    if (!grow_unlocked()) lk.lock();
    if (p) (void)(st ? hipFreeAsync(p, st) : hipFree(p));
    for (T* q : retired) (void)(st ? hipFreeAsync(q, st) : hipFree(q));
    retired.clear();
    p = nullptr;
    cap = 0;
  }
};

template <class T>
struct HostBuf {
  T* p = nullptr;
  size_t cap = 0;
  void ensure(size_t n) {
    if (n <= cap) return;
    std::unique_lock<std::mutex> lk(g_grow_mu, std::defer_lock);
    if (!grow_unlocked()) lk.lock();
    if (p) HIPCHK(hipHostFree(p));
    p = nullptr;
    size_t c = std::max<size_t>(n, cap * 2);
    HIPCHK(hipHostMalloc((void**)&p, c * sizeof(T), hipHostMallocDefault));
    if (poison_buffers()) memset(p, 0x5A, c * sizeof(T));
    cap = c;
  }
  void release() {
    if (p) (void)hipHostFree(p);
    p = nullptr;
    cap = 0;
  }
};

constexpr int kStages = 8;
constexpr size_t kMillerLineWords = (size_t)MILLER_STEPS * W_LINE;

inline size_t al256(size_t x) { return (x + 255) & ~(size_t)255; }

struct Slot {
  hipEvent_t join_in = nullptr, join_msg = nullptr, join_pk = nullptr, join_mask = nullptr, join_gsm = nullptr,
             join_dec = nullptr, join_msm = nullptr, join_rsig = nullptr, done = nullptr;
  hipEvent_t ev[2 * (kStages + 2)] = {};
  DevBuf<uint8_t> d_in, d_res, d_bytes, d_ok, d_fbflags;
  DevBuf<uint32_t> d_work, d_lines, d_S, d_F, d_G, d_list, d_msmB, d_msmW, d_fb;
  DevBuf<uint32_t> d_fkeep;
  DevBuf<uint32_t> d_fseg;
  HostBuf<uint8_t> h_in, h_res, h_ok;
  HostBuf<uint32_t> h_list;
  hipStream_t fb = nullptr;
  bool retire = false;
  bool in_flight = false;
  bool alone = false;
  bool urgent = false;

  void set_stream(hipStream_t st) {
    for (auto* b : {&d_in, &d_res, &d_bytes, &d_ok, &d_fbflags}) b->st = st;
    for (auto* b : {&d_work, &d_lines, &d_S, &d_F, &d_G, &d_list, &d_msmB, &d_msmW, &d_fb, &d_fkeep, &d_fseg}) b->st = st;
  }
  void release_all() {
    d_in.release(); d_res.release(); d_bytes.release(); d_ok.release(); d_fbflags.release();
    d_work.release(); d_lines.release(); d_S.release(); d_F.release(); d_list.release();
    d_msmB.release(); d_msmW.release(); d_fb.release(); d_G.release(); d_fkeep.release(); d_fseg.release();
    h_in.release(); h_res.release(); h_ok.release(); h_list.release();
  }
};

struct Call;
struct Task {
  Call* call;
  uint32_t shard;
};

enum { kSig = 0, kMsg = 1, kPk = 2, kTail = 3, kStreams = 4, kMaxPairs = 3 };
#ifndef BLSGPU_STREAM_PRIO
#define BLSGPU_STREAM_PRIO ((1 << kMsg) | (1 << kTail))
#endif
#ifndef BLSGPU_STREAM_PAIRS
#define BLSGPU_STREAM_PAIRS 1
#endif


struct Device {
  int id = 0;
  hipStream_t table_stream = nullptr;
  hipStream_t st[2 * kMaxPairs] = {};
  int npairs = 2;
  std::mutex enq_mu;
  std::mutex helper_mu;
  Slot helper;
  hipStream_t same_st[2] = {};
  hipEvent_t same_ev[3] = {};
  std::shared_mutex table_mu;
  DevBuf<uint32_t> table;
  uint32_t table_n = 0;
  std::mutex q_mu;
  std::condition_variable q_cv;
  std::deque<Task> queue;
  bool stop = false;
  std::vector<Slot*> slots;
  std::vector<std::thread> workers;
  int runs_inflight = 0;
  std::atomic<uint32_t> run_seq{0};
  std::atomic<int64_t> load{0};
  hipStream_t ust[4] = {};
  std::vector<uint32_t> umask;
  int uprio = 0;
  std::deque<Task> uqueue;
  Slot* uslot = nullptr;
  std::thread uworker;
  std::atomic<int> upending{0};
  std::atomic<uint64_t> spurious_groups{0};
  int urgent_cus = 0;
  std::vector<uint32_t> main_mask;
  bool blocking_sync = true;
  std::mutex fail_mu;
  double fail_rate = 0;
};

struct Options {
  int64_t group_sets = 1024;
  int64_t max_devices = 64;
  bool profile = false;
  bool dedupe = true;
  int64_t miller_k = 0;
  int64_t merge_sets = 131072;
  int64_t merge_wait_us = 2000;
  int64_t idle_wait_us = 0;
  int64_t pipeline_depth = 3;
  int64_t group_policy = 0;
  bool serial = false;
  int64_t miller_segments = 0;
  int64_t miller_lanes = 0;
  int64_t f_run_max = 16;
  int64_t lane_tail_min = 0;
  int64_t lane_tail_parts = 3;
  int64_t msm_slice_mid = 32;
  int64_t lines_lanes = 2;
  int64_t merge_balance = 0;
  int64_t early_release = 0;
  int64_t tail_on_msg = 0;
  int64_t copy_stream = 0;
  int64_t msm_tree = 1;
  int64_t coop_max = 512;
  int64_t coop_g2_max = 4096;
  int64_t coop_excl_max = 512;
  int64_t rsig_spec = 1;
  int64_t spec_large = 1;
  int64_t spec_gsm = 0;
  int64_t fb_lane_min = 256;
  int64_t route_split_sets = 16384;
  int64_t acc6_max = 16384;
  int64_t miller_pairs = 0;
  int64_t small_max = 4096;
  int64_t fb_direct_min = 1024;
  int64_t fb_check6 = 2;
  int64_t keep_f = 1;
  int64_t keep_copy = 0;
  int64_t fb_force_busy = 0;
  int64_t urgent_lane = 1;
  int64_t urgent_max_sets = 512;
  int64_t urgent_excl = 0;
  int64_t urgent_wait_us = 300;
  int64_t group_adapt = 1;
  bool same_run(const struct Options& o) const {
    return group_sets == o.group_sets && profile == o.profile && dedupe == o.dedupe && miller_k == o.miller_k &&
           group_policy == o.group_policy && serial == o.serial && miller_lanes == o.miller_lanes && miller_segments == o.miller_segments &&
           f_run_max == o.f_run_max && lane_tail_min == o.lane_tail_min &&
           lane_tail_parts == o.lane_tail_parts &&
           msm_slice_mid == o.msm_slice_mid && msm_tree == o.msm_tree &&
           lines_lanes == o.lines_lanes && merge_balance == o.merge_balance && early_release == o.early_release && tail_on_msg == o.tail_on_msg && copy_stream == o.copy_stream && coop_max == o.coop_max &&
           coop_g2_max == o.coop_g2_max && coop_excl_max == o.coop_excl_max && rsig_spec == o.rsig_spec && spec_large == o.spec_large && spec_gsm == o.spec_gsm &&
           fb_lane_min == o.fb_lane_min && acc6_max == o.acc6_max && miller_pairs == o.miller_pairs && small_max == o.small_max &&
           fb_direct_min == o.fb_direct_min && fb_check6 == o.fb_check6 && fb_force_busy == o.fb_force_busy &&
           group_adapt == o.group_adapt && keep_f == o.keep_f && keep_copy == o.keep_copy;
  }
};

struct MsgIndex {
  std::vector<uint32_t> slot;
  uint64_t key;
  explicit MsgIndex(uint32_t n, uint64_t k) : key(k) {
    size_t cap = 16;
    while (cap < (size_t)n * 2) cap <<= 1;
    slot.assign(cap, 0);
  }
  static uint64_t mix(uint64_t z) {
    z = (z ^ (z >> 30)) * 0xBF58476D1CE4E5B9ull;
    z = (z ^ (z >> 27)) * 0x94D049BB133111EBull;
    return z ^ (z >> 31);
  }
  size_t hash(const uint8_t* msgs, uint32_t i) const {
    uint64_t w[4];
    memcpy(w, msgs + (size_t)i * 32, 32);
    return (size_t)(mix(w[0] ^ key) ^ mix(w[1] + key) ^ w[2] ^ (w[3] << 1)) & (slot.size() - 1);
  }
  uint32_t find_or_add(const uint8_t* msgs, uint32_t i, std::vector<uint32_t>& uniq) {
    return find_or_add_h(msgs, i, hash(msgs, i), uniq);
  }
  uint32_t find_or_add_h(const uint8_t* msgs, uint32_t i, size_t h, std::vector<uint32_t>& uniq) {
    const size_t mask = slot.size() - 1;
    for (;;) {
      const uint32_t s = slot[h];
      if (!s) {
        uniq.push_back(i);
        slot[h] = (uint32_t)uniq.size();
        return (uint32_t)uniq.size() - 1;
      }
      if (memcmp(msgs + (size_t)uniq[s - 1] * 32, msgs + (size_t)i * 32, 32) == 0) return s - 1;
      h = (h + 1) & mask;
    }
  }
};

inline double ms_since(std::chrono::steady_clock::time_point t) {
  return std::chrono::duration<double, std::milli>(std::chrono::steady_clock::now() - t).count();
}

bool resolve_key(uint64_t seed, batch_rand::Key& key, uint64_t& hash_key);

}

struct blsgpu_ctx {
  std::vector<blsgpu_rt::Device*> devs;
  std::atomic<bool> closed{false};
  std::mutex active_mu;
  std::condition_variable active_cv;
  int active = 0;
  std::mutex table_mu;
  std::mutex opt_mu;
  blsgpu_rt::Options opt;
  int64_t slots_per_device = 2;
  int64_t hw_queues = 4;
  std::mutex slots_mu;
  bool slots_started = false;
  std::atomic<uint32_t> route_seq{0};
  int64_t urgent_cus = 0;
  int64_t urgent_isolate = 1;
  int64_t blocking_sync = 1;
  int64_t pipeline_prio = 1;
};

namespace blsgpu_rt __attribute__((visibility("hidden"))) {
inline bool enter(blsgpu_ctx* ctx) {
  std::lock_guard<std::mutex> lk(ctx->active_mu);
  if (ctx->closed) return false;
  ctx->active++;
  return true;
}
inline void leave(blsgpu_ctx* ctx) {
  {
    std::lock_guard<std::mutex> lk(ctx->active_mu);
    ctx->active--;
  }
  ctx->active_cv.notify_all();
}
}
```

### lodestar_amd/native.py

```python
import ctypes
import os

import numpy as np

PKG = os.path.dirname(os.path.abspath(__file__))
LIB_PATH = os.environ.get("BLSGPU_LIB") or os.path.join(PKG, "libblsgpu.so")

OK = 0
BAD_ENCODING = 1
POINT_NOT_ON_CURVE = 2
POINT_NOT_IN_GROUP = 3
PK_IS_INFINITY = 6
INVALID_SIZE = 8
EMPTY_AGGREGATE = 9
EMPTY_SET = 10
DEVICE_ERROR = 11
ERR_ARGS = 100
ERR_NO_DEVICE = 101
ERR_CLOSED = 102
ERR_ENTROPY = 103
JOB_BATCHABLE = 1
JOB_URGENT = 2
AGG_VALIDATE = 1
AGG_MAX_SIGS = 1 << 20
INJECT_ENTROPY = 1
INJECT_DEVICE = 2

EXPORTED_SYMBOLS = [
    "blsgpu_init",
    "blsgpu_destroy",
    "blsgpu_device_count",
    "blsgpu_pubkeys_upload",
    "blsgpu_pubkeys_count",
    "blsgpu_verify",
    "blsgpu_submit",
    "blsgpu_set_option",
    "blsgpu_code_name",
    "blsgpu_debug_op",
    "blsgpu_aggregate_pubkeys",
    "blsgpu_key_validate",
    "blsgpu_signing_roots",
    "blsgpu_shard_jobs",
    "blsgpu_get_option",
    "blsgpu_chunkify",
    "blsgpu_batch_scalars",
    "blsgpu_debug_inject",
    "blsgpu_route_call",
    "blsgpu_aggregate_signatures",
    "blsgpu_sig_agg_lanes",
    "blsgpu_randomness_words",
    "blsgpu_aggregate_with_randomness",
    "blsgpu_awr_lanes",
    "blsgpu_verify_same_message",
    "blsgpu_same_message_form",
]
SAME_LANE_FORMS = 1
ROOT_OBJECT = 0
ROOT_ATTESTATION_DATA = 1


class Batch(ctypes.Structure):
    _fields_ = [
        ("n_sets", ctypes.c_uint32),
        ("n_jobs", ctypes.c_uint32),
        ("job_first_set", ctypes.c_void_p),
        ("job_flags", ctypes.c_void_p),
        ("pk_bytes", ctypes.c_void_p),
        ("set_pk_first", ctypes.c_void_p),
        ("pk_index", ctypes.c_void_p),
        ("msgs", ctypes.c_void_p),
        ("sigs", ctypes.c_void_p),
        ("sig_len", ctypes.c_void_p),
        ("sig_stride", ctypes.c_uint32),
        ("seed", ctypes.c_uint64),
    ]


class Stats(ctypes.Structure):
    _fields_ = [
        ("groups", ctypes.c_uint32),
        ("batch_retries", ctypes.c_uint32),
        ("batch_sigs_success", ctypes.c_uint32),
        ("devices_used", ctypes.c_uint32),
        ("device_ms", ctypes.c_double),
        ("stage_ms", ctypes.c_double * 8),
        ("unique_messages", ctypes.c_uint32),
        ("pairing_units", ctypes.c_uint32),
        ("miller_chunks", ctypes.c_uint32),
        ("run_sets", ctypes.c_uint32),
        ("run_calls", ctypes.c_uint32),
        ("fallback_jobs", ctypes.c_uint32),
        ("fallback_miller", ctypes.c_uint32),
        ("urgent_lane", ctypes.c_uint32),
        ("host_ms", ctypes.c_double),
    ]


class SameMessageStats(ctypes.Structure):
    _fields_ = [
        ("groups_accepted", ctypes.c_uint32),
        ("groups_retried", ctypes.c_uint32),
        ("retry_sets", ctypes.c_uint32),
        ("unique_messages", ctypes.c_uint32),
        ("form", ctypes.c_uint32),
        ("device_ms", ctypes.c_double),
    ]


STAGES = ["sig_decode", "hash_to_g2", "pk_aggregate", "pk_finish", "sig_msm", "miller_sets",
          "group_reduce", "group_check"]
KERNEL_OF_STAGE = ["k_sig_decode+k_sig_subgroup2+k_sig_subgroup_coop",
                   "k_hash_prep+k_batch_inv+k_hash_map+k_hash_clear+k_hash_clear2+k_hash_clear_coop+k_h_affine",
                   "k_pk_aggregate+k_pk_aggregate_g", "k_pk_finish+k_batch_inv+k_pk_affine",
                   "k_job_mask+k_msm_bucket+k_msm_bucket2+k_msm_slice_pairs+k_msm_slice_pairs2+k_msm_window+k_msm_window2"
                   "+k_msm_horner+k_msm_horner_lane",
                   "k_miller_lines+k_miller_lines2+k_miller_acc+k_miller_acc2+k_miller_acc6+k_miller_accx+k_miller_coop",
                   "k_f_runs+k_f_pairs+k_f_gather", "k_group_sig_miller+k_group_check"]


DONE_CB = ctypes.CFUNCTYPE(None, ctypes.c_void_p, ctypes.c_int)

_lib = None


def load():
    global _lib
    if _lib is not None:
        return _lib
    if not os.path.exists(LIB_PATH):
        raise RuntimeError(
            f"{LIB_PATH} is missing: build it with `python -m lodestar_amd.build` (hipcc, gfx950). "
            "There is no CPU verification path."
        )
    lib = ctypes.CDLL(LIB_PATH)
    lib.blsgpu_init.argtypes = [ctypes.POINTER(ctypes.c_int), ctypes.c_int, ctypes.POINTER(ctypes.c_void_p)]
    lib.blsgpu_init.restype = ctypes.c_int
    lib.blsgpu_destroy.argtypes = [ctypes.c_void_p]
    lib.blsgpu_destroy.restype = None
    lib.blsgpu_device_count.argtypes = [ctypes.c_void_p]
    lib.blsgpu_device_count.restype = ctypes.c_int
    lib.blsgpu_pubkeys_upload.argtypes = [ctypes.c_void_p, ctypes.c_uint32, ctypes.c_char_p, ctypes.c_uint32]
    lib.blsgpu_pubkeys_upload.restype = ctypes.c_int
    lib.blsgpu_pubkeys_count.argtypes = [ctypes.c_void_p]
    lib.blsgpu_pubkeys_count.restype = ctypes.c_uint32
    lib.blsgpu_verify.argtypes = [ctypes.c_void_p, ctypes.POINTER(Batch), ctypes.c_void_p, ctypes.POINTER(Stats)]
    lib.blsgpu_verify.restype = ctypes.c_int
    lib.blsgpu_submit.argtypes = [ctypes.c_void_p, ctypes.POINTER(Batch), ctypes.c_void_p, ctypes.POINTER(Stats),
                                  DONE_CB, ctypes.c_void_p]
    lib.blsgpu_submit.restype = ctypes.c_int
    lib.blsgpu_set_option.argtypes = [ctypes.c_void_p, ctypes.c_char_p, ctypes.c_int64]
    lib.blsgpu_set_option.restype = ctypes.c_int
    lib.blsgpu_code_name.argtypes = [ctypes.c_int]
    lib.blsgpu_code_name.restype = ctypes.c_char_p
    lib.blsgpu_debug_op.argtypes = [ctypes.c_void_p, ctypes.c_int, ctypes.c_uint32, ctypes.c_void_p, ctypes.c_uint32,
                                    ctypes.c_void_p, ctypes.c_uint32, ctypes.c_void_p]
    lib.blsgpu_debug_op.restype = ctypes.c_int
    vp, u32 = ctypes.c_void_p, ctypes.c_uint32
    lib.blsgpu_aggregate_pubkeys.argtypes = [vp, ctypes.POINTER(Batch), vp, u32, vp]
    lib.blsgpu_key_validate.argtypes = [vp, u32, vp, u32, u32, vp, vp]
    lib.blsgpu_signing_roots.argtypes = [vp, ctypes.c_int, u32, vp, u32, vp, u32, vp]
    lib.blsgpu_shard_jobs.argtypes = [vp, vp, u32, u32, vp]
    lib.blsgpu_get_option.argtypes = [vp, ctypes.c_char_p, ctypes.POINTER(ctypes.c_int64)]
    lib.blsgpu_chunkify.argtypes = [u32, u32, vp, vp]
    lib.blsgpu_batch_scalars.argtypes = [ctypes.POINTER(Batch), vp]
    lib.blsgpu_batch_scalars.restype = ctypes.c_int
    lib.blsgpu_debug_inject.argtypes = [ctypes.c_int, ctypes.c_int64, ctypes.c_int64]
    lib.blsgpu_debug_inject.restype = ctypes.c_int
    lib.blsgpu_route_call.argtypes = [u32, u32, vp, ctypes.c_int64, u32, vp, vp]
    lib.blsgpu_route_call.restype = ctypes.c_int
    lib.blsgpu_aggregate_signatures.argtypes = [vp, u32, vp, vp, u32, vp, u32, vp, u32, vp, vp]
    lib.blsgpu_aggregate_signatures.restype = ctypes.c_int
    lib.blsgpu_sig_agg_lanes.argtypes = [u32, u32]
    lib.blsgpu_sig_agg_lanes.restype = u32
    lib.blsgpu_randomness_words.argtypes = [u32, ctypes.c_uint64, vp]
    lib.blsgpu_randomness_words.restype = ctypes.c_int
    lib.blsgpu_aggregate_with_randomness.argtypes = [vp, u32, vp, vp, vp, vp, u32, vp, ctypes.c_uint64, vp, u32, vp,
                                                     u32, vp, vp]
    lib.blsgpu_aggregate_with_randomness.restype = ctypes.c_int
    lib.blsgpu_awr_lanes.argtypes = [u32, u32]
    lib.blsgpu_awr_lanes.restype = u32
    lib.blsgpu_verify_same_message.argtypes = [vp, u32, vp, vp, vp, vp, vp, u32, vp, ctypes.c_uint64, u32, vp, vp, vp]
    lib.blsgpu_verify_same_message.restype = ctypes.c_int
    lib.blsgpu_same_message_form.argtypes = [u32, u32]
    lib.blsgpu_same_message_form.restype = u32
    _lib = lib
    return lib


def code_name(code: int) -> str:
    n = load().blsgpu_code_name(code)
    return n.decode() if n else f"BLSGPU_{code}"


def shard_jobs(job_first_set, n_parts, set_pk_first=None):
    jfs = np.ascontiguousarray(job_first_set, dtype=np.uint32)
    spf = None if set_pk_first is None else np.ascontiguousarray(set_pk_first, dtype=np.uint32)
    out = np.zeros(n_parts + 1, np.uint32)
    rc = load().blsgpu_shard_jobs(jfs.ctypes.data, None if spf is None else spf.ctypes.data, len(jfs) - 1, n_parts,
                                  out.ctypes.data)
    if rc != OK:
        raise ValueError(f"blsgpu_shard_jobs -> {code_name(rc)}")
    return [(int(out[k]), int(out[k + 1])) for k in range(n_parts)]


def route_call(n_sets, device_load, split_sets=16384, start=0):
    dl = np.ascontiguousarray(device_load, dtype=np.int64)
    out = np.zeros(max(len(dl), 1), np.uint32)
    k = ctypes.c_uint32(0)
    rc = load().blsgpu_route_call(n_sets, len(dl), dl.ctypes.data, split_sets, start, out.ctypes.data,
                                  ctypes.addressof(k))
    if rc != OK:
        raise ValueError(f"blsgpu_route_call -> {code_name(rc)}")
    return [int(x) for x in out[: k.value]]


def sig_agg_lanes(n_groups, n_sigs):
    return int(load().blsgpu_sig_agg_lanes(n_groups, n_sigs))


def aggregate_layout(sigs, group_first, sig_len=None, sig_stride=None, out_len=96):
    gf = np.ascontiguousarray(group_first, dtype=np.int64)
    if gf.ndim != 1 or len(gf) == 0:
        raise ValueError("group_first needs n_groups + 1 >= 1 entries")
    if gf[0] != 0 or (np.diff(gf) < 0).any():
        raise ValueError("group_first must start at 0 and never decrease")
    n = int(gf[-1])
    if n > AGG_MAX_SIGS:
        raise ValueError(f"at most {AGG_MAX_SIGS} signatures per call")
    if out_len not in (96, 192):
        raise ValueError("out_len must be 96 or 192")
    buf = _u8(sigs)
    if sig_stride is None:
        sig_stride = (len(buf) // n) if n else 96
    if sig_stride < 96:
        raise ValueError("sig_stride must be at least 96")
    if len(buf) < n * sig_stride:
        raise ValueError(f"{n} signatures of stride {sig_stride} need {n * sig_stride} bytes, got {len(buf)}")
    sl = np.full(n, sig_stride if sig_stride in (96, 192) else 96, np.uint32) if sig_len is None else \
        np.ascontiguousarray(sig_len, dtype=np.uint32)
    if sl.ndim != 1 or len(sl) != n:
        raise ValueError(f"sig_len needs one entry per signature ({n})")
    if sig_stride < 192 and (sl == 192).any():
        raise ValueError("a 192-byte signature needs sig_stride >= 192")
    return buf, gf.astype(np.uint32), sl, int(sig_stride)


def awr_lanes(n_groups, n_sets):
    return int(load().blsgpu_awr_lanes(n_groups, n_sets))


def same_message_form(n_items, flags=0):
    return int(load().blsgpu_same_message_form(n_items, flags))


def randomness_words(n, seed):
    out = np.zeros(max(n, 1), np.uint64)
    rc = load().blsgpu_randomness_words(n, seed, out.ctypes.data)
    if rc != OK:
        raise RuntimeError(f"blsgpu_randomness_words -> {code_name(rc)}")
    return out[:n]


def awr_layout(group_first, sigs, pk_bytes=None, pk_index=None, sig_len=None, sig_stride=None, out_pk_len=96,
               out_sig_len=192):
    if out_pk_len not in (48, 96):
        raise ValueError("out_pk_len must be 48 or 96")
    buf, gf, sl, stride = aggregate_layout(sigs, group_first, sig_len, sig_stride, out_sig_len)
    n = int(gf[-1])
    if (pk_bytes is None) == (pk_index is None):
        raise ValueError("exactly one of pk_bytes and pk_index")
    pkb = pki = None
    if pk_bytes is not None:
        pkb = _u8(pk_bytes)
        if len(pkb) != 96 * n:
            raise ValueError(f"{n} sets need {96 * n} pubkey bytes, got {len(pkb)}")
    else:
        idx = np.ascontiguousarray(pk_index, dtype=np.int64)
        if idx.ndim != 1 or len(idx) != n:
            raise ValueError(f"pk_index needs one entry per set ({n})")
        if n and (idx.min() < 0 or idx.max() > 0xFFFFFFFF):
            raise ValueError("pk_index entries must be table indices")
        pki = idx.astype(np.uint32)
    return gf, buf, sl, stride, pkb, pki


def chunkify(length, min_per_chunk):
    out = np.zeros(length // max(min_per_chunk, 1) + 2, np.uint32)
    nc = ctypes.c_uint32(0)
    rc = load().blsgpu_chunkify(length, min_per_chunk, out.ctypes.data, ctypes.addressof(nc))
    if rc != OK:
        raise ValueError(f"blsgpu_chunkify -> {code_name(rc)}")
    return [list(range(int(out[k]), int(out[k + 1]))) for k in range(nc.value)]


def batch_scalars(job_first_set, job_flags=None, seed=0):
    jfs = np.ascontiguousarray(job_first_set, dtype=np.uint32)
    if len(jfs) == 0:
        raise ValueError("job_first_set needs n_jobs + 1 >= 1 entries")
    n = int(jfs[-1])
    b = Batch()
    b.n_sets = n
    b.n_jobs = len(jfs) - 1
    b.job_first_set = jfs.ctypes.data
    keep = [jfs]
    if job_flags is not None:
        fl = np.ascontiguousarray(job_flags, dtype=np.uint8)
        keep.append(fl)
        b.job_flags = fl.ctypes.data
    b.seed = seed
    out = np.zeros(max(n, 1), np.uint64)
    rc = load().blsgpu_batch_scalars(ctypes.byref(b), out.ctypes.data)
    if rc != OK:
        raise RuntimeError(f"blsgpu_batch_scalars -> {code_name(rc)}")
    return out[:n]


def debug_inject(what, skip=0, count=1):
    rc = load().blsgpu_debug_inject(what, skip, count)
    if rc != OK:
        raise ValueError(f"blsgpu_debug_inject -> {code_name(rc)}")


def _u8(b):
    return np.frombuffer(bytes(b), dtype=np.uint8) if not isinstance(b, np.ndarray) else np.ascontiguousarray(b)


def make_batch(job_first_set, sigs, sig_len, msgs, pk_bytes=None, set_pk_first=None, pk_index=None,
               job_flags=None, sig_stride=None, seed=0x4C4F444553544152):
    job_first_set = np.ascontiguousarray(job_first_set, dtype=np.uint32)
    sig_len = np.ascontiguousarray(sig_len, dtype=np.uint32)
    n_sets = len(sig_len)
    sigs, msgs = _u8(sigs), _u8(msgs)
    if sig_stride is None:
        sig_stride = (len(sigs) // n_sets) if n_sets else 96
    keep = [job_first_set, sig_len, sigs, msgs]
    b = Batch()
    b.n_sets = n_sets
    b.n_jobs = len(job_first_set) - 1
    b.job_first_set = job_first_set.ctypes.data
    if job_flags is not None:
        job_flags = np.ascontiguousarray(job_flags, dtype=np.uint8)
        keep.append(job_flags)
        b.job_flags = job_flags.ctypes.data
    if pk_bytes is not None:
        pk = _u8(pk_bytes)
        if len(pk) == 0:
            pk = np.zeros(1, np.uint8)
        keep.append(pk)
        b.pk_bytes = pk.ctypes.data
    if set_pk_first is not None:
        set_pk_first = np.ascontiguousarray(set_pk_first, dtype=np.uint32)
        keep.append(set_pk_first)
        b.set_pk_first = set_pk_first.ctypes.data
    if pk_index is not None:
        pk_index = np.ascontiguousarray(pk_index, dtype=np.uint32)
        keep.append(pk_index)
        b.pk_index = pk_index.ctypes.data if len(pk_index) else set_pk_first.ctypes.data
    b.msgs = msgs.ctypes.data if len(msgs) else 0
    b.sigs = sigs.ctypes.data if len(sigs) else 0
    b.sig_len = sig_len.ctypes.data if len(sig_len) else 0
    b.sig_stride = sig_stride
    b.seed = seed
    return b, keep


class Pending:

    status = None
    t_done = None

    def wait(self, timeout=None):
        if not self.ev.wait(timeout):
            raise TimeoutError("blsgpu_submit: call not completed")
        if self.status != OK:
            raise RuntimeError(f"blsgpu_submit -> {code_name(self.status)}")
        return self.res[: self.n_jobs], self.st


class Context:

    def __init__(self, devices=None):
        lib = load()
        self._lib = lib
        h = ctypes.c_void_p()
        if devices:
            arr = (ctypes.c_int * len(devices))(*devices)
            rc = lib.blsgpu_init(arr, len(devices), ctypes.byref(h))
        else:
            rc = lib.blsgpu_init(None, 0, ctypes.byref(h))
        if rc != OK:
            raise RuntimeError(f"blsgpu_init failed: {code_name(rc)} (no usable MI355X?)")
        self.h = h

    def close(self):
        if self.h:
            self._lib.blsgpu_destroy(self.h)
            self.h = None

    def __del__(self):
        try:
            self.close()
        except Exception:
            pass

    @property
    def device_count(self):
        return self._lib.blsgpu_device_count(self.h)

    def set_option(self, key: str, value: int):
        rc = self._lib.blsgpu_set_option(self.h, key.encode(), int(value))
        if rc != OK:
            raise ValueError(f"blsgpu_set_option({key}) -> {code_name(rc)}")

    def get_option(self, key: str) -> int:
        v = ctypes.c_int64(0)
        rc = self._lib.blsgpu_get_option(self.h, key.encode(), ctypes.byref(v))
        if rc != OK:
            raise ValueError(f"blsgpu_get_option({key}) -> {code_name(rc)}")
        return v.value

    def upload_pubkeys(self, first_index: int, pk96: bytes):
        n = len(pk96) // 96
        rc = self._lib.blsgpu_pubkeys_upload(self.h, first_index, pk96, n)
        if rc != OK:
            raise ValueError(f"blsgpu_pubkeys_upload -> {code_name(rc)}")

    @property
    def pubkeys_count(self):
        return self._lib.blsgpu_pubkeys_count(self.h)

    def verify_raw(self, job_first_set, sigs, sig_len, msgs, pk_bytes=None, set_pk_first=None, pk_index=None,
                   job_flags=None, sig_stride=None, seed=0x4C4F444553544152):
        b, keep = make_batch(job_first_set, sigs, sig_len, msgs, pk_bytes, set_pk_first, pk_index, job_flags,
                             sig_stride, seed)
        res = np.zeros(max(b.n_jobs, 1), dtype=np.int8)
        st = Stats()
        rc = self._lib.blsgpu_verify(self.h, ctypes.byref(b), res.ctypes.data, ctypes.byref(st))
        if rc != OK:
            raise RuntimeError(f"blsgpu_verify -> {code_name(rc)}")
        return res[: b.n_jobs], st

    def submit_raw(self, job_first_set, sigs, sig_len, msgs, pk_bytes=None, set_pk_first=None, pk_index=None,
                   job_flags=None, sig_stride=None, seed=0x4C4F444553544152):
        import threading

        b, keep = make_batch(job_first_set, sigs, sig_len, msgs, pk_bytes, set_pk_first, pk_index, job_flags,
                             sig_stride, seed)
        p = Pending()
        p.res = np.zeros(max(b.n_jobs, 1), dtype=np.int8)
        p.n_jobs = b.n_jobs
        p.st = Stats()
        p.ev = threading.Event()

        def done(user, status):
            p.status = status
            p.t_done = __import__("time").perf_counter()
            p.ev.set()

        p.cb = DONE_CB(done)
        rc = self._lib.blsgpu_submit(self.h, ctypes.byref(b), p.res.ctypes.data, ctypes.byref(p.st), p.cb, None)
        if rc != OK:
            raise RuntimeError(f"blsgpu_submit -> {code_name(rc)}")
        return p

    def aggregate_pubkeys(self, pk_bytes=None, set_pk_first=None, pk_index=None, out_len=96):
        n = (len(set_pk_first) - 1) if set_pk_first is not None else len(pk_bytes) // 96
        b, keep = make_batch(np.array([0, n]), b"", np.zeros(n, np.uint32), b"", pk_bytes, set_pk_first, pk_index)
        out = np.zeros(max(n, 1) * out_len, np.uint8)
        st = np.zeros(max(n, 1), np.int8)
        rc = self._lib.blsgpu_aggregate_pubkeys(self.h, ctypes.byref(b), out.ctypes.data, out_len, st.ctypes.data)
        if rc != OK:
            raise RuntimeError(f"blsgpu_aggregate_pubkeys -> {code_name(rc)}")
        return [out[out_len * i: out_len * (i + 1)].tobytes() for i in range(n)], st[:n]

    def aggregate_signatures(self, sigs, group_first, sig_len=None, sig_stride=None, validate=True, out_len=96):
        buf, gf, sl, stride = aggregate_layout(sigs, group_first, sig_len, sig_stride, out_len)
        n = len(gf) - 1
        if len(buf) == 0:
            buf = np.zeros(1, np.uint8)
        if len(sl) == 0:
            sl = np.zeros(1, np.uint32)
        out = np.zeros(max(n, 1) * out_len, np.uint8)
        st = np.zeros(max(n, 1), np.int8)
        fb = np.full(max(n, 1), 0xFFFFFFFF, np.uint32)
        rc = self._lib.blsgpu_aggregate_signatures(self.h, n, gf.ctypes.data, buf.ctypes.data, stride, sl.ctypes.data,
                                                   AGG_VALIDATE if validate else 0, out.ctypes.data, out_len,
                                                   st.ctypes.data, fb.ctypes.data)
        if rc != OK:
            raise RuntimeError(f"blsgpu_aggregate_signatures -> {code_name(rc)}")
        return [out[out_len * i: out_len * (i + 1)].tobytes() for i in range(n)], st[:n], fb[:n]

    def aggregate_with_randomness(self, group_first, sigs, pk_bytes=None, pk_index=None, sig_len=None,
                                  sig_stride=None, seed=0, out_pk_len=96, out_sig_len=192):
        gf, buf, sl, stride, pkb, pki = awr_layout(group_first, sigs, pk_bytes, pk_index, sig_len, sig_stride,
                                                   out_pk_len, out_sig_len)
        n = len(gf) - 1
        if len(buf) == 0:
            buf = np.zeros(1, np.uint8)
        if len(sl) == 0:
            sl = np.zeros(1, np.uint32)
        if pkb is not None and len(pkb) == 0:
            pkb = np.zeros(1, np.uint8)
        if pki is not None and len(pki) == 0:
            pki = np.zeros(1, np.uint32)
        opk = np.zeros(max(n, 1) * out_pk_len, np.uint8)
        osig = np.zeros(max(n, 1) * out_sig_len, np.uint8)
        st = np.zeros(max(n, 1), np.int8)
        fb = np.full(max(n, 1), 0xFFFFFFFF, np.uint32)
        rc = self._lib.blsgpu_aggregate_with_randomness(
            self.h, n, gf.ctypes.data, None if pkb is None else pkb.ctypes.data,
            None if pki is None else pki.ctypes.data, buf.ctypes.data, stride, sl.ctypes.data, seed, opk.ctypes.data,
            out_pk_len, osig.ctypes.data, out_sig_len, st.ctypes.data, fb.ctypes.data)
        if rc != OK:
            raise RuntimeError(f"blsgpu_aggregate_with_randomness -> {code_name(rc)}")
        return ([opk[out_pk_len * i: out_pk_len * (i + 1)].tobytes() for i in range(n)],
                [osig[out_sig_len * i: out_sig_len * (i + 1)].tobytes() for i in range(n)], st[:n], fb[:n])

    def verify_same_message(self, group_first, msgs, sigs, pk_bytes=None, pk_index=None, sig_len=None,
                            sig_stride=None, seed=0, flags=0):
        gf, buf, sl, stride, pkb, pki = awr_layout(group_first, sigs, pk_bytes, pk_index, sig_len, sig_stride)
        n_groups = len(gf) - 1
        n = int(gf[-1])
        m = _u8(msgs)
        if len(m) != 32 * n_groups:
            raise ValueError(f"{n_groups} groups need {32 * n_groups} message bytes, got {len(m)}")
        if len(m) == 0:
            m = np.zeros(1, np.uint8)
        if len(buf) == 0:
            buf = np.zeros(1, np.uint8)
        if len(sl) == 0:
            sl = np.zeros(1, np.uint32)
        if pkb is not None and len(pkb) == 0:
            pkb = np.zeros(1, np.uint8)
        if pki is not None and len(pki) == 0:
            pki = np.zeros(1, np.uint32)
        res = np.zeros(max(n, 1), np.int8)
        gres = np.zeros(max(n_groups, 1), np.int8)
        st = SameMessageStats()
        rc = self._lib.blsgpu_verify_same_message(
            self.h, n_groups, gf.ctypes.data, m.ctypes.data, None if pkb is None else pkb.ctypes.data,
            None if pki is None else pki.ctypes.data, buf.ctypes.data, stride, sl.ctypes.data, seed, flags,
            res.ctypes.data, gres.ctypes.data, ctypes.byref(st))
        if rc != OK:
            raise RuntimeError(f"blsgpu_verify_same_message -> {code_name(rc)}")
        return res[:n], gres[:n_groups], st

    def key_validate(self, pks: bytes, pk_len: int):
        n = len(pks) // pk_len
        src = _u8(pks)
        out = np.zeros(max(n, 1) * 96, np.uint8)
        st = np.zeros(max(n, 1), np.int8)
        rc = self._lib.blsgpu_key_validate(self.h, n, src.ctypes.data, pk_len, pk_len, out.ctypes.data, st.ctypes.data)
        if rc != OK:
            raise RuntimeError(f"blsgpu_key_validate -> {code_name(rc)}")
        return out[: 96 * n].tobytes(), st[:n]

    def signing_roots(self, kind: int, objects: bytes, domains: bytes):
        obj_len = 32 if kind == ROOT_OBJECT else 128
        n = len(objects) // obj_len
        o, d = _u8(objects), _u8(domains)
        dstride = 0 if len(domains) == 32 else 32
        out = np.zeros(max(n, 1) * 32, np.uint8)
        rc = self._lib.blsgpu_signing_roots(self.h, kind, n, o.ctypes.data, obj_len, d.ctypes.data, dstride,
                                            out.ctypes.data)
        if rc != OK:
            raise RuntimeError(f"blsgpu_signing_roots -> {code_name(rc)}")
        return [out[32 * i: 32 * i + 32].tobytes() for i in range(n)]

    def debug_op(self, op: int, inputs: bytes, in_stride: int, out_stride: int):
        n = len(inputs) // in_stride
        inb = np.frombuffer(inputs, dtype=np.uint8).copy()
        out = np.zeros(n * out_stride, dtype=np.uint8)
        st = np.zeros(n, dtype=np.int32)
        rc = self._lib.blsgpu_debug_op(self.h, op, n, inb.ctypes.data, in_stride, out.ctypes.data, out_stride,
                                       st.ctypes.data)
        if rc != OK:
            raise RuntimeError(f"blsgpu_debug_op -> {code_name(rc)}")
        return out.tobytes(), st
```

Measured before the change: 4.272 million sets/s.

## Precompute per-pubkey comb tables for fixed-base 64-bit scalar multiplication

New measurement: 4.192 million sets/s. 0.981x the previous value.

```diff
diff --git a/include/blsgpu.h b/include/blsgpu.h
--- a/include/blsgpu.h
+++ b/include/blsgpu.h
@@ -72,6 +72,7 @@
 
 int blsgpu_pubkeys_upload(blsgpu_ctx* ctx, uint32_t first_index, const uint8_t* pk96, uint32_t n);
 uint32_t blsgpu_pubkeys_count(const blsgpu_ctx* ctx);
+uint64_t blsgpu_pubkeys_comb_bytes(const blsgpu_ctx* ctx);
 
 int blsgpu_verify(blsgpu_ctx* ctx, const blsgpu_batch* batch, int8_t* job_result, blsgpu_stats* stats);
 
diff --git a/lodestar_amd/build.py b/lodestar_amd/build.py
--- a/lodestar_amd/build.py
+++ b/lodestar_amd/build.py
@@ -10,7 +10,7 @@
 LIB = os.environ.get("BLSGPU_LIB") or os.path.join(PKG, "libblsgpu.so")
 ARCH = os.environ.get("BLSGPU_ARCH", "gfx950")
 HIPCC = os.environ.get("HIPCC", "/opt/rocm/bin/hipcc")
-SOURCES = ["k_sig.hip", "k_msm.hip", "k_hash.hip", "k_hmap.hip", "k_pk.hip", "k_sigagg.hip", "k_awr.hip", "k_same.hip", "k_miller.hip", "k_group.hip", "k_inv.hip", "k_ssz.hip", "k_debug.hip",
+SOURCES = ["k_sig.hip", "k_msm.hip", "k_hash.hip", "k_hmap.hip", "k_pk.hip", "k_pkcomb.hip", "k_sigagg.hip", "k_awr.hip", "k_same.hip", "k_miller.hip", "k_group.hip", "k_inv.hip", "k_ssz.hip", "k_debug.hip",
            "runtime.cpp", "helpers.cpp"]
 
 
@@ -58,7 +58,7 @@
 def _tu_deps(src):
     if src.endswith(".cpp"):
         return [os.path.join(CSRC, f) for f in (src, "kernels.h", "batch_rand.hpp", "runtime_internal.hpp",
-                                                "helper_layout.hpp", "miller_plan.hpp")] + [
+                                                "helper_layout.hpp", "miller_plan.hpp", "pk_comb_host.hpp")] + [
             os.path.join(ROOT, "include", "blsgpu.h")]
     return [os.path.join(CSRC, src)] + _headers()
 
diff --git a/lodestar_amd/csrc/helpers.cpp b/lodestar_amd/csrc/helpers.cpp
--- a/lodestar_amd/csrc/helpers.cpp
+++ b/lodestar_amd/csrc/helpers.cpp
@@ -113,6 +113,70 @@
   ab.err_k = reinterpret_cast<uint32_t*>(bytes + l.b_ek);
   ab.err_c = reinterpret_cast<int8_t*>(bytes + l.b_ec);
   return ab;
+}
+
+int debug_pk_comb(blsgpu_ctx* ctx, uint32_t n, const uint8_t* in, uint32_t in_stride, uint8_t* out, uint32_t out_stride,
+                  int32_t* status) {
+  return helper_call(ctx, true, [&](Device& d, Slot&, hipStream_t s) -> int {
+    if (!pk_comb::usable(ctx->opt.pk_comb != 0, d.comb.p, d.comb_n, d.table_n)) return BLSGPU_ERR_ARGS;
+    const size_t o_first = n, o_list = o_first + n + 1, o_words = (o_list + n + 1) & ~(size_t)1, words_total = o_words + 2 * (size_t)n;
+    std::vector<uint32_t> h(words_total);
+    uint32_t n_comb = 0;
+    auto has_table = [&](uint32_t idx) {
+      return !std::binary_search(d.comb_flagged.begin(), d.comb_flagged.end(), idx);
+    };
+    for (uint32_t i = 0; i < n; i++) {
+      uint32_t idx;
+      uint64_t w;
+      memcpy(&idx, in + (size_t)i * in_stride, 4);
+      memcpy(&w, in + (size_t)i * in_stride + 4, 8);
+      if (idx >= d.table_n) return BLSGPU_ERR_ARGS;
+      h[i] = idx;
+      h[o_first + i] = i;
+      memcpy(&h[o_words + 2 * (size_t)i], &w, 8);
+      n_comb += has_table(idx);
+    }
+    h[o_first + n] = n;
+    for (uint32_t i = 0, c = 0, r = n_comb; i < n; i++) h[o_list + (has_table(h[i]) ? c++ : r++)] = i;
+    struct Temp {
+      void* p = nullptr;
+      ~Temp() {
+        if (p) (void)hipFree(p);
+      }
+    } din, dwork, dbytes, dout, dst;
+    HIPCHK(hipMalloc(&din.p, words_total * 4));
+    HIPCHK(hipMalloc(&dwork.p, (size_t)n * 9 * W_G1J * 4));
+    HIPCHK(hipMalloc(&dbytes.p, (size_t)n * 3));
+    HIPCHK(hipMalloc(&dout.p, (size_t)n * out_stride));
+    HIPCHK(hipMalloc(&dst.p, (size_t)n * 4));
+    HIPCHK(hipMemcpyAsync(din.p, h.data(), words_total * 4, hipMemcpyHostToDevice, s));
+    HIPCHK(hipMemsetAsync(dbytes.p, 0, (size_t)n * 3, s));
+    HIPCHK(hipMemsetAsync(dout.p, 0, (size_t)n * out_stride, s));
+    uint32_t* const w = static_cast<uint32_t*>(din.p);
+    PipelineBuffers pb{};
+    pb.n = n;
+    pb.pk_index = w;
+    pb.set_pk_first = w + o_first;
+    pb.pk_table = d.table.p;
+    pb.pk_table_n = d.table_n;
+    pb.pk_direct1 = 1;
+    pb.pk_comb = d.comb.p;
+    pb.comb_sets = w + o_list;
+    pb.n_comb = n_comb;
+    pb.rest_sets = w + o_list + n_comb;
+    pb.n_rest = n - n_comb;
+    pb.scalars = reinterpret_cast<const uint64_t*>(w + o_words);
+    pb.pk_jac = static_cast<uint32_t*>(dwork.p);
+    pb.scal_tab = pb.pk_jac + (size_t)n * W_G1J;
+    pb.status = static_cast<int8_t*>(dbytes.p);
+    launch_pk_finish(pb, n, s);
+    launch_pk_comb_out(pb, n, static_cast<uint8_t*>(dout.p), out_stride, static_cast<int32_t*>(dst.p), s);
+    HIPCHK(hipGetLastError());
+    HIPCHK(hipMemcpyAsync(out, dout.p, (size_t)n * out_stride, hipMemcpyDeviceToHost, s));
+    HIPCHK(hipMemcpyAsync(status, dst.p, (size_t)n * 4, hipMemcpyDeviceToHost, s));
+    HIPCHK(hipStreamSynchronize(s));
+    return BLSGPU_OK;
+  });
 }
 
 }
@@ -503,12 +567,14 @@
   };
   static const OpSize kOpSizes[] = {{0, 96, 48},    {1, 194, 192},  {2, 32, 192},   {3, 288, 576},  {4, 576, 576},
                                     {5, 104, 96},   {6, 200, 192},  {7, 64, 96},    {8, 32, 96},    {9, 200, 2880},
-                                    {10, 104, 1440}, {11, 840, 56}, {16, 576, 576}, {17, 288, 576}, {18, 384, 192}};
+                                    {10, 104, 1440}, {11, 840, 56}, {16, 576, 576}, {17, 288, 576}, {18, 384, 192},
+                                    {19, 12, 96}};
   const OpSize* sz = nullptr;
   for (const OpSize& o : kOpSizes)
     if (o.op == op) sz = &o;
   if (!sz || in_stride < sz->in || out_stride < sz->out) return BLSGPU_ERR_ARGS;
   if (n == 0) return BLSGPU_OK;
+  if (op == 19) return debug_pk_comb(ctx, n, in, in_stride, out, out_stride, status);
   return helper_call(ctx, false, [&](Device& d, Slot& sl, hipStream_t s) -> int {
     struct Temp {
       void* p = nullptr;
diff --git a/lodestar_amd/csrc/k_pk.hip b/lodestar_amd/csrc/k_pk.hip
--- a/lodestar_amd/csrc/k_pk.hip
+++ b/lodestar_amd/csrc/k_pk.hip
@@ -188,9 +188,11 @@
   return jac_is_inf(P) ? BLS_PK_IS_INFINITY : BLS_OK;
 }
 
-STAGE_KERNEL_W(BLSGPU_WPE_PK) void k_pk_finish(PipelineBuffers b, uint32_t n_sets, int8_t* pk_status) {
+STAGE_KERNEL_W(BLSGPU_WPE_PK) void k_pk_finish(PipelineBuffers b, uint32_t n_sets, int8_t* pk_status,
+                                               const uint32_t* list) {
   uint32_t i = blockIdx.x * WAVE + threadIdx.x;
   if (i >= n_sets) return;
+  if (list) i = list[i];
   g1j P;
   int st = set_pubkey(b, i, P);
   g1j R = jac_infinity<fp>();
@@ -305,7 +307,13 @@
     hipLaunchKernelGGL(k_pk_aggregate_g<8>, dim3((n * 8 + WAVE - 1) / WAVE), dim3(WAVE), 0, s, b, n);
 }
 void launch_pk_finish(const PipelineBuffers& b, uint32_t n, hipStream_t s) {
-  if (n) hipLaunchKernelGGL(k_pk_finish, grid_for(n), dim3(WAVE), 0, s, b, n, b.status + b.n);
+  if (!b.pk_comb) {
+    if (n) hipLaunchKernelGGL(k_pk_finish, grid_for(n), dim3(WAVE), 0, s, b, n, b.status + b.n, (const uint32_t*)nullptr);
+    return;
+  }
+  launch_pk_comb(b, b.n_comb, s);
+  if (b.n_rest)
+    hipLaunchKernelGGL(k_pk_finish, grid_for(b.n_rest), dim3(WAVE), 0, s, b, b.n_rest, b.status + b.n, b.rest_sets);
 }
 void launch_unit_aggregate(const PipelineBuffers& b, hipStream_t s) {
   if (b.n_units) hipLaunchKernelGGL(k_unit_aggregate, grid_for(b.n_units), dim3(WAVE), 0, s, b);
diff --git a/lodestar_amd/csrc/k_pkcomb.hip b/lodestar_amd/csrc/k_pkcomb.hip
--- /dev/null
+++ b/lodestar_amd/csrc/k_pkcomb.hip
@@ -0,0 +1,104 @@
+#include "k_common.hpp"
+#include "pk_comb.hpp"
+
+typedef pk_comb::Comb<PK_COMB_T> Comb;
+static_assert(PK_COMB_ENTRIES == Comb::kEntries, "kernels.h restates the entries per key");
+
+#define PK_COMB_FLAG_WORD (2 * BLS_NL)
+
+STAGE_KERNEL_W(2) void k_pk_comb(PipelineBuffers b, uint32_t n_list, int8_t* pk_status) {
+  const uint32_t t = blockIdx.x * WAVE + threadIdx.x;
+  if (t >= n_list) return;
+  const uint32_t i = b.comb_sets ? b.comb_sets[t] : t;
+  const uint32_t idx = b.pk_index[b.set_pk_first[i]];
+  g1j R = jac_infinity<fp>();
+  int st = BLS_OK;
+  if (idx >= b.pk_table_n) {
+    st = BLS_DEVICE_ERROR;
+  } else {
+    const uint64_t w = b.scalars[i];
+    const uint32_t* key = b.pk_comb + (size_t)idx * (Comb::kEntries * W_PKTAB);
+    if (w == 0)
+      R = jac_from_aff(ld_pktab(b.pk_table, idx));
+    else if (key[PK_COMB_FLAG_WORD])
+      st = BLS_DEVICE_ERROR;
+    else
+      R = pk_comb::eval<PK_COMB_T>(w, [&](int e) { return ld_pktab(key, (uint32_t)e); });
+  }
+  st_g1j(b.pk_jac, b.n, i, R);
+  pk_status[i] = (int8_t)st;
+}
+
+__global__ __launch_bounds__(WAVE) void k_pk_comb_build(const uint32_t* keys, uint32_t n, uint32_t* jac) {
+  const uint32_t i = blockIdx.x * WAVE + threadIdx.x;
+  if (i >= n) return;
+  const uint32_t stride = n * Comb::kEntries;
+  pk_comb::build<PK_COMB_T>(ld_pktab(keys, i), [&](int e, const g1j& p) { st_g1j(jac, stride, (uint32_t)e * n + i, p); });
+}
+
+__global__ __launch_bounds__(WAVE) void k_pk_comb_write(const uint32_t* jac, const uint32_t* inv, uint32_t n,
+                                                        uint32_t* dst, uint8_t* flag) {
+  const uint32_t i = blockIdx.x * WAVE + threadIdx.x;
+  if (i >= n) return;
+  const uint32_t stride = n * Comb::kEntries;
+  bool finite = true;
+#pragma unroll 1
+  for (int e = 0; e < Comb::kEntries; e++)
+    finite = finite && !fp_is_zero(ld_fp(jac, stride, (uint32_t)e * n + i, 2 * W_FP));
+  flag[i] = finite ? 0 : 1;
+#pragma unroll 1
+  for (int e = 0; e < Comb::kEntries; e++) {
+    const uint32_t m = (uint32_t)e * n + i;
+    g1a a;
+    a.x = fp_zero();
+    a.y = fp_zero();
+    if (finite) {
+      const g1j p = ld_g1j(jac, stride, m);
+      const fp zi = ld_fp(inv, stride, m, 0);
+      const fp zi2 = fp_sqr(zi);
+      a.x = fp_mul(p.x, zi2);
+      a.y = fp_mul(p.y, fp_mul(zi2, zi));
+    }
+    uint32_t* o = dst + ((size_t)i * Comb::kEntries + e) * W_PKTAB;
+    for (int l = 0; l < BLS_NL; l++) {
+      o[l] = a.x.l[l];
+      o[BLS_NL + l] = a.y.l[l];
+    }
+    o[PK_COMB_FLAG_WORD] = finite ? 0u : 1u;
+    o[PK_COMB_FLAG_WORD + 1] = 0;
+    o[PK_COMB_FLAG_WORD + 2] = 0;
+    o[PK_COMB_FLAG_WORD + 3] = 0;
+  }
+}
+
+__global__ __launch_bounds__(WAVE) void k_pk_comb_out(PipelineBuffers b, uint32_t n, const int8_t* pk_status, uint8_t* out,
+                                                      uint32_t out_stride, int32_t* status) {
+  const uint32_t i = blockIdx.x * WAVE + threadIdx.x;
+  if (i >= n) return;
+  int st = pk_status[i];
+  g1a a;
+  if (st == 0 && !jac_to_aff(ld_g1j(b.pk_jac, b.n, i), a)) st = -1;
+  if (st == 0) {
+    g1a_to_be96(a, out + (size_t)i * out_stride);
+    const uint32_t idx = b.pk_index[i];
+    if (b.pk_comb[(size_t)idx * (Comb::kEntries * W_PKTAB) + PK_COMB_FLAG_WORD]) st = 256;
+  }
+  status[i] = st;
+}
+
+static inline dim3 grid_for(uint32_t n) { return dim3((n + WAVE - 1) / WAVE); }
+
+void launch_pk_comb(const PipelineBuffers& b, uint32_t n_list, hipStream_t s) {
+  if (n_list) hipLaunchKernelGGL(k_pk_comb, grid_for(n_list), dim3(WAVE), 0, s, b, n_list, b.status + b.n);
+}
+void launch_pk_comb_build(const uint32_t* keys, uint32_t n, uint32_t* jac, uint32_t* inv, uint32_t* dst,
+                          uint8_t* flag, hipStream_t s) {
+  if (!n) return;
+  hipLaunchKernelGGL(k_pk_comb_build, grid_for(n), dim3(WAVE), 0, s, keys, n, jac);
+  launch_batch_inv(jac, n * Comb::kEntries, 2 * W_FP, inv, n * Comb::kEntries, s);
+  hipLaunchKernelGGL(k_pk_comb_write, grid_for(n), dim3(WAVE), 0, s, jac, inv, n, dst, flag);
+}
+void launch_pk_comb_out(const PipelineBuffers& b, uint32_t n, uint8_t* out, uint32_t out_stride, int32_t* status,
+                        hipStream_t s) {
+  if (n) hipLaunchKernelGGL(k_pk_comb_out, grid_for(n), dim3(WAVE), 0, s, b, n, b.status + b.n, out, out_stride, status);
+}
diff --git a/lodestar_amd/csrc/kernels.h b/lodestar_amd/csrc/kernels.h
--- a/lodestar_amd/csrc/kernels.h
+++ b/lodestar_amd/csrc/kernels.h
@@ -10,6 +10,10 @@
 #define W_G2J (6 * W_FP)
 #define W_FP12 (12 * W_FP)
 #define W_PKTAB 32
+#ifndef PK_COMB_T
+#define PK_COMB_T 2
+#endif
+#define PK_COMB_ENTRIES (PK_COMB_T * 8)
 #define MILLER_STEPS 68
 #define W_LINE (3 * 2 * W_FP)
 
@@ -29,6 +33,11 @@
   const uint32_t* agg_sets;
   uint32_t n_agg;
   uint32_t pk_direct1;
+  const uint32_t* pk_comb;
+  const uint32_t* comb_sets;
+  uint32_t n_comb;
+  const uint32_t* rest_sets;
+  uint32_t n_rest;
   const uint64_t* scalars;
   uint32_t* scal_tab;
   const uint32_t* job_first_set;
@@ -75,6 +84,11 @@
                        bool exclusive = true);
 void launch_pk_aggregate(const PipelineBuffers& b, uint32_t n_sets, hipStream_t s);
 void launch_pk_finish(const PipelineBuffers& b, uint32_t n_sets, hipStream_t s);
+void launch_pk_comb(const PipelineBuffers& b, uint32_t n_list, hipStream_t s);
+void launch_pk_comb_build(const uint32_t* keys, uint32_t n, uint32_t* jac, uint32_t* inv, uint32_t* dst, uint8_t* flag,
+                          hipStream_t s);
+void launch_pk_comb_out(const PipelineBuffers& b, uint32_t n, uint8_t* out, uint32_t out_stride, int32_t* status,
+                        hipStream_t s);
 void launch_batch_inv(const uint32_t* src, uint32_t src_stride, int w0, uint32_t* dst, uint32_t n, hipStream_t s);
 void launch_pk_affine(const PipelineBuffers& b, uint32_t n_sets, hipStream_t s);
 void launch_h_affine(const PipelineBuffers& b, hipStream_t s);
diff --git a/lodestar_amd/csrc/pk_comb.hpp b/lodestar_amd/csrc/pk_comb.hpp
--- /dev/null
+++ b/lodestar_amd/csrc/pk_comb.hpp
@@ -0,0 +1,83 @@
+#pragma once
+#include "curve.hpp"
+
+#ifndef PK_COMB_T
+#define PK_COMB_T 2
+#endif
+
+namespace pk_comb {
+
+constexpr int kWindows = 8;
+constexpr int kOdd = 8;
+
+template <int T>
+struct Comb {
+  static_assert(T == 1 || T == 2 || T == 4 || T == 8, "blocks per key: 1, 2, 4 or 8");
+  static constexpr int kT = T;
+  static constexpr int kB = kWindows / T;
+  static constexpr int kEntries = T * kOdd;
+};
+template <int T>
+BLS_HD int entry_of(int j, int e) {
+  return j * kOdd + e;
+}
+template <int T>
+BLS_HD int window_of(int j, int i) {
+  return Comb<T>::kB * j + i;
+}
+
+BLS_HD int digit(uint64_t w, int k, bool& neg) {
+  const int d = 2 * (int)((w >> (4 * k)) & 15u) - 15;
+  neg = d < 0;
+  return (d < 0 ? -d : d) >> 1;
+}
+
+template <int T, class Store>
+BLS_INL bool build(const g1a& P, Store store) {
+  typedef Comb<T> C;
+  bool finite = true;
+  g1j base = jac_from_aff(P);
+#pragma unroll 1
+  for (int j = 0; j < T; j++) {
+    const g1j two = jac_dbl(base);
+    g1j t = base;
+#pragma unroll 1
+    for (int e = 0; e < kOdd; e++) {
+      if (e) t = jac_add(t, two);
+      finite = finite && !jac_is_inf(t);
+      store(entry_of<T>(j, e), t);
+    }
+    if (j + 1 < T) {
+#pragma unroll 1
+      for (int k = 0; k < 4 * C::kB; k++) base = jac_dbl(base);
+    }
+  }
+  return finite;
+}
+
+template <int T, class LoadEntry>
+BLS_INL g1j eval(uint64_t w, LoadEntry entry) {
+  typedef Comb<T> C;
+  g1j r = jac_infinity<fp>();
+#pragma unroll 1
+  for (int i = C::kB - 1; i >= 0; i--) {
+    if (i != C::kB - 1) {
+#pragma unroll 1
+      for (int k = 0; k < 4; k++) r = jac_dbl(r);
+    }
+#pragma unroll 1
+    for (int t = 0; t < 2 * T; t++) {
+      const int j = t >> 1;
+      const bool hi = t & 1;
+      bool neg;
+      const int e = digit(w, window_of<T>(j, i) + (hi ? kWindows : 0), neg);
+      g1a q = entry(entry_of<T>(j, e));
+      if (hi) q.x = fp_mul(q.x, G1_BETA);
+      q.y = fp_select(neg, fp_neg(q.y), q.y);
+      r = jac_add_aff(r, q);
+    }
+  }
+  return r;
+}
+
+}
diff --git a/lodestar_amd/csrc/pk_comb_host.hpp b/lodestar_amd/csrc/pk_comb_host.hpp
--- /dev/null
+++ b/lodestar_amd/csrc/pk_comb_host.hpp
@@ -0,0 +1,20 @@
+#pragma once
+#include <stdint.h>
+
+namespace pk_comb {
+
+enum Action { kSkip = 0, kBuild = 1, kDrop = 2 };
+inline Action upload_action(bool enabled, uint32_t comb_n, uint32_t first) {
+  if (!enabled || first > comb_n) return comb_n ? kDrop : kSkip;
+  return kBuild;
+}
+inline Action on_alloc_failure() { return kDrop; }
+inline bool usable(bool enabled, const void* buf, uint32_t comb_n, uint32_t table_n) {
+  return enabled && buf && table_n > 0 && comb_n >= table_n;
+}
+inline uint32_t grown_keys(uint32_t need, uint32_t have) {
+  const uint64_t g = (uint64_t)have + have / 2;
+  return g > need ? (uint32_t)(g > UINT32_MAX ? UINT32_MAX : g) : need;
+}
+
+}
diff --git a/lodestar_amd/csrc/runtime.cpp b/lodestar_amd/csrc/runtime.cpp
--- a/lodestar_amd/csrc/runtime.cpp
+++ b/lodestar_amd/csrc/runtime.cpp
@@ -401,6 +401,22 @@
   if (table_mode || bytes_agg)
     for (uint32_t i = 0; i < n; i++)
       if (b.set_pk_first[s0 + i + 1] - b.set_pk_first[s0 + i] >= 2) agg_sets.push_back(i);
+  std::vector<uint32_t> pk_lists;
+  uint32_t n_comb = 0;
+  if (table_mode && pk_comb::usable(opt.pk_comb != 0, d.comb.p, d.comb_n, d.table_n)) {
+    auto comb_set = [&](uint32_t i) {
+      const uint32_t first = b.set_pk_first[s0 + i];
+      return b.set_pk_first[s0 + i + 1] - first == 1 &&
+             (d.comb_flagged.empty() ||
+              !std::binary_search(d.comb_flagged.begin(), d.comb_flagged.end(), b.pk_index[first]));
+    };
+    for (uint32_t i = 0; i < n; i++) n_comb += comb_set(i);
+    if (n_comb && n_comb != n) {
+      pk_lists.resize(n);
+      uint32_t c = 0, r = n_comb;
+      for (uint32_t i = 0; i < n; i++) pk_lists[comb_set(i) ? c++ : r++] = i;
+    }
+  }
 
   const double t_struct_ms = host_trace() ? ms_since(t_prep0) : 0;
   uint32_t sig_w = 96;
@@ -416,7 +432,7 @@
                o_ufirst = al256(o_franges + (size_t)std::max(n_franges, 1u) * 8),
                o_usets = al256(o_ufirst + (size_t)(n_units + 1) * 4), o_umsgi = al256(o_usets + (size_t)unit_sets.size() * 4),
                o_cfirst = al256(o_umsgi + (size_t)n_units * 4), o_citems = al256(o_cfirst + (size_t)(n_chunks + 1) * 4),
-               o_agg = al256(o_citems + chunk_items.size() * 4), o_slices = al256(o_agg + agg_sets.size() * 4),
+               o_agg = al256(o_citems + chunk_items.size() * 4), o_slices = al256(o_agg + (agg_sets.size() + pk_lists.size()) * 4),
                o_rslices = al256(o_slices + slices.size() * 4), o_ftree = al256(o_rslices + range_slices.size() * 4),
                o_pk = al256(o_ftree + ftree.size() * 4);
   size_t in_bytes;
@@ -465,6 +481,7 @@
   memcpy(hin + o_cfirst, chunk_first.data(), chunk_first.size() * 4);
   memcpy(hin + o_citems, chunk_items.data(), chunk_items.size() * 4);
   if (!agg_sets.empty()) memcpy(hin + o_agg, agg_sets.data(), agg_sets.size() * 4);
+  if (!pk_lists.empty()) memcpy(hin + o_agg + agg_sets.size() * 4, pk_lists.data(), pk_lists.size() * 4);
   if (!slices.empty()) memcpy(hin + o_slices, slices.data(), slices.size() * 4);
   memcpy(hin + o_rslices, range_slices.data(), range_slices.size() * 4);
   if (!ftree.empty()) memcpy(hin + o_ftree, ftree.data(), ftree.size() * 4);
@@ -520,6 +537,15 @@
   pb.agg_sets = reinterpret_cast<uint32_t*>(din + o_agg);
   pb.n_agg = (uint32_t)agg_sets.size();
   pb.pk_direct1 = 1;
+  if (n_comb) {
+    pb.pk_comb = d.comb.p;
+    pb.n_comb = n_comb;
+    pb.n_rest = n - n_comb;
+    if (!pk_lists.empty()) {
+      pb.comb_sets = reinterpret_cast<uint32_t*>(din + o_agg) + agg_sets.size();
+      pb.rest_sets = pb.comb_sets + n_comb;
+    }
+  }
   pb.scalars = reinterpret_cast<uint64_t*>(din + o_scal);
   pb.job_first_set = reinterpret_cast<uint32_t*>(din + o_jobs);
   pb.n_jobs = nj;
@@ -1667,6 +1693,7 @@
     if (e) (void)hipEventDestroy(e);
   d->helper.release_all();
   d->table.release();
+  d->comb.release();
   if (d->table_stream) (void)hipStreamDestroy(d->table_stream);
   delete d;
 }
@@ -1839,6 +1866,7 @@
     const long j = strtol(v, nullptr, 10);
     if (j >= 1 && j <= MILLER_MAX_SEGS) ctx->opt.miller_segments = j;
   }
+  if (const char* v = getenv("BLSGPU_PK_COMB")) ctx->opt.pk_comb = !(v[0] == '0' && v[1] == 0);
   try {
     for (int id : ids) {
       Device* d = new Device();
@@ -1876,6 +1904,16 @@
     n = std::min(n, d->table_n);
   }
   return n;
+}
+
+uint64_t blsgpu_pubkeys_comb_bytes(const blsgpu_ctx* ctx) {
+  uint64_t bytes = 0;
+  if (!ctx) return 0;
+  for (Device* d : ctx->devs) {
+    std::shared_lock<std::shared_mutex> lk(d->table_mu);
+    bytes += (uint64_t)d->comb.cap * 4;
+  }
+  return bytes;
 }
 
 int blsgpu_pubkeys_upload(blsgpu_ctx* ctx, uint32_t first_index, const uint8_t* pk96, uint32_t n) {
@@ -1908,6 +1946,9 @@
       HIPCHK(hipStreamSynchronize(ts));
       int err = 0;
       for (uint32_t i = 0; i < n && !err; i++) err = hst[i];
+      pk_comb::Action act = pk_comb::upload_action(ctx->opt.pk_comb != 0, d->comb_n, first_index);
+      CombUpload cu;
+      if (!err && act == pk_comb::kBuild && !cu.build(tmp, n, dst, ts)) act = pk_comb::on_alloc_failure();
       if (!err) {
         std::unique_lock<std::shared_mutex> lk(d->table_mu);
         if (need > d->table.cap / W_PKTAB) {
@@ -1920,8 +1961,37 @@
         }
         HIPCHK(hipMemcpyAsync(d->table.p + (size_t)first_index * W_PKTAB, tmp, (size_t)n * W_PKTAB * 4,
                               hipMemcpyDeviceToDevice, ts));
+        if (act == pk_comb::kBuild && need > d->comb.cap / kCombKeyWords) {
+          DevBuf<uint32_t> nc;
+          try {
+            nc.ensure((size_t)pk_comb::grown_keys(need, d->comb_n) * kCombKeyWords);
+            if (d->comb_n)
+              HIPCHK(hipMemcpyAsync(nc.p, d->comb.p, (size_t)d->comb_n * kCombKeyWords * 4, hipMemcpyDeviceToDevice, ts));
+            d->comb.release();
+            d->comb = nc;
+          } catch (HipError&) {
+            (void)hipGetLastError();
+            nc.release();
+            act = pk_comb::on_alloc_failure();
+          }
+        }
+        if (act == pk_comb::kBuild) {
+          HIPCHK(hipMemcpyAsync(d->comb.p + (size_t)first_index * kCombKeyWords, cu.entries, (size_t)n * kCombKeyWords * 4,
+                                hipMemcpyDeviceToDevice, ts));
+          auto& fl = d->comb_flagged;
+          fl.erase(std::lower_bound(fl.begin(), fl.end(), first_index), std::lower_bound(fl.begin(), fl.end(), need));
+          for (uint32_t i = 0; i < n; i++)
+            if (cu.flags[i]) fl.insert(std::lower_bound(fl.begin(), fl.end(), first_index + i), first_index + i);
+        }
         HIPCHK(hipStreamSynchronize(ts));
         d->table_n = std::max(d->table_n, need);
+        if (act == pk_comb::kBuild) {
+          d->comb_n = std::max(d->comb_n, need);
+        } else if (act == pk_comb::kDrop) {
+          d->comb.release();
+          d->comb_n = 0;
+          d->comb_flagged.clear();
+        }
       }
       (void)hipFree(dpk);
       (void)hipFree(dst);
diff --git a/lodestar_amd/csrc/runtime_internal.hpp b/lodestar_amd/csrc/runtime_internal.hpp
--- a/lodestar_amd/csrc/runtime_internal.hpp
+++ b/lodestar_amd/csrc/runtime_internal.hpp
@@ -17,6 +17,7 @@
 #include "../../include/blsgpu.h"
 #include "batch_rand.hpp"
 #include "kernels.h"
+#include "pk_comb_host.hpp"
 
 namespace blsgpu_rt __attribute__((visibility("hidden"))) {
 
@@ -197,6 +198,9 @@
   std::shared_mutex table_mu;
   DevBuf<uint32_t> table;
   uint32_t table_n = 0;
+  DevBuf<uint32_t> comb;
+  uint32_t comb_n = 0;
+  std::vector<uint32_t> comb_flagged;
   std::mutex q_mu;
   std::condition_variable q_cv;
   std::deque<Task> queue;
@@ -219,6 +223,39 @@
   bool blocking_sync = true;
   std::mutex fail_mu;
   double fail_rate = 0;
+};
+
+constexpr size_t kCombKeyWords = (size_t)PK_COMB_ENTRIES * W_PKTAB;
+
+struct CombUpload {
+  uint32_t* entries = nullptr;
+  std::vector<uint8_t> flags;
+  uint32_t* jac = nullptr;
+  uint32_t* inv = nullptr;
+  static constexpr uint32_t kChunk = 32768;
+  ~CombUpload() {
+    for (uint32_t* p : {entries, jac, inv})
+      if (p) (void)hipFree(p);
+  }
+  bool build(const uint32_t* keys, uint32_t n, int8_t* flag_dev, hipStream_t ts) {
+    const uint32_t chunk = std::min(n, kChunk);
+    if (hipMalloc((void**)&entries, (size_t)n * kCombKeyWords * 4) != hipSuccess ||
+        hipMalloc((void**)&jac, (size_t)chunk * PK_COMB_ENTRIES * W_G1J * 4) != hipSuccess ||
+        hipMalloc((void**)&inv, (size_t)chunk * PK_COMB_ENTRIES * W_FP * 4) != hipSuccess) {
+      (void)hipGetLastError();
+      return false;
+    }
+    for (uint32_t c0 = 0; c0 < n; c0 += chunk) {
+      const uint32_t cn = std::min(chunk, n - c0);
+      launch_pk_comb_build(keys + (size_t)c0 * W_PKTAB, cn, jac, inv, entries + (size_t)c0 * kCombKeyWords,
+                           reinterpret_cast<uint8_t*>(flag_dev) + c0, ts);
+      HIPCHK(hipGetLastError());
+    }
+    flags.resize(n);
+    HIPCHK(hipMemcpyAsync(flags.data(), flag_dev, n, hipMemcpyDeviceToHost, ts));
+    HIPCHK(hipStreamSynchronize(ts));
+    return true;
+  }
 };
 
 struct Options {
@@ -265,6 +302,7 @@
   int64_t urgent_max_sets = 512;
   int64_t urgent_excl = 0;
   int64_t urgent_wait_us = 300;
+  int64_t pk_comb = 1;
   int64_t group_adapt = 1;
   bool same_run(const struct Options& o) const {
     return group_sets == o.group_sets && profile == o.profile && dedupe == o.dedupe && miller_k == o.miller_k &&
diff --git a/lodestar_amd/native.py b/lodestar_amd/native.py
--- a/lodestar_amd/native.py
+++ b/lodestar_amd/native.py
@@ -32,6 +32,7 @@
     "blsgpu_device_count",
     "blsgpu_pubkeys_upload",
     "blsgpu_pubkeys_count",
+    "blsgpu_pubkeys_comb_bytes",
     "blsgpu_verify",
     "blsgpu_submit",
     "blsgpu_set_option",
@@ -143,6 +144,8 @@
     lib.blsgpu_pubkeys_upload.restype = ctypes.c_int
     lib.blsgpu_pubkeys_count.argtypes = [ctypes.c_void_p]
     lib.blsgpu_pubkeys_count.restype = ctypes.c_uint32
+    lib.blsgpu_pubkeys_comb_bytes.argtypes = [ctypes.c_void_p]
+    lib.blsgpu_pubkeys_comb_bytes.restype = ctypes.c_uint64
     lib.blsgpu_verify.argtypes = [ctypes.c_void_p, ctypes.POINTER(Batch), ctypes.c_void_p, ctypes.POINTER(Stats)]
     lib.blsgpu_verify.restype = ctypes.c_int
     lib.blsgpu_submit.argtypes = [ctypes.c_void_p, ctypes.POINTER(Batch), ctypes.c_void_p, ctypes.POINTER(Stats),
@@ -429,6 +432,10 @@
     def pubkeys_count(self):
         return self._lib.blsgpu_pubkeys_count(self.h)
 
+    @property
+    def pubkeys_comb_bytes(self):
+        return self._lib.blsgpu_pubkeys_comb_bytes(self.h)
+
     def verify_raw(self, job_first_set, sigs, sig_len, msgs, pk_bytes=None, set_pk_first=None, pk_index=None,
                    job_flags=None, sig_stride=None, seed=0x4C4F444553544152):
         b, keep = make_batch(job_first_set, sigs, sig_len, msgs, pk_bytes, set_pk_first, pk_index, job_flags,
```
